# ruiminshen/yolo-tf

Hardware: AMD Instinct MI355X
Metric: train_throughput (higher is better)
Workload: dtype bf16; 1 GPU; Darknet-19 YOLOv2 VOC-20 416x416 training step (standardise+fwd+loss+bwd+Adam), batch 16 per GPU (BASELINE configs[1]); global_batch=16, parallelism=dp1, optimizer=adam, weights=random-init (Xavier, seed 0), collective=none (1 rank)

## Files before the change

include/yolo2_hip.h:

```cpp
#ifndef YOLO2_HIP_H
#define YOLO2_HIP_H

#include <stddef.h>
#include <stdint.h>

#ifdef __cplusplus
extern "C" {
#endif

enum { YOLO2_F32 = 0, YOLO2_BF16 = 1 };
enum {
    YOLO2_OK = 0,
    YOLO2_E_ARG = 1,
    YOLO2_E_LAUNCH = 2,
    YOLO2_E_UNSUPPORTED = 3
};

int yolo2_abi_version(void);
const char *yolo2_last_error(void);
uint32_t yolo2_crc32c(const void *data, size_t n, uint32_t crc);
int yolo2_shutdown(void);
int yolo2_check_async_errors(void *stream);
#define YOLO2_ASYNC_ERROR_WORDS 8
int yolo2_async_error_snapshot(unsigned *host_words, void *stream);

size_t yolo2_conv2d_workspace_bytes(int B, int H, int W, int Cp, int Nf, int ksize, int dtype);
size_t yolo2_bn_workspace_bytes(int C);
size_t yolo2_bias_grad_workspace_bytes(int ld);
size_t yolo2_image_prep_workspace_bytes(int B);
size_t yolo2_loss_workspace_bytes(int B, int cells, int A);
size_t yolo2_nms_workspace_bytes(int B, int N, int C);
size_t yolo2_clip_workspace_bytes(int nseg);
size_t yolo2_augment_workspace_bytes(int B);

int yolo2_conv2d(const void *P, const void *F, const float *bias, void *O,
                 int B, int H, int W, int Cp, int ldp, int Nf, int ldo, int ksize,
                 int dtype, void *stream);

int yolo2_conv2d_ws(const void *P, const void *F, const float *bias, void *O, float *ws,
                    size_t ws_bytes, int B, int H, int W, int Cp, int ldp, int Nf, int ldo,
                    int ksize, int dtype, void *stream);

int yolo2_conv2d_wgrad_accumulates(int B, int H, int W, int Cin, int ldx, int Cout, int ldy, int ksize, int dtype);
int yolo2_conv2d_wgrad(const void *X, const void *dY, float *dW,
                       int B, int H, int W, int Cin, int ldx, int Cout, int ldy, int ksize,
                       int dtype, void *stream);

size_t yolo2_conv2d_wgrad_workspace_bytes(int B, int H, int W, int Cin, int ldx, int Cout, int ldy, int ksize, int dtype);
int yolo2_conv2d_wgrad_ws(const void *X, const void *dY, float *dW, float *ws, size_t ws_bytes, int B, int H, int W,
                          int Cin, int ldx, int Cout, int ldy, int ksize, int dtype, void *stream);
int yolo2_set_deterministic(int on);
int yolo2_get_deterministic(void);

int yolo2_filter_prep(const float *W, void *Ffwd, void *Fdgr, int ksize, int Cin, int ldcin,
                      int Cout, int ldcout, int dtype, void *stream);

#define YOLO2_FILTER_PREP_TILE 64
#define YOLO2_FILTER_PREP_TILE_N 128
int yolo2_filter_prep_blocks(int ksize, int ldcin, int ldcout);
typedef struct yolo2_filter_desc {
    const float *W;
    void *Ffwd;
    void *Fdgr;
    int ksize, cin, ldcin, cout, ldcout, first_block;
} yolo2_filter_desc;
int yolo2_filter_prep_batch(const yolo2_filter_desc *descs_device, int n, int total_blocks, int dtype,
                            void *stream);

int yolo2_adam_filter_prep(const yolo2_filter_desc *descs_device, int n, int total_blocks, const long *small_ranges_device, int n_small,
                           float *params, const float *grads, float *m, float *v, float alpha, float beta1, float beta2, float eps,
                           float gscale, int dtype, void *stream);

int yolo2_conv2d_bias_leaky(const void *P, const void *F, const float *bias, void *O, float *ws, size_t ws_bytes, int B,
                            int H, int W, int Cp, int ldp, int Nf, int ldo, int ksize, float alpha, int dtype, void *stream);

int yolo2_conv2d_dgrad_bn(const void *dY, const void *F, void *dX, float *ws, size_t ws_bytes, int B, int H, int W, int Cp, int ldp,
                          int Nf, int ldo, int ksize, const void *Yprev, const float *mean, const float *var, const float *gamma,
                          const float *beta, float *dgamma, float *dbeta, float *bn_part, double *red_ws, float eps, float alpha,
                          int *pending, int dtype, void *stream);
int yolo2_conv2d_dgrad_bn_fuses(int B, int H, int W, int Nf, int ksize, int dtype);
int yolo2_bn_part_to_grads(float *bn_part, int C, float *dgamma, float *dbeta, void *stream);

#define YOLO2_BN_PART_ROWS 256
int yolo2_conv2d_bn(const void *P, const void *F, void *O, float *ws, size_t ws_bytes, int B, int H, int W, int Cp, int ldp,
                    int Nf, int ldo, int ksize, const float *shift, float *bn_part, int dtype, void *stream);
int yolo2_bn_finalize(float *bn_part, const float *shift, long M, int C, float *mean, float *var, float *moving_mean,
                      float *moving_var, double decay, void *stream);

int yolo2_last_bn_part_rows(void);
int yolo2_bn_fin_supported(int rows, int C, int dtype);
int yolo2_bn_leaky_fin(const void *Y, const float *bn_part, int rows, const float *shift, float *mean, float *var, float *moving_mean,
                       float *moving_var, double decay, const float *gamma, const float *beta, void *A, long M, int C, int lda,
                       float eps, float alpha, float *zero, long zero_floats, int dtype, void *stream);
int yolo2_bn_leaky_pool_fin(const void *Y, const float *bn_part, int rows, const float *shift, float *mean, float *var,
                            float *moving_mean, float *moving_var, double decay, const float *gamma, const float *beta, void *P,
                            unsigned char *idx, void *ymax, void *A_full, int B, int H, int W, int C, int ldp, float eps, float alpha,
                            float *zero, long zero_floats, int dtype, void *stream);
int yolo2_bn_leaky_bwd_apply_fin(const void *dA, int ldda, const void *Y, const float *mean, const float *var, const float *gamma,
                                 const float *beta, const float *part, int rows, long plane_stride, float *dgamma, float *dbeta,
                                 void *dY, long M, int C, float eps, float alpha, float *zero, long zero_floats, int dtype, void *stream);
int yolo2_bn_leaky_pool_bwd_apply_fin(const void *dP, int lddp, const unsigned char *idx, const void *Y, const float *mean,
                                      const float *var, const float *gamma, const float *beta, const float *part, int rows,
                                      long plane_stride, float *dgamma, float *dbeta, void *dY, int B, int H, int W, int C, float eps,
                                      float alpha, float *zero, long zero_floats, int dtype, void *stream);
int yolo2_first_layer_wgrad_bn(const void *X, const void *Y, const void *dP, int lddp, const unsigned char *idx, const float *mean, const float *var,
                               const float *gamma, const float *beta, const float *part, int rows, long plane_stride, float *dgamma, float *dbeta,
                               float *dW, int B, int H, int W, int Cin, float eps, float alpha, float *zero, long zero_floats, int dtype, void *stream);
int yolo2_bn_leaky_bwd_reduce_part(const void *dA, int ldda, const void *Y, const float *mean, const float *var, const float *gamma,
                                   const float *beta, double *ws, int *rows, int rows_limit, long M, int C, float eps, float alpha,
                                   int dtype, void *stream);
int yolo2_bn_leaky_pool_bwd_reduce_part(const void *dP, int lddp, const unsigned char *idx, const void *Y, const float *mean,
                                        const float *var, const float *gamma, const float *beta, double *ws, int *rows,
                                        int rows_limit, int B, int H, int W, int C, float eps, float alpha, int dtype, void *stream);

int yolo2_first_layer_stats(const void *P, const void *F, int B, int H, int W, const float *shift, float *bn_part, int dtype, void *stream);
int yolo2_first_layer_bn_leaky_pool(const void *P, const void *F, const float *mean, const float *var, const float *gamma,
                                    const float *beta, void *Pout, unsigned char *idx, int B, int H, int W, int ldp, float eps,
                                    float alpha, int dtype, void *stream);
int yolo2_first_layer_pool_bwd_reduce(const void *P, const void *F, const void *dP, int lddp, const unsigned char *idx,
                                      const float *mean, const float *var, const float *gamma, const float *beta, float *bn_part,
                                      int B, int H, int W, float eps, float alpha, int dtype, void *stream);
int yolo2_first_layer_pool_bwd_apply(const void *P, const void *F, const void *dP, int lddp, const unsigned char *idx,
                                     const float *mean, const float *var, const float *gamma, const float *beta,
                                     const float *dgamma, const float *dbeta, void *dY, int B, int H, int W, float eps, float alpha,
                                     int dtype, void *stream);

int yolo2_bn_stats(const void *Y, float *mean, float *var, double *ws, long M, int C,
                   int dtype, void *stream);
int yolo2_bn_stats_ema(const void *Y, float *mean, float *var, float *moving_mean, float *moving_var,
                       double decay, double *ws, long M, int C, int dtype, void *stream);
int yolo2_bn_ema(float *moving_mean, float *moving_var, const float *mean, const float *var,
                 int C, double decay, void *stream);
int yolo2_bn_leaky(const void *Y, const float *mean, const float *var, const float *gamma,
                   const float *beta, void *A, long M, int C, int lda, float eps, float alpha,
                   int dtype, void *stream);
int yolo2_bn_leaky_bwd_reduce(const void *dA, int ldda, const void *Y, const float *mean,
                              const float *var, const float *gamma, const float *beta,
                              float *dgamma, float *dbeta, double *ws, long M, int C,
                              float eps, float alpha, int dtype, void *stream);
int yolo2_bn_leaky_bwd_apply(const void *dA, int ldda, const void *Y, const float *mean,
                             const float *var, const float *gamma, const float *beta,
                             const float *dgamma, const float *dbeta, void *dY, long M, int C,
                             float eps, float alpha, int dtype, void *stream);

int yolo2_bn_leaky_pool(const void *Y, const float *mean, const float *var, const float *gamma, const float *beta, void *P,
                        unsigned char *idx, int B, int H, int W, int C, int ldp, float eps, float alpha, int dtype, void *stream);
int yolo2_bn_leaky_pool_bwd_reduce(const void *dP, int lddp, const unsigned char *idx, const void *Y, const float *mean,
                                   const float *var, const float *gamma, const float *beta, float *dgamma, float *dbeta,
                                   double *ws, int B, int H, int W, int C, float eps, float alpha, int dtype, void *stream);
int yolo2_bn_leaky_pool_bwd_apply(const void *dP, int lddp, const unsigned char *idx, const void *Y, const float *mean,
                                  const float *var, const float *gamma, const float *beta, const float *dgamma,
                                  const float *dbeta, void *dY, int B, int H, int W, int C, float eps, float alpha,
                                  int dtype, void *stream);

int yolo2_maxpool_fwd(const void *A, void *P, int B, int H, int W, int C, int stride,
                      int dtype, void *stream);
int yolo2_maxpool_bwd(const void *A, const void *dP, void *dA, int B, int H, int W, int C,
                      int stride, int dtype, void *stream);
int yolo2_maxpool_bwd_acc(const void *A, const void *dP, void *dA, int B, int H, int W, int C, int dtype, void *stream);

int yolo2_reorg(const void *in, void *out, int B, int H, int W, int C, int ldo, int dtype,
                void *stream);
int yolo2_reorg_bwd(const void *dout, int ldd, void *din, int B, int H, int W, int C, int dtype,
                    void *stream);
int yolo2_copy_channels(const void *src, int lds, void *dst, int ldd, long M, int C, int dtype,
                        void *stream);
int yolo2_add_inplace(void *dst, const void *src, long n, int dtype, void *stream);
int yolo2_bias_grad(const void *dY, int ld, float *dbias, double *ws, long M, int C, int dtype,
                    void *stream);

int yolo2_image_prep(const float *img, void *out, double *ws, int B, int HW, int mode, int dtype,
                     void *stream);

int yolo2_head_decode(const void *logits, int ld, const float *anchors, float *conf,
                      float *xy_min, float *xy_max, int *nan_flag, int B, int cell_h, int cell_w,
                      int A, int C, int dtype, void *stream);

int yolo2_head_decode_attrs(const void *logits, int ld, const float *anchors, float *iou, float *prob,
                            float *xy, float *wh, int B, int cell_h, int cell_w, int A, int C,
                            int dtype, void *stream);

int yolo2_loss(const void *logits, int ld, const float *anchors, const float *mask,
               const float *prob, const float *coords, const float *off_min, const float *off_max,
               const float *areas, const float *hparam, float *objectives, void *dlogits,
               float *ws, int B, int cell_h, int cell_w, int A, int C, int dtype, void *stream);
int yolo2_loss_partials(const void *logits, int ld, const float *anchors, const float *mask, const float *prob,
                        const float *coords, const float *off_min, const float *off_max, const float *areas,
                        const float *hparam, void *dlogits, float *ws, int B, int cell_h, int cell_w, int A, int C, int dtype,
                        void *stream);
int yolo2_loss_objectives(const float *ws, float *objectives, int B, int cell_h, int cell_w, int A, void *stream);
int yolo2_loss_box(const void *logits, int ld, const float *anchors, const float *mask,
                   const float *prob, const float *coords, const float *off_min, const float *off_max,
                   const float *areas, const float *hparam, float *objectives, void *dlogits,
                   float *ws, int B, int cell_h, int cell_w, int A, int C, int dtype, void *stream, int box_loss);
int yolo2_loss_box_partials(const void *logits, int ld, const float *anchors, const float *mask, const float *prob,
                            const float *coords, const float *off_min, const float *off_max, const float *areas,
                            const float *hparam, void *dlogits, float *ws, int B, int cell_h, int cell_w, int A, int C, int dtype,
                            void *stream, int box_loss);
typedef struct yolo2_loss_options {
    int   size;
    int   box_loss;
    int   class_loss;
    int   rescore;
    float ignore_thresh;
    float label_smoothing;
    float focal_gamma;
} yolo2_loss_options;
int yolo2_loss_ex(const void *logits, int ld, const float *anchors, const float *mask,
                  const float *prob, const float *coords, const float *off_min, const float *off_max,
                  const float *areas, const float *hparam, float *objectives, void *dlogits,
                  float *ws, int B, int cell_h, int cell_w, int A, int C, int dtype, void *stream, const yolo2_loss_options *opt);
int yolo2_loss_ex_partials(const void *logits, int ld, const float *anchors, const float *mask, const float *prob,
                           const float *coords, const float *off_min, const float *off_max, const float *areas,
                           const float *hparam, void *dlogits, float *ws, int B, int cell_h, int cell_w, int A, int C, int dtype,
                           void *stream, const yolo2_loss_options *opt);

int yolo1_loss(const void *net, int ld, const float *mask, const float *prob, const float *coords, const float *off_min,
               const float *off_max, const float *areas, const float *hparam, float *objectives, void *dnet, float *ws,
               int B, int cell_h, int cell_w, int boxes_per_cell, int C, int dtype, void *stream);
int yolo1_head_decode(const void *net, int ld, float *conf, float *xy_min, float *xy_max, int *nan_flag, int B, int cell_h,
                      int cell_w, int boxes_per_cell, int C, int dtype, void *stream);
int yolo2_leaky_bwd(const void *A, const void *dA, void *dZ, long n, float alpha, int dtype, void *stream);
int yolo2_dropout(const void *X, void *Y, unsigned char *mask, long n, float keep_prob, unsigned long long seed, int dtype,
                  void *stream);
int yolo2_dropout_bwd(const void *dY, const unsigned char *mask, void *dX, long n, float keep_prob, int dtype, void *stream);
int yolo2_l2_regularizer(const float *w, float *g, long n, float scale, double *loss, void *stream);

int yolo2_nms(float *conf, const float *xy_min, const float *xy_max, int *order_out, int *ws,
              int B, int N, int C, float threshold, float threshold_iou, void *stream);

#define YOLO2_NMS_HARD 0
#define YOLO2_NMS_LINEAR 1
#define YOLO2_NMS_GAUSSIAN 2
int yolo2_soft_nms(float *conf, const float *xy_min, const float *xy_max, int *order_out, int B, int N, int C, int method,
                   float threshold, float threshold_iou, float sigma, void *stream);

#define YOLO2_WBF_MAX_CANDIDATES 4096
#define YOLO2_WBF_FLAG_CANDIDATES 1
#define YOLO2_WBF_FLAG_CLUSTERS 2
#define YOLO2_WBF_FLAG_ROWS 4
size_t yolo2_wbf_workspace_bytes(int B, int C, int max_per_class);
int yolo2_tta_gather(const float *conf, const float *xy_min, const float *xy_max, float *out_conf, float *out_xy_min, float *out_xy_max,
                     int B, int N, int C, int M, int offset, float sx, float sy, float cell_w0, int flip, void *stream);
int yolo2_wbf(const float *conf, const float *xy_min, const float *xy_max, float *out_conf, float *out_xy_min, float *out_xy_max, int *rows,
              int *flags, void *ws, int B, int M, int C, int V, int max_per_class, int R, float threshold, float fuse_iou, void *stream);

int yolo2_adam(float *w, const float *g, float *m, float *v, long n, float alpha, float beta1,
               float beta2, float eps, float gscale, void *stream);
int yolo2_momentum(float *w, const float *g, float *acc, long n, float lr, float momentum,
                   float gscale, void *stream);
int yolo2_sgd(float *w, const float *g, long n, float lr, float gscale, void *stream);
int yolo2_rmsprop(float *w, const float *g, float *ms, float *mom, long n, float lr, float decay,
                  float momentum, float eps, float gscale, void *stream);
int yolo2_adagrad(float *w, const float *g, float *acc, long n, float lr, float gscale,
                  void *stream);
int yolo2_adadelta(float *w, const float *g, float *acc, float *acc_update, long n, float lr,
                   float rho, float eps, float gscale, void *stream);
int yolo2_ftrl(float *w, const float *g, float *accum, float *linear, long n, float lr, float lr_power,
               float l1, float l2, float gscale, void *stream);
int yolo2_ema_update(float *ema, const float *w, long n, float one_minus_decay, void *stream);
enum { YOLO2_GRAD_STORE = 0, YOLO2_GRAD_ADD = 1, YOLO2_GRAD_FINAL = 2 };
#define YOLO2_GRAD_COMBINE_CHUNK 4096
int yolo2_grad_combine(float *g, float *acc, float *w, long n, int mode, float scale, float decay, float shrink,
                       const long *ranges_device, int n_ranges, void *stream);
int yolo2_scale(float *x, long n, float scale, void *stream);
int yolo2_zero_ranges(float *x, const long *ranges_host, int nranges, void *stream);
int yolo2_bn_fold(const float *W, const float *gamma, const float *beta, const float *moving_mean,
                  const float *moving_var, float *Wf, float *bias, long rows, int C, float eps, void *stream);
int yolo2_clip_by_norm(float *g, const long *seg_off, int nseg, float clip, double *ws,
                       void *stream);
size_t yolo2_clip_fixed_workspace_bytes(int nseg);
int yolo2_clip_by_norm_fixed(float *g, const long *seg_off, int nseg, float clip, double *ws, size_t ws_bytes, void *stream);

int yolo2_selftest_tr16(short *out, void *stream);
int yolo2_debug_last_conv_plan(int *out8);
int yolo2_debug_conv_route(int B, int H, int W, int Cp, int ldp, int Nf, int ldo, int ksize, int dtype, int mode, int align_bits, size_t ws_bytes,
                           int cus, unsigned exclude, int *out12);
int yolo2_debug_noop(void *stream);
int yolo2_debug_set_igemm_tap(int mode);
int yolo2_debug_set_s4_abl(int abl);
int yolo2_debug_set_pp(int grid, int sched, int min_steps, int min_share);
int yolo2_debug_set_pp_cost(int cv);
int yolo2_debug_set_streamk_wait_us(int us, int unclamped);
int yolo2_debug_last_wgrad_plan(int *out8);
void yolo2_debug_set_wgrad_variant(int variant);
int yolo2_debug_wgrad_row_plan(int B, int H, int W, int Cin, int Cout, int cus, int force_variant, int *out9);
int yolo2_debug_wgrad_ws_plan(int B, int H, int W, int Cin, int ldx, int Cout, int ldy, int ksize, int dtype, int cus, int *out4);
int yolo2_debug_magic_u32(unsigned d, unsigned *m, unsigned *s);

#define YOLO2_AUG_FLIP 1u
#define YOLO2_AUG_BRIGHTNESS 2u
#define YOLO2_AUG_SATURATION 4u
#define YOLO2_AUG_HUE 8u
#define YOLO2_AUG_CONTRAST 16u
#define YOLO2_AUG_NOISE 32u
#define YOLO2_AUG_GRAY 64u
typedef struct yolo2_augment_params {
    long long src_offset;
    int src_w, src_h;
    int crop_x, crop_y, crop_w, crop_h;
    unsigned flags;
    float brightness, saturation, hue, contrast, noise_scale;
    unsigned long long noise_seed;
} yolo2_augment_params;
int yolo2_augment_images(const unsigned char *src, const yolo2_augment_params *params_device, double *ws, float *out,
                         int B, int H, int W, int any_contrast, void *stream);

typedef struct yolo2_compose_tile {
    long long src_offset;
    int src_w, src_h;
    int crop_x, crop_y, crop_w, crop_h;
    int view_w, view_h;
    int origin_x, origin_y;
    int x0, y0, x1, y1;
    unsigned flip;
} yolo2_compose_tile;
int yolo2_compose_images(const unsigned char *src, const yolo2_compose_tile *tiles, const yolo2_augment_params *photo,
                         const float *mix, double *ws, float *out, int B, int L, int T, int H, int W, float fill,
                         int any_contrast, void *stream);

int yolo2_transform_labels(const int *objects_class, const float *objects_coord, const int *first_object, float *mask,
                           float *prob, float *coords, float *offset_xy_min, float *offset_xy_max, float *areas, int B,
                           int classes, int cell_width, int cell_height, int *error_flag, void *stream);

int yolo2_set_stream_workgroups(int n);
int yolo2_get_stream_workgroups(void);
int yolo2_cast_f32_bf16(const float *src, void *dst, long n, void *stream);
int yolo2_cast_bf16_f32(const void *src, float *dst, long n, void *stream);
int yolo2_debug_occupy(int workgroups, int *stop, int *started, int max_us, void *stream);

enum { YOLO2_EVAL_MODE_DETECT = 0, YOLO2_EVAL_MODE_ALL = 1 };
enum { YOLO2_EVAL_FP = 0, YOLO2_EVAL_TP = 1, YOLO2_EVAL_IGNORED = 2 };
#define YOLO2_EVAL_MAX_GT_PER_IMAGE 512
#define YOLO2_EVAL_MAX_CLASSES (1 << 20)
#define YOLO2_EVAL_STATE_WORDS 2
typedef struct {
    float score;
    int image;
    int box;
    unsigned class_flag;
} yolo2_eval_record;
size_t yolo2_eval_record_bytes(long max_records);
size_t yolo2_eval_collect_workspace_bytes(int B);
size_t yolo2_eval_workspace_bytes(long max_records, int C);
size_t yolo2_eval_result_bytes(int C);
int yolo2_eval_collect(const float *conf, const float *xy_min, const float *xy_max, const int *gt_class, const float *gt_box,
                       const unsigned char *gt_difficult, const int *gt_first, int G, int B, int N, int C, int n_valid, int image_base,
                       int mode, float threshold, float iou_threshold, void *records, long max_records, unsigned long long *state,
                       int *npos, int *ws, void *stream);
int yolo2_eval_finalize(const void *records, long max_records, unsigned long long *state, const int *npos, int C, int n_images, int N,
                        void *ws, size_t ws_bytes, void *results, void *sorted_records, int *cum_tp, int *cum_fp, void *stream);

#define YOLO2_EVAL_COCO_MAX_AREAS 4
#define YOLO2_EVAL_COCO_MAX_IOUS 10
#define YOLO2_EVAL_COCO_MAX_RECALLS 101
#define YOLO2_EVAL_COCO_MAX_SLICES 8
#define YOLO2_EVAL_COCO_MAX_DETS 128
#define YOLO2_EVAL_COCO_MAX_CLASSES 1024
typedef struct {
    float score;
    int image;
    int box;
    int cls;
    int rank;
    unsigned reserved;
    unsigned long long matched;
    unsigned long long ignored;
} yolo2_eval_coco_record;
size_t yolo2_eval_coco_record_bytes(long max_records);
size_t yolo2_eval_coco_collect_workspace_bytes(int B, int N, int C);
size_t yolo2_eval_coco_workspace_bytes(long max_records, int C);
size_t yolo2_eval_coco_result_bytes(int S, int T, int A, int C);
int yolo2_eval_coco_collect(const float *conf, const float *xy_min, const float *xy_max, const int *gt_class, const float *gt_box,
                            const float *gt_area, const unsigned char *gt_flags, const int *gt_first, const float *scale, int G, int B,
                            int N, int C, int n_valid, int image_base, int mode, float threshold, const float *area_ranges, int A,
                            const float *iou_thresholds, int T, int max_dets, void *records, long max_records,
                            unsigned long long *state, int *npig, void *ws, size_t ws_bytes, void *stream);
int yolo2_eval_coco_finalize(const void *records, long max_records, unsigned long long *state, const int *npig, int C, int n_images, int N,
                             int A, int T, int max_dets, const int *slices, int S, const double *recall_thresholds, int R, void *ws,
                             size_t ws_bytes, void *results, void *stream);

#define YOLO2_ANCHOR_MAX_K 32
#define YOLO2_ANCHOR_MAX_JOBS 65535
#define YOLO2_ANCHOR_MAX_BOXES ((1 << 27) - 1)
size_t yolo2_anchor_workspace_bytes(int jobs, int kmax);
int yolo2_anchor_assign(const float *boxes, int n, const float *centroids, const int *job_k, int jobs, int kmax,
                        unsigned long long *ws, size_t ws_bytes, const int *done, unsigned char *assignment, void *stream);
int yolo2_anchor_update(float *centroids, const int *job_k, int jobs, int kmax, unsigned long long *ws, size_t ws_bytes, int n,
                        int *done, int *iterations, long long *counts, double *avg_iou, void *stream);

#define YOLO2_HIST_BUCKETS 1550
#define YOLO2_HIST_WORDS (YOLO2_HIST_BUCKETS + 6)
typedef struct yolo2_hist_job {
    const void *base;
    long long rows;
    int c, ld, dtype;
    int first_item;
} yolo2_hist_job;
size_t yolo2_histogram_workspace_bytes(int njobs);
size_t yolo2_histogram_result_bytes(int njobs);
int yolo2_histogram_items(long long rows, int c, int ld, int dtype);
int yolo2_histogram(const yolo2_hist_job *jobs, int njobs, int items, void *out, size_t out_bytes, void *ws, size_t ws_bytes, void *stream);

#define YOLO2_IMAGE_GROUP 8
#define YOLO2_IMAGE_RECORD_BYTES 16
typedef struct yolo2_image_job {
    const void *base;
    long long rows;
    int c, ld, dtype;
    int first_item;
    long long out_offset;
    long long sum_offset;
} yolo2_image_job;
size_t yolo2_image_summary_workspace_bytes(int njobs, long long sum_pixels);
size_t yolo2_image_summary_result_bytes(int njobs, long long image_bytes);
int yolo2_image_summary_items(long long rows, int c, int ld, int dtype);
// ... 32 lines not shown
```

yolo_tf_amd/_lib.py:

```python
import ctypes
import os

_HERE = os.path.dirname(os.path.abspath(__file__))
LIB_PATH = os.environ.get('YOLO2_LIB_PATH') or os.path.join(_HERE, 'csrc', 'libyolo2hip.so')

F32, BF16 = 0, 1
I8_OUT_I8, I8_OUT_BF16, I8_OUT_F32, I8_OUT_ACC = 0, 1, 2, 3
NMS_METHODS = {'hard': 0, 'linear': 1, 'gaussian': 2}
BOX_LOSSES = {'mse': 0, 'iou': 1, 'giou': 2, 'diou': 3, 'ciou': 4}
CLASS_LOSSES = {'mse': 0, 'ce': 1, 'focal': 2}


class HipKernelError(RuntimeError):
    pass


class LossOptions(ctypes.Structure):
    _fields_ = [('size', ctypes.c_int), ('box_loss', ctypes.c_int), ('class_loss', ctypes.c_int), ('rescore', ctypes.c_int),
                ('ignore_thresh', ctypes.c_float), ('label_smoothing', ctypes.c_float), ('focal_gamma', ctypes.c_float)]


_p = ctypes.c_void_p
_i = ctypes.c_int
_l = ctypes.c_long
_f = ctypes.c_float

SIGNATURES = {
    'yolo2_conv2d': [_p, _p, _p, _p, _i, _i, _i, _i, _i, _i, _i, _i, _i, _p],
    'yolo2_conv2d_ws': [_p, _p, _p, _p, _p, ctypes.c_size_t, _i, _i, _i, _i, _i, _i, _i, _i, _i, _p],
    'yolo2_conv2d_bias_leaky': [_p, _p, _p, _p, _p, ctypes.c_size_t, _i, _i, _i, _i, _i, _i, _i, _i, _f, _i, _p],
    'yolo2_conv2d_dgrad_bn': [_p, _p, _p, _p, ctypes.c_size_t, _i, _i, _i, _i, _i, _i, _i, _i, _p, _p, _p, _p, _p, _p, _p, _p, _p, _f, _f, _p, _i, _p],
    'yolo2_bn_part_to_grads': [_p, _i, _p, _p, _p],
    'yolo2_debug_noop': [_p],
    'yolo2_conv2d_wgrad': [_p, _p, _p, _i, _i, _i, _i, _i, _i, _i, _i, _i, _p],
    'yolo2_conv2d_wgrad_ws': [_p, _p, _p, _p, ctypes.c_size_t, _i, _i, _i, _i, _i, _i, _i, _i, _i, _p],
    'yolo2_set_deterministic': [_i],
    'yolo2_filter_prep': [_p, _p, _p, _i, _i, _i, _i, _i, _i, _p],
    'yolo2_filter_prep_batch': [_p, _i, _i, _i, _p],
    'yolo2_adam_filter_prep': [_p, _i, _i, _p, _i, _p, _p, _p, _p, _f, _f, _f, _f, _f, _i, _p],
    'yolo2_first_layer_stats': [_p, _p, _i, _i, _i, _p, _p, _i, _p],
    'yolo2_first_layer_bn_leaky_pool': [_p, _p, _p, _p, _p, _p, _p, _p, _i, _i, _i, _i, _f, _f, _i, _p],
    'yolo2_first_layer_pool_bwd_reduce': [_p, _p, _p, _i, _p, _p, _p, _p, _p, _p, _i, _i, _i, _f, _f, _i, _p],
    'yolo2_first_layer_pool_bwd_apply': [_p, _p, _p, _i, _p, _p, _p, _p, _p, _p, _p, _p, _i, _i, _i, _f, _f, _i, _p],
    'yolo2_conv2d_bn': [_p, _p, _p, _p, ctypes.c_size_t, _i, _i, _i, _i, _i, _i, _i, _i, _p, _p, _i, _p],
    'yolo2_bn_finalize': [_p, _p, _l, _i, _p, _p, _p, _p, ctypes.c_double, _p],
    'yolo2_bn_leaky_fin': [_p, _p, _i, _p, _p, _p, _p, _p, ctypes.c_double, _p, _p, _p, _l, _i, _i, _f, _f, _p, _l, _i, _p],
    'yolo2_bn_leaky_pool_fin': [_p, _p, _i, _p, _p, _p, _p, _p, ctypes.c_double, _p, _p, _p, _p, _p, _p, _i, _i, _i, _i, _i, _f, _f, _p, _l, _i, _p],
    'yolo2_bn_leaky_bwd_apply_fin': [_p, _i, _p, _p, _p, _p, _p, _p, _i, _l, _p, _p, _p, _l, _i, _f, _f, _p, _l, _i, _p],
    'yolo2_first_layer_wgrad_bn': [_p, _p, _p, _i, _p, _p, _p, _p, _p, _p, _i, _l, _p, _p, _p, _i, _i, _i, _i, _f, _f, _p, _l, _i, _p],
    'yolo2_bn_leaky_pool_bwd_apply_fin': [_p, _i, _p, _p, _p, _p, _p, _p, _p, _i, _l, _p, _p, _p, _i, _i, _i, _i, _f, _f, _p, _l, _i, _p],
    'yolo2_bn_leaky_bwd_reduce_part': [_p, _i, _p, _p, _p, _p, _p, _p, _p, _i, _l, _i, _f, _f, _i, _p],
    'yolo2_bn_leaky_pool_bwd_reduce_part': [_p, _i, _p, _p, _p, _p, _p, _p, _p, _p, _i, _i, _i, _i, _i, _f, _f, _i, _p],
    'yolo2_bn_leaky_pool': [_p, _p, _p, _p, _p, _p, _p, _i, _i, _i, _i, _i, _f, _f, _i, _p],
    'yolo2_bn_leaky_pool_bwd_reduce': [_p, _i, _p, _p, _p, _p, _p, _p, _p, _p, _p, _i, _i, _i, _i, _f, _f, _i, _p],
    'yolo2_bn_leaky_pool_bwd_apply': [_p, _i, _p, _p, _p, _p, _p, _p, _p, _p, _p, _i, _i, _i, _i, _f, _f, _i, _p],
    'yolo2_augment_images': [_p, _p, _p, _p, _i, _i, _i, _i, _p],
    'yolo2_compose_images': [_p, _p, _p, _p, _p, _p, _i, _i, _i, _i, _i, _f, _i, _p],
    'yolo2_transform_labels': [_p, _p, _p, _p, _p, _p, _p, _p, _p, _i, _i, _i, _i, _p, _p],
    'yolo2_bn_stats': [_p, _p, _p, _p, _l, _i, _i, _p],
    'yolo2_bn_stats_ema': [_p, _p, _p, _p, _p, ctypes.c_double, _p, _l, _i, _i, _p],
    'yolo2_bn_ema': [_p, _p, _p, _p, _i, ctypes.c_double, _p],
    'yolo2_bn_leaky': [_p, _p, _p, _p, _p, _p, _l, _i, _i, _f, _f, _i, _p],
    'yolo2_bn_leaky_bwd_reduce': [_p, _i, _p, _p, _p, _p, _p, _p, _p, _p, _l, _i, _f, _f, _i, _p],
    'yolo2_bn_leaky_bwd_apply': [_p, _i, _p, _p, _p, _p, _p, _p, _p, _p, _l, _i, _f, _f, _i, _p],
    'yolo2_maxpool_fwd': [_p, _p, _i, _i, _i, _i, _i, _i, _p],
    'yolo2_maxpool_bwd': [_p, _p, _p, _i, _i, _i, _i, _i, _i, _p],
    'yolo2_maxpool_bwd_acc': [_p, _p, _p, _i, _i, _i, _i, _i, _p],
    'yolo2_reorg': [_p, _p, _i, _i, _i, _i, _i, _i, _p],
    'yolo2_reorg_bwd': [_p, _i, _p, _i, _i, _i, _i, _i, _p],
    'yolo2_copy_channels': [_p, _i, _p, _i, _l, _i, _i, _p],
    'yolo2_add_inplace': [_p, _p, _l, _i, _p],
    'yolo2_bias_grad': [_p, _i, _p, _p, _l, _i, _i, _p],
    'yolo2_image_prep': [_p, _p, _p, _i, _i, _i, _i, _p],
    'yolo2_head_decode': [_p, _i, _p, _p, _p, _p, _p, _i, _i, _i, _i, _i, _i, _p],
    'yolo2_head_decode_attrs': [_p, _i, _p, _p, _p, _p, _p, _i, _i, _i, _i, _i, _i, _p],
    'yolo2_loss': [_p, _i, _p, _p, _p, _p, _p, _p, _p, ctypes.POINTER(_f), _p, _p, _p, _i, _i, _i, _i, _i, _i, _p],
    'yolo2_loss_partials': [_p, _i, _p, _p, _p, _p, _p, _p, _p, ctypes.POINTER(_f), _p, _p, _i, _i, _i, _i, _i, _i, _p],
    'yolo2_loss_objectives': [_p, _p, _i, _i, _i, _i, _p],
    'yolo2_loss_box': [_p, _i, _p, _p, _p, _p, _p, _p, _p, ctypes.POINTER(_f), _p, _p, _p, _i, _i, _i, _i, _i, _i, _p, _i],
    'yolo2_loss_box_partials': [_p, _i, _p, _p, _p, _p, _p, _p, _p, ctypes.POINTER(_f), _p, _p, _i, _i, _i, _i, _i, _i, _p, _i],
    'yolo2_loss_ex': [_p, _i, _p, _p, _p, _p, _p, _p, _p, ctypes.POINTER(_f), _p, _p, _p, _i, _i, _i, _i, _i, _i, _p, ctypes.POINTER(LossOptions)],
    'yolo2_loss_ex_partials': [_p, _i, _p, _p, _p, _p, _p, _p, _p, ctypes.POINTER(_f), _p, _p, _i, _i, _i, _i, _i, _i, _p, ctypes.POINTER(LossOptions)],
    'yolo1_loss': [_p, _i, _p, _p, _p, _p, _p, _p, ctypes.POINTER(_f), _p, _p, _p, _i, _i, _i, _i, _i, _i, _p],
    'yolo1_head_decode': [_p, _i, _p, _p, _p, _p, _i, _i, _i, _i, _i, _i, _p],
    'yolo2_leaky_bwd': [_p, _p, _p, _l, _f, _i, _p],
    'yolo2_dropout': [_p, _p, _p, _l, _f, ctypes.c_ulonglong, _i, _p],
    'yolo2_dropout_bwd': [_p, _p, _p, _l, _f, _i, _p],
    'yolo2_l2_regularizer': [_p, _p, _l, _f, _p, _p],
    'yolo2_nms': [_p, _p, _p, _p, _p, _i, _i, _i, _f, _f, _p],
    'yolo2_soft_nms': [_p, _p, _p, _p, _i, _i, _i, _i, _f, _f, _f, _p],
    'yolo2_tta_gather': [_p, _p, _p, _p, _p, _p, _i, _i, _i, _i, _i, _f, _f, _f, _i, _p],
    'yolo2_wbf': [_p, _p, _p, _p, _p, _p, _p, _p, _p, _i, _i, _i, _i, _i, _i, _f, _f, _p],
    'yolo2_adam': [_p, _p, _p, _p, _l, _f, _f, _f, _f, _f, _p],
    'yolo2_momentum': [_p, _p, _p, _l, _f, _f, _f, _p],
    'yolo2_sgd': [_p, _p, _l, _f, _f, _p],
    'yolo2_rmsprop': [_p, _p, _p, _p, _l, _f, _f, _f, _f, _f, _p],
    'yolo2_adagrad': [_p, _p, _p, _l, _f, _f, _p],
    'yolo2_adadelta': [_p, _p, _p, _p, _l, _f, _f, _f, _f, _p],
    'yolo2_clip_by_norm': [_p, _p, _i, _f, _p, _p],
    'yolo2_clip_by_norm_fixed': [_p, _p, _i, _f, _p, ctypes.c_size_t, _p],
    'yolo2_ftrl': [_p, _p, _p, _p, _l, _f, _f, _f, _f, _f, _p],
    'yolo2_scale': [_p, _l, _f, _p],
    'yolo2_ema_update': [_p, _p, _l, _f, _p],
    'yolo2_grad_combine': [_p, _p, _p, _l, _i, _f, _f, _f, _p, _i, _p],
    'yolo2_zero_ranges': [_p, _p, _i, _p],
    'yolo2_bn_fold': [_p, _p, _p, _p, _p, _p, _p, _l, _i, _f, _p],
    'yolo2_selftest_tr16': [_p, _p],
    'yolo2_set_stream_workgroups': [_i],
    'yolo2_cast_f32_bf16': [_p, _p, _l, _p],
    'yolo2_cast_bf16_f32': [_p, _p, _l, _p],
    'yolo2_debug_occupy': [_i, _p, _p, _i, _p],
    'yolo2_check_async_errors': [_p],
    'yolo2_async_error_snapshot': [_p, _p],
    'yolo2_debug_set_streamk_wait_us': [_i, _i],
    'yolo2_eval_collect': [_p, _p, _p, _p, _p, _p, _p, _i, _i, _i, _i, _i, _i, _i, _f, _f, _p, _l, _p, _p, _p, _p],
    'yolo2_eval_finalize': [_p, _l, _p, _p, _i, _i, _i, _p, ctypes.c_size_t, _p, _p, _p, _p, _p],
    'yolo2_eval_coco_collect': [_p] * 9 + [_i] * 7 + [_f, _p, _i, _p, _i, _i, _p, _l, _p, _p, _p, ctypes.c_size_t, _p],
    'yolo2_eval_coco_finalize': [_p, _l, _p, _p, _i, _i, _i, _i, _i, _i, _p, _i, _p, _i, _p, ctypes.c_size_t, _p, _p],
    'yolo2_anchor_assign': [_p, _i, _p, _p, _i, _i, _p, ctypes.c_size_t, _p, _p, _p],
    'yolo2_anchor_update': [_p, _p, _i, _i, _p, ctypes.c_size_t, _i, _p, _p, _p, _p, _p],
    'yolo2_histogram': [_p, _i, _i, _p, ctypes.c_size_t, _p, ctypes.c_size_t, _p],
    'yolo2_image_summary': [_p, _i, _i, _p, ctypes.c_size_t, _p, ctypes.c_size_t, _p],
    'yolo2_conv2d_i8': [_p, _p, _p, _p, _p, _i, _i, _i, _i, _i, _i, _i, _i, _f, _f, _i, _p],
    'yolo2_absmax': [_p, _i, _p, _p],
    'yolo2_calib_histogram': [_p, _i, _p, _p],
    'yolo2_quantize': [_p, _i, _p, _i, _l, _i, _f, _i, _p],
    'yolo2_maxpool_i8': [_p, _i, _p, _i, _i, _i, _i, _i, _i, _p],
    'yolo2_reorg_i8': [_p, _p, _i, _i, _i, _i, _i, _p],
}

QUERIES = {
    'yolo2_abi_version': (_i, []),
    'yolo2_last_error': (ctypes.c_char_p, []),
    'yolo2_shutdown': (_i, []),
    'yolo2_crc32c': (ctypes.c_uint32, [_p, ctypes.c_size_t, ctypes.c_uint32]),
    'yolo2_conv2d_wgrad_accumulates': (_i, [_i] * 9),
    'yolo2_filter_prep_blocks': (_i, [_i, _i, _i]),
    'yolo2_conv2d_dgrad_bn_fuses': (_i, [_i] * 6),
    'yolo2_debug_set_wgrad_variant': (None, [_i]),
    'yolo2_last_bn_part_rows': (_i, []),
    'yolo2_get_stream_workgroups': (_i, []),
    'yolo2_bn_fin_supported': (_i, [_i, _i, _i]),
    'yolo2_debug_last_conv_plan': (_i, [ctypes.POINTER(_i)]),
    'yolo2_debug_conv_route': (_i, [_i] * 11 + [ctypes.c_size_t, _i, ctypes.c_uint, ctypes.POINTER(_i)]),
    'yolo2_debug_set_igemm_tap': (_i, [_i]),
    'yolo2_debug_set_pp': (_i, [_i, _i, _i, _i]),
    'yolo2_debug_set_pp_cost': (_i, [_i]),
    'yolo2_debug_set_s4_abl': (_i, [_i]),
    'yolo2_debug_last_wgrad_plan': (_i, [ctypes.POINTER(_i)]),
    'yolo2_debug_wgrad_row_plan': (_i, [_i, _i, _i, _i, _i, _i, _i, ctypes.POINTER(_i)]),
    'yolo2_debug_wgrad_ws_plan': (_i, [_i] * 10 + [ctypes.POINTER(_i)]),
    'yolo2_conv2d_wgrad_workspace_bytes': (ctypes.c_size_t, [_i] * 9),
    'yolo2_get_deterministic': (_i, []),
    'yolo2_debug_magic_u32': (_i, [ctypes.c_uint, ctypes.POINTER(ctypes.c_uint), ctypes.POINTER(ctypes.c_uint)]),
    'yolo2_conv2d_workspace_bytes': (ctypes.c_size_t, [_i] * 7),
    'yolo2_bn_workspace_bytes': (ctypes.c_size_t, [_i]),
    'yolo2_bias_grad_workspace_bytes': (ctypes.c_size_t, [_i]),
    'yolo2_image_prep_workspace_bytes': (ctypes.c_size_t, [_i]),
    'yolo2_loss_workspace_bytes': (ctypes.c_size_t, [_i, _i, _i]),
    'yolo2_nms_workspace_bytes': (ctypes.c_size_t, [_i, _i, _i]),
    'yolo2_wbf_workspace_bytes': (ctypes.c_size_t, [_i, _i, _i]),
    'yolo2_clip_workspace_bytes': (ctypes.c_size_t, [_i]),
    'yolo2_clip_fixed_workspace_bytes': (ctypes.c_size_t, [_i]),
    'yolo2_augment_workspace_bytes': (ctypes.c_size_t, [_i]),
    'yolo2_eval_record_bytes': (ctypes.c_size_t, [_l]),
    'yolo2_eval_collect_workspace_bytes': (ctypes.c_size_t, [_i]),
    'yolo2_eval_workspace_bytes': (ctypes.c_size_t, [_l, _i]),
    'yolo2_eval_result_bytes': (ctypes.c_size_t, [_i]),
    'yolo2_eval_coco_record_bytes': (ctypes.c_size_t, [_l]),
    'yolo2_eval_coco_collect_workspace_bytes': (ctypes.c_size_t, [_i, _i, _i]),
    'yolo2_eval_coco_workspace_bytes': (ctypes.c_size_t, [_l, _i]),
    'yolo2_eval_coco_result_bytes': (ctypes.c_size_t, [_i, _i, _i, _i]),
    'yolo2_anchor_workspace_bytes': (ctypes.c_size_t, [_i, _i]),
    'yolo2_histogram_workspace_bytes': (ctypes.c_size_t, [_i]),
    'yolo2_histogram_result_bytes': (ctypes.c_size_t, [_i]),
    'yolo2_histogram_items': (_i, [ctypes.c_longlong, _i, _i, _i]),
    'yolo2_image_summary_workspace_bytes': (ctypes.c_size_t, [_i, ctypes.c_longlong]),
    'yolo2_image_summary_result_bytes': (ctypes.c_size_t, [_i, ctypes.c_longlong]),
    'yolo2_image_summary_items': (_i, [ctypes.c_longlong, _i, _i, _i]),
    'yolo2_image_summary_depth': (_i, [_i]),
}


class AugmentParams(ctypes.Structure):
    _fields_ = [('src_offset', ctypes.c_longlong), ('src_w', _i), ('src_h', _i), ('crop_x', _i), ('crop_y', _i), ('crop_w', _i), ('crop_h', _i),
                ('flags', ctypes.c_uint), ('brightness', _f), ('saturation', _f), ('hue', _f), ('contrast', _f), ('noise_scale', _f),
                ('noise_seed', ctypes.c_ulonglong)]


class ComposeTile(ctypes.Structure):
    _fields_ = [('src_offset', ctypes.c_longlong), ('src_w', _i), ('src_h', _i), ('crop_x', _i), ('crop_y', _i), ('crop_w', _i), ('crop_h', _i),
                ('view_w', _i), ('view_h', _i), ('origin_x', _i), ('origin_y', _i), ('x0', _i), ('y0', _i), ('x1', _i), ('y1', _i),
                ('flip', ctypes.c_uint)]


class HistJob(ctypes.Structure):
    _fields_ = [('base', ctypes.c_void_p), ('rows', ctypes.c_longlong), ('c', _i), ('ld', _i), ('dtype', _i), ('first_item', _i)]


class ImageJob(ctypes.Structure):
    _fields_ = [('base', ctypes.c_void_p), ('rows', ctypes.c_longlong), ('c', _i), ('ld', _i), ('dtype', _i), ('first_item', _i),
                ('out_offset', ctypes.c_longlong), ('sum_offset', ctypes.c_longlong)]


class AbsmaxJob(ctypes.Structure):
    _fields_ = [('base', ctypes.c_void_p), ('rows', ctypes.c_longlong), ('c', _i), ('ld', _i), ('dtype', _i), ('slot', _i)]


CALIB_BINS = 2048
CALIB_WORDS = CALIB_BINS + 2


class CalibJob(ctypes.Structure):
    _fields_ = [('base', ctypes.c_void_p), ('rows', ctypes.c_longlong), ('c', _i), ('ld', _i), ('dtype', _i), ('slot', _i), ('limit', _f), ('inv_width', _f)]


class FilterDesc(ctypes.Structure):
    _fields_ = [('W', ctypes.c_void_p), ('Ffwd', ctypes.c_void_p), ('Fdgr', ctypes.c_void_p), ('ksize', _i), ('cin', _i),
                ('ldcin', _i), ('cout', _i), ('ldcout', _i), ('first_block', _i)]


_lib = None
MISSING = set()


def _mapped_hip_runtimes():
    try:
        with open('/proc/self/maps') as f:
            return sorted({line.split()[-1] for line in f if 'libamdhip64' in line})
    except OSError:
        return []


def load():
    global _lib
    if _lib is not None:
        return _lib
    if not os.path.exists(LIB_PATH):
        raise HipKernelError(
            'HIP extension %s is missing: run `python yolo_tf_amd/csrc/build.py` (or __graft_entry__.build()). '
            'There is no CPU fallback.' % LIB_PATH)
    import torch
    lib = ctypes.CDLL(LIB_PATH)
    runtimes = _mapped_hip_runtimes()
    if len(runtimes) > 1:
        raise HipKernelError('two HIP runtimes are mapped in this process (%s): something loaded %s before torch' % (', '.join(runtimes), LIB_PATH))
    baseline = os.environ.get('YOLO2_LIB_BASELINE') == '1' and bool(os.environ.get('YOLO2_LIB_PATH'))

    def resolve(name):
        try:
            return getattr(lib, name)
        except AttributeError:
            if not baseline:
                raise
            MISSING.add(name)

            def absent(*_args, _name=name):
                raise HipKernelError('%s is not exported by the baseline library %s' % (_name, LIB_PATH))
            setattr(lib, name, absent)
            return None
    for name, (res, args) in QUERIES.items():
        fn = resolve(name)
        if fn is not None:
            fn.restype = res
            fn.argtypes = args
    for name, args in SIGNATURES.items():
        fn = resolve(name)
        if fn is not None:
            fn.restype = _i
            fn.argtypes = args
    _lib = lib
    over = env_overrides()
    if over:
        import warnings
        warnings.warn('YOLO2_* switches set in the environment change kernel selection away from the tested defaults: %s' % ', '.join(over))
    return lib


def env_overrides():
    return sorted('%s=%s' % (k, v) for k, v in os.environ.items() if k.startswith('YOLO2_'))


def query(name, *args):
    return getattr(load(), name)(*args)


def call(name, *args):
    lib = load()
    rc = getattr(lib, name)(*args)
    if rc != 0:
        raise HipKernelError('%s failed (code %d): %s' % (name, rc, lib.yolo2_last_error().decode()))


def ptr(t):
    return None if t is None else t.data_ptr()


def dtype_code(torch_dtype):
    import torch
    if torch_dtype == torch.float32:
        return F32
    if torch_dtype == torch.bfloat16:
        return BF16
    raise ValueError('unsupported dtype %r' % (torch_dtype,))
```

yolo_tf_amd/csrc/bn.hip:

```cpp
#include "common.h"
#include "bn_leaky.h"
#include "colsum.h"

template <typename T>
__global__ __launch_bounds__(256) void bn_leaky_kernel(const T *__restrict__ Y, const float *__restrict__ mean, const float *__restrict__ var,
                                                       const float *__restrict__ gamma, const float *__restrict__ beta, T *__restrict__ A,
                                                       long M, int C, int lda, float eps, float alpha) {
    constexpr int N = Vec16<T>::N;
    RowMap rm(C, N);
    if (!rm.active) return;
    float mu[N], sc[N], bt[N];
#pragma unroll
    for (int j = 0; j < N; ++j) {
        int c = rm.cg * N + j;
        mu[j] = mean[c];
        sc[j] = bn_inv_std(var[c], eps) * gamma[c];
        bt[j] = beta[c];
    }
    for (long r = (long)blockIdx.x * rm.rpp + rm.rs; r < M; r += (long)gridDim.x * rm.rpp) {
        Vec16<T> v = ld16(Y + r * C + rm.cg * N), o;
#pragma unroll
        for (int j = 0; j < N; ++j) o.set(j, bn_leaky(v.get(j), mu[j], sc[j], bt[j], alpha));
        st16(A + r * lda + rm.cg * N, o);
    }
}

static int rowmap_grid(long M, int C, int vec, int rows_per_thread) {
    int tpr = C / vec, rpp = 256 / tpr;
    if (rpp < 1) rpp = 1;
    long g = (M + (long)rpp * rows_per_thread - 1) / ((long)rpp * rows_per_thread);
    if (g > 4096) g = 4096;
    if (g < 1) g = 1;
    return (int)g;
}

extern "C" int yolo2_bn_leaky(const void *Y, const float *mean, const float *var, const float *gamma, const float *beta,
                              void *A, long M, int C, int lda, float eps, float alpha, int dtype, void *stream) {
    Y2_CHECK_ARG(Y && mean && var && gamma && beta && A && M > 0 && C > 0 && lda >= C);
    const int vec = dtype == YOLO2_BF16 ? 8 : 4;
    Y2_CHECK_ARG(C % vec == 0 && C / vec <= 256 && lda % vec == 0);
    int grid = rowmap_grid(M, C, vec, 4);
    Y2_DISPATCH_DTYPE(dtype, bn_leaky_kernel<T><<<grid, 256, 0, (hipStream_t)stream>>>((const T *)Y, mean, var, gamma, beta, (T *)A, M, C, lda, eps, alpha));
    Y2_CHECK_LAUNCH();
    return YOLO2_OK;
}

template <typename T>
__global__ __launch_bounds__(256) void bn_bwd_reduce_kernel(const T *__restrict__ dA, int ldda, const T *__restrict__ Y, const float *__restrict__ mean,
                                                            const float *__restrict__ var, const float *__restrict__ gamma, const float *__restrict__ beta,
                                                            float *__restrict__ ws, long M, int C, float eps, float alpha) {
    constexpr int N = Vec16<T>::N;
    RowMap rm(C, N);
    float part[2][N];
    float mu[N], inv[N], ga[N], bt[N];
#pragma unroll
    for (int j = 0; j < N; ++j) {
        part[0][j] = part[1][j] = 0.f;
        int c = rm.cg * N + j;
        bool ok = rm.active;
        mu[j] = ok ? mean[c] : 0.f;
        inv[j] = ok ? bn_inv_std(var[c], eps) : 0.f;
        ga[j] = ok ? gamma[c] : 0.f;
        bt[j] = ok ? beta[c] : 0.f;
    }
    if (rm.active) {
        const long step = (long)gridDim.x * rm.rpp;
        long r = (long)blockIdx.x * rm.rpp + rm.rs;
        auto accum = [&](const Vec16<T> &y, const Vec16<T> &d) {
#pragma unroll
            for (int j = 0; j < N; ++j) {
                const BnBwdTerm t = bn_leaky_bwd(y.get(j), d.get(j), mu[j], inv[j], ga[j], bt[j], alpha);
                part[0][j] += t.g * t.xh;
                part[1][j] += t.g;
            }
        };
        for (; r + 3 * step < M; r += 4 * step) {
            Vec16<T> y[4], d[4];
#pragma unroll
            for (int u = 0; u < 4; ++u) {
                y[u] = ld16(Y + (r + u * step) * C + rm.cg * N);
                d[u] = ld16(dA + (r + u * step) * ldda + rm.cg * N);
            }
#pragma unroll
            for (int u = 0; u < 4; ++u) accum(y[u], d[u]);
        }
        for (; r < M; r += step) {
            Vec16<T> y = ld16(Y + r * C + rm.cg * N), d = ld16(dA + r * ldda + rm.cg * N);
            accum(y, d);
        }
    }
    block_colsum_store<N, 2>(part, rm, C, ws, gridDim.x);
}
extern "C" int yolo2_bn_leaky_bwd_reduce(const void *dA, int ldda, const void *Y, const float *mean, const float *var, const float *gamma,
                                         const float *beta, float *dgamma, float *dbeta, double *ws, long M, int C, float eps, float alpha,
                                         int dtype, void *stream) {
    Y2_CHECK_ARG(dA && Y && mean && var && gamma && beta && dgamma && dbeta && ws && M > 0 && C > 0 && ldda >= C);
    const int vec = dtype == YOLO2_BF16 ? 8 : 4;
    Y2_CHECK_ARG(C % vec == 0 && C / vec <= 256 && ldda % vec == 0);
    hipStream_t st = (hipStream_t)stream;
    const int nb = colsum_grid(M, C, vec);
    float *part = (float *)ws;
    Y2_DISPATCH_DTYPE(dtype, bn_bwd_reduce_kernel<T><<<nb, 256, 0, st>>>((const T *)dA, ldda, (const T *)Y, mean, var, gamma, beta, part, M, C, eps, alpha));
    reduce_finalize_kernel<1><<<cdiv(C, 16), 256, 0, st>>>(part, nb, C, M, dgamma, dbeta, C);
    Y2_CHECK_LAUNCH();
    return YOLO2_OK;
}

template <typename T>
__global__ __launch_bounds__(256) void bn_bwd_apply_kernel(const T *__restrict__ dA, int ldda, const T *__restrict__ Y, const float *__restrict__ mean,
                                                           const float *__restrict__ var, const float *__restrict__ gamma, const float *__restrict__ beta,
                                                           const float *__restrict__ dgamma, const float *__restrict__ dbeta, T *__restrict__ dY,
                                                           long M, int C, float eps, float alpha) {
    constexpr int N = Vec16<T>::N;
    RowMap rm(C, N);
    if (!rm.active) return;
    const float invM = 1.0f / (float)M;
    float mu[N], inv[N], ga[N], bt[N], dgm[N], dbm[N];
#pragma unroll
    for (int j = 0; j < N; ++j) {
        int c = rm.cg * N + j;
        mu[j] = mean[c];
        inv[j] = bn_inv_std(var[c], eps);
        ga[j] = gamma[c];
        bt[j] = beta[c];
        dgm[j] = dgamma[c] * invM;
        dbm[j] = dbeta[c] * invM;
    }
    for (long r = (long)blockIdx.x * rm.rpp + rm.rs; r < M; r += (long)gridDim.x * rm.rpp) {
        Vec16<T> y = ld16(Y + r * C + rm.cg * N), d = ld16(dA + r * ldda + rm.cg * N), o;
#pragma unroll
        for (int j = 0; j < N; ++j) {
            float xh = (y.get(j) - mu[j]) * inv[j];
            float z = (y.get(j) - mu[j]) * (inv[j] * ga[j]) + bt[j];
            float g = z >= 0.f ? d.get(j) : alpha * d.get(j);
            o.set(j, (ga[j] * inv[j]) * (g - dbm[j] - xh * dgm[j]));
        }
        st16(dY + r * C + rm.cg * N, o);
    }
}

extern "C" int yolo2_bn_leaky_bwd_apply(const void *dA, int ldda, const void *Y, const float *mean, const float *var, const float *gamma,
                                        const float *beta, const float *dgamma, const float *dbeta, void *dY, long M, int C, float eps,
                                        float alpha, int dtype, void *stream) {
    Y2_CHECK_ARG(dA && Y && mean && var && gamma && beta && dgamma && dbeta && dY && M > 0 && C > 0 && ldda >= C);
    const int vec = dtype == YOLO2_BF16 ? 8 : 4;
    Y2_CHECK_ARG(C % vec == 0 && C / vec <= 256 && ldda % vec == 0);
    int grid = rowmap_grid(M, C, vec, 4);
    Y2_DISPATCH_DTYPE(dtype, bn_bwd_apply_kernel<T><<<grid, 256, 0, (hipStream_t)stream>>>((const T *)dA, ldda, (const T *)Y, mean, var, gamma, beta, dgamma, dbeta, (T *)dY, M, C, eps, alpha));
    Y2_CHECK_LAUNCH();
    return YOLO2_OK;
}

template <typename T>
__global__ __launch_bounds__(256) void bn_leaky_pool_kernel(const T *__restrict__ Y, const float *__restrict__ mean, const float *__restrict__ var,
                                                            const float *__restrict__ gamma, const float *__restrict__ beta, T *__restrict__ P,
                                                            unsigned char *__restrict__ idx, int B, int H, int W, int C, int ldp, float eps, float alpha) {
    constexpr int N = Vec16<T>::N;
    RowMap rm(C, N);
    if (!rm.active) return;
    float mu[N], sc[N], bt[N];
#pragma unroll
    for (int j = 0; j < N; ++j) {
        int c = rm.cg * N + j;
        mu[j] = mean[c];
        sc[j] = bn_inv_std(var[c], eps) * gamma[c];
        bt[j] = beta[c];
    }
    const PoolRow pr(H, W, C);
    const long MP = (long)B * pr.OH * pr.OW;
    for (long r = (long)blockIdx.x * rm.rpp + rm.rs; r < MP; r += (long)gridDim.x * rm.rpp) {
        const T *src = Y + pr.base(r) + rm.cg * N;
        Vec16<T> v[4], o;
        v[0] = ld16(src);
        v[1] = ld16(src + C);
        v[2] = ld16(src + (long)W * C);
        v[3] = ld16(src + (long)W * C + C);
        typename IdxPack<N>::type pack = 0;
#pragma unroll
        for (int j = 0; j < N; ++j) {
            float a[4], m;
#pragma unroll
            for (int k = 0; k < 4; ++k) a[k] = pool_round<T>(bn_leaky(v[k].get(j), mu[j], sc[j], bt[j], alpha));
            const int arg = pool_first_max(a, m);
            o.set(j, m);
            pack |= idx_pack_byte<N>(arg, j);
        }
        st16(P + r * ldp + rm.cg * N, o);
        if (idx) *reinterpret_cast<typename IdxPack<N>::type *>(idx + r * C + rm.cg * N) = pack;
    }
}

template <typename T>
__global__ __launch_bounds__(256) void bn_pool_bwd_reduce_kernel(const T *__restrict__ dP, int lddp, const unsigned char *__restrict__ idx, const T *__restrict__ Y,
                                                                 const float *__restrict__ mean, const float *__restrict__ var, const float *__restrict__ gamma,
                                                                 const float *__restrict__ beta, float *__restrict__ ws, int B, int H, int W, int C, float eps, float alpha) {
    constexpr int N = Vec16<T>::N;
    RowMap rm(C, N);
    float part[2][N];
    float mu[N], inv[N], ga[N], bt[N];
#pragma unroll
    for (int j = 0; j < N; ++j) {
        part[0][j] = part[1][j] = 0.f;
        int c = rm.cg * N + j;
        bool ok = rm.active;
        mu[j] = ok ? mean[c] : 0.f;
        inv[j] = ok ? bn_inv_std(var[c], eps) : 0.f;
        ga[j] = ok ? gamma[c] : 0.f;
        bt[j] = ok ? beta[c] : 0.f;
    }
    if (rm.active) {
        const PoolRow pr(H, W, C);
        const long MP = (long)B * pr.OH * pr.OW;
        for (long r = (long)blockIdx.x * rm.rpp + rm.rs; r < MP; r += (long)gridDim.x * rm.rpp) {
            const T *src = Y + pr.base(r) + rm.cg * N;
            Vec16<T> v[4];
            v[0] = ld16(src);
            v[1] = ld16(src + C);
            v[2] = ld16(src + (long)W * C);
            v[3] = ld16(src + (long)W * C + C);
            const Vec16<T> d = ld16(dP + r * lddp + rm.cg * N);
            const typename IdxPack<N>::type pack = *reinterpret_cast<const typename IdxPack<N>::type *>(idx + r * C + rm.cg * N);
#pragma unroll
            for (int j = 0; j < N; ++j) {
                const int k = idx_pack_get(pack, j);
                const float y = k == 0 ? v[0].get(j) : k == 1 ? v[1].get(j) : k == 2 ? v[2].get(j) : v[3].get(j);
                const float xh = (y - mu[j]) * inv[j];
                const float z = (y - mu[j]) * (inv[j] * ga[j]) + bt[j];
                const float g = z >= 0.f ? d.get(j) : alpha * d.get(j);
                part[0][j] += g * xh;
                part[1][j] += g;
            }
        }
    }
    block_colsum_store<N, 2>(part, rm, C, ws, gridDim.x);
}

template <typename T>
__global__ __launch_bounds__(256) void bn_pool_bwd_apply_kernel(const T *__restrict__ dP, int lddp, const unsigned char *__restrict__ idx, const T *__restrict__ Y,
                                                                const float *__restrict__ mean, const float *__restrict__ var, const float *__restrict__ gamma,
                                                                const float *__restrict__ beta, const float *__restrict__ dgamma, const float *__restrict__ dbeta,
                                                                T *__restrict__ dY, int B, int H, int W, int C, float eps, float alpha) {
    constexpr int N = Vec16<T>::N;
    RowMap rm(C, N);
    if (!rm.active) return;
    const float invM = 1.0f / (float)((long)B * H * W);
    float mu[N], inv[N], ga[N], bt[N], dgm[N], dbm[N];
#pragma unroll
    for (int j = 0; j < N; ++j) {
        int c = rm.cg * N + j;
        mu[j] = mean[c];
        inv[j] = bn_inv_std(var[c], eps);
        ga[j] = gamma[c];
        bt[j] = beta[c];
        dgm[j] = dgamma[c] * invM;
        dbm[j] = dbeta[c] * invM;
    }
    const PoolRow pr(H, W, C);
    const long MP = (long)B * pr.OH * pr.OW;
    for (long r = (long)blockIdx.x * rm.rpp + rm.rs; r < MP; r += (long)gridDim.x * rm.rpp) {
        const long off = pr.base(r) + rm.cg * N;
        const long koff[4] = {0, C, (long)W * C, (long)W * C + C};
        Vec16<T> v[4];
#pragma unroll
        for (int k = 0; k < 4; ++k) v[k] = ld16(Y + off + koff[k]);
        const Vec16<T> d = ld16(dP + r * lddp + rm.cg * N);
        const typename IdxPack<N>::type pack = *reinterpret_cast<const typename IdxPack<N>::type *>(idx + r * C + rm.cg * N);
#pragma unroll
        for (int k = 0; k < 4; ++k) {
            Vec16<T> o;
#pragma unroll
            for (int j = 0; j < N; ++j) {
                const float da = pool_route(idx_pack_get(pack, j), k, d.get(j));
                o.set(j, bn_bwd_apply(bn_leaky_bwd(v[k].get(j), da, mu[j], inv[j], ga[j], bt[j], alpha), inv[j], ga[j], dgm[j], dbm[j]));
            }
            st16(dY + off + koff[k], o);
        }
    }
}

struct SliceMap {
    int lpr, rpb, lane, row, cg, cs, c0;
    __device__ SliceMap(int C, int vec) {
        const int tpr = C / vec;
        lpr = tpr < 16 ? tpr : 16;
        rpb = 256 / lpr;
        lane = threadIdx.x % lpr;
        row = threadIdx.x / lpr;
        cg = blockIdx.y * lpr + lane;
        cs = lpr * vec;
        c0 = blockIdx.y * cs;
    }
};
#define Y2_SLICE_MAX 128

template <int G>
__device__ __forceinline__ void slice_wave_sums(double (&v)[4]) {
#pragma unroll
    for (int j = 0; j < 4; ++j) v[j] = y2_lane_group_sum_f64<G>(v[j]);
}
__device__ __forceinline__ void slice_partial_sums(const float *__restrict__ part, int rows, long plane, int C, const SliceMap &sm, double (&sums)[2]) {
    __shared__ double red[4 * Y2_SLICE_MAX];
    const int q = sm.cs >> 2;
    const int l4 = threadIdx.x % q, g = threadIdx.x / q, ng = 256 / q;
    const int lane = threadIdx.x & 63, wave = threadIdx.x >> 6;
    const bool valu = q == 4 || q == 8 || q == 16 || q == 32;
    sums[0] = sums[1] = 0.0;
#pragma unroll
    for (int k = 0; k < 2; ++k) {
        const float *p = part + (long)k * plane + sm.c0 + l4 * 4;
        double s[4] = {0.0, 0.0, 0.0, 0.0}, t[4] = {0.0, 0.0, 0.0, 0.0};
        for (int r = g; r < rows; r += 4 * ng) {
            f32x4 v[4];
#pragma unroll
            for (int u = 0; u < 4; ++u) v[u] = *reinterpret_cast<const f32x4 *>(p + (long)(r + u * ng < rows ? r + u * ng : g) * C);
#pragma unroll
            for (int u = 0; u < 4; ++u) {
                const bool ok = r + u * ng < rows;
#pragma unroll
                for (int j = 0; j < 4; ++j) {
                    const double x = ok ? (double)v[u][j] : 0.0;
                    if (u & 1) t[j] += x; else s[j] += x;
                }
            }
        }
#pragma unroll
        for (int j = 0; j < 4; ++j) s[j] += t[j];
        if (k) __syncthreads();
        if (valu) {
            if (q == 4) slice_wave_sums<4>(s); else if (q == 8) slice_wave_sums<8>(s); else if (q == 16) slice_wave_sums<16>(s); else slice_wave_sums<32>(s);
            if (lane < q) {
#pragma unroll
                for (int j = 0; j < 4; ++j) red[wave * sm.cs + lane * 4 + j] = s[j];
            }
            __syncthreads();
            if (threadIdx.x < sm.cs) sums[k] = (red[threadIdx.x] + red[sm.cs + threadIdx.x]) + (red[2 * sm.cs + threadIdx.x] + red[3 * sm.cs + threadIdx.x]);
        } else {
            const int gmax = 4 * Y2_SLICE_MAX / sm.cs;
            double a = 0.0;
            for (int g0 = 0; g0 < ng; g0 += gmax) {
                if (g0) __syncthreads();
                if (g >= g0 && g < g0 + gmax) {
#pragma unroll
                    for (int j = 0; j < 4; ++j) red[(g - g0) * sm.cs + l4 * 4 + j] = s[j];
                }
                __syncthreads();
                if (threadIdx.x < sm.cs)
                    for (int j = 0; j < gmax && g0 + j < ng; ++j) a += red[j * sm.cs + threadIdx.x];
            }
            if (threadIdx.x < sm.cs) sums[k] = a;
        }
    }
    __syncthreads();
}

__device__ __forceinline__ void grid_zero(float *__restrict__ zero, long zero_vec4) {
    if (!zero) return;
    const long nthreads = (long)gridDim.x * gridDim.y * 256;
    f32x4 z = {0.f, 0.f, 0.f, 0.f};
    for (long i = ((long)blockIdx.y * gridDim.x + blockIdx.x) * 256 + threadIdx.x; i < zero_vec4; i += nthreads) reinterpret_cast<f32x4 *>(zero)[i] = z;
}

template <typename T, bool POOL>
__global__ __launch_bounds__(256) void bn_leaky_fin_kernel(const T *__restrict__ Y, const float *__restrict__ part, int rows, const float *__restrict__ shift,
                                                           long Mstat, float *__restrict__ mean_out, float *__restrict__ var_out, float *__restrict__ mm,
                                                           float *__restrict__ mv, float omd, const float *__restrict__ gamma, const float *__restrict__ beta,
                                                           T *__restrict__ A, unsigned char *__restrict__ idx, T *__restrict__ ymax, T *__restrict__ Afull,
                                                           int B, int H, int W, int C, int lda, float eps, float alpha, float *__restrict__ zero, long zero_vec4) {
    constexpr int N = Vec16<T>::N;
    const SliceMap sm(C, N);
    double sums[2];
    __shared__ float cst[3][Y2_SLICE_MAX];
    const PoolRow pr(H, W, C);
    const long ML = POOL ? (long)B * pr.OH * pr.OW : (long)B * H * W;
    const long step = (long)gridDim.x * sm.rpb;
    long r = (long)blockIdx.x * sm.rpb + sm.row;
    Vec16<T> v[POOL ? 4 : 1];
    if (r < ML) {
        if (POOL) {
            const T *src = Y + pr.base(r) + sm.cg * N;
            v[0] = ld16(src);
            v[POOL ? 1 : 0] = ld16(src + C);
            v[POOL ? 2 : 0] = ld16(src + (long)W * C);
            v[POOL ? 3 : 0] = ld16(src + (long)W * C + C);
        } else v[0] = ld16(Y + r * C + sm.cg * N);
    }
    slice_partial_sums(part, rows, (long)Y2_BN_PART_ROWS * C, C, sm, sums);
    if (threadIdx.x < sm.cs) {
        const int c = sm.c0 + threadIdx.x;
        const double dm = sums[0] / (double)Mstat;
        const double var = sums[1] / (double)Mstat - dm * dm;
        const float fm = (float)((double)shift[c] + dm), fv = (float)(var > 0.0 ? var : 0.0);
        cst[0][threadIdx.x] = fm;
        cst[1][threadIdx.x] = bn_inv_std(fv, eps) * gamma[c];
        cst[2][threadIdx.x] = beta[c];
        if (blockIdx.x == 0) {
            mean_out[c] = fm;
            var_out[c] = fv;
            if (mm) {
                mm[c] = bn_ema(mm[c], fm, omd);
                mv[c] = bn_ema(mv[c], fv, omd);
            }
        }
    }
    __syncthreads();
    float mu[N], sc[N], bt[N];
#pragma unroll
    for (int j = 0; j < N; ++j) {
        mu[j] = cst[0][sm.lane * N + j];
        sc[j] = cst[1][sm.lane * N + j];
        bt[j] = cst[2][sm.lane * N + j];
    }
    grid_zero(zero, zero_vec4);
    while (r < ML) {
        const long rn = r + step;
        Vec16<T> vn[POOL ? 4 : 1];
        if (rn < ML) {
            if (POOL) {
                const T *src = Y + pr.base(rn) + sm.cg * N;
                vn[0] = ld16(src);
                vn[POOL ? 1 : 0] = ld16(src + C);
                vn[POOL ? 2 : 0] = ld16(src + (long)W * C);
                vn[POOL ? 3 : 0] = ld16(src + (long)W * C + C);
            } else vn[0] = ld16(Y + rn * C + sm.cg * N);
        }
        Vec16<T> o;
        if (!POOL) {
#pragma unroll
            for (int j = 0; j < N; ++j) o.set(j, bn_leaky(v[0].get(j), mu[j], sc[j], bt[j], alpha));
            st16(A + r * lda + sm.cg * N, o);
        } else {
            typename IdxPack<N>::type pack = 0;
            Vec16<T> ym, af[4];
#pragma unroll
            for (int j = 0; j < N; ++j) {
                float a[4], m;
#pragma unroll
                for (int k = 0; k < 4; ++k) {
                    a[k] = pool_round<T>(bn_leaky(v[POOL ? k : 0].get(j), mu[j], sc[j], bt[j], alpha));
                    af[k].set(j, a[k]);
                }
                const int arg = pool_first_max(a, m);
                o.set(j, m);
                ym.set(j, arg == 0 ? v[0].get(j) : arg == 1 ? v[POOL ? 1 : 0].get(j) : arg == 2 ? v[POOL ? 2 : 0].get(j) : v[POOL ? 3 : 0].get(j));
                pack |= idx_pack_byte<N>(arg, j);
            }
            st16(A + r * lda + sm.cg * N, o);
            if (idx) *reinterpret_cast<typename IdxPack<N>::type *>(idx + r * C + sm.cg * N) = pack;
            if (Afull) {
                T *dst = Afull + pr.base(r) + sm.cg * N;
                st16(dst, af[0]);
                st16(dst + C, af[1]);
                st16(dst + (long)W * C, af[2]);
                st16(dst + (long)W * C + C, af[3]);
            }
            if (ymax) st16(ymax + r * C + sm.cg * N, ym);
        }
#pragma unroll
        for (int k = 0; k < (POOL ? 4 : 1); ++k) v[k] = vn[k];
        r = rn;
    }
}

template <typename T, bool POOL>
__global__ __launch_bounds__(256) void bn_bwd_apply_fin_kernel(const T *__restrict__ dA, int ldda, const unsigned char *__restrict__ idx, const T *__restrict__ Y,
                                                               const float *__restrict__ mean, const float *__restrict__ var, const float *__restrict__ gamma,
                                                               const float *__restrict__ beta, const float *__restrict__ part, int rows, long plane,
                                                               float *__restrict__ dgamma, float *__restrict__ dbeta, T *__restrict__ dY, int B, int H, int W, int C,
                                                               float eps, float alpha, float *__restrict__ zero, long zero_vec4) {
    constexpr int N = Vec16<T>::N;
    const SliceMap sm(C, N);
    double sums[2];
    __shared__ float cst[2][Y2_SLICE_MAX];
    const PoolRow pr(H, W, C);
    const long ML = POOL ? (long)B * pr.OH * pr.OW : (long)B * H * W;
    const long step = (long)gridDim.x * sm.rpb;
    long r = (long)blockIdx.x * sm.rpb + sm.row;
    const long koff[4] = {0, C, (long)W * C, (long)W * C + C};
    Vec16<T> v[POOL ? 4 : 1], d;
    typename IdxPack<N>::type pack = 0;
    auto fetch = [&](long row, Vec16<T> (&yv)[POOL ? 4 : 1], Vec16<T> &dv, typename IdxPack<N>::type &pk) {
        if (POOL) {
            const long off = pr.base(row) + sm.cg * N;
#pragma unroll
            for (int k = 0; k < (POOL ? 4 : 1); ++k) yv[k] = ld16(Y + off + koff[k]);
            pk = *reinterpret_cast<const typename IdxPack<N>::type *>(idx + row * C + sm.cg * N);
        } else yv[0] = ld16(Y + row * C + sm.cg * N);
        dv = ld16(dA + row * ldda + sm.cg * N);
    };
    if (r < ML) fetch(r, v, d, pack);
    slice_partial_sums(part, rows, plane, C, sm, sums);
    if (threadIdx.x < sm.cs) {
        const float dg = (float)sums[0], db = (float)sums[1];
        cst[0][threadIdx.x] = dg;
        cst[1][threadIdx.x] = db;
        if (blockIdx.x == 0) {
            dgamma[sm.c0 + threadIdx.x] = dg;
            dbeta[sm.c0 + threadIdx.x] = db;
        }
    }
    __syncthreads();
    const float invM = 1.0f / (float)((long)B * H * W);
    float mu[N], inv[N], ga[N], bt[N], dgm[N], dbm[N];
#pragma unroll
    for (int j = 0; j < N; ++j) {
        const int c = sm.cg * N + j;
        mu[j] = mean[c];
        inv[j] = bn_inv_std(var[c], eps);
        ga[j] = gamma[c];
        bt[j] = beta[c];
        dgm[j] = cst[0][sm.lane * N + j] * invM;
        dbm[j] = cst[1][sm.lane * N + j] * invM;
    }
    grid_zero(zero, zero_vec4);
    while (r < ML) {
        const long rn = r + step;
        Vec16<T> vn[POOL ? 4 : 1], dn;
        typename IdxPack<N>::type packn = 0;
        if (rn < ML) fetch(rn, vn, dn, packn);
        if (!POOL) {
            Vec16<T> o;
#pragma unroll
            for (int j = 0; j < N; ++j) {
                float xh = (v[0].get(j) - mu[j]) * inv[j];
                float z = (v[0].get(j) - mu[j]) * (inv[j] * ga[j]) + bt[j];
                float g = z >= 0.f ? d.get(j) : alpha * d.get(j);
                o.set(j, (ga[j] * inv[j]) * (g - dbm[j] - xh * dgm[j]));
            }
            st16(dY + r * C + sm.cg * N, o);
        } else {
            const long off = pr.base(r) + sm.cg * N;
#pragma unroll
            for (int k = 0; k < 4; ++k) {
                Vec16<T> o;
#pragma unroll
                for (int j = 0; j < N; ++j) {
                    const float da = pool_route(idx_pack_get(pack, j), k, d.get(j));
                    o.set(j, bn_bwd_apply(bn_leaky_bwd(v[POOL ? k : 0].get(j), da, mu[j], inv[j], ga[j], bt[j], alpha), inv[j], ga[j], dgm[j], dbm[j]));
                }
                st16(dY + off + koff[k], o);
            }
        }
#pragma unroll
        for (int k = 0; k < (POOL ? 4 : 1); ++k) v[k] = vn[k];
        d = dn;
        pack = packn;
        r = rn;
    }
}

static bool pool_args_ok(int B, int H, int W, int C, int dtype) {
    const int vec = dtype == YOLO2_BF16 ? 8 : 4;
    return B > 0 && H > 0 && W > 0 && C > 0 && H % 2 == 0 && W % 2 == 0 && C % vec == 0 && C / vec <= 256;
}
extern "C" int yolo2_bn_leaky_pool(const void *Y, const float *mean, const float *var, const float *gamma, const float *beta, void *P,
                                   unsigned char *idx, int B, int H, int W, int C, int ldp, float eps, float alpha, int dtype, void *stream) {
    Y2_CHECK_ARG(Y && mean && var && gamma && beta && P && ldp >= C);
    Y2_CHECK_ARG(pool_args_ok(B, H, W, C, dtype) && ldp % (dtype == YOLO2_BF16 ? 8 : 4) == 0);
    const int vec = dtype == YOLO2_BF16 ? 8 : 4;
    const long MP = (long)B * (H / 2) * (W / 2);
    int grid = rowmap_grid(MP, C, vec, 2);
    Y2_DISPATCH_DTYPE(dtype, bn_leaky_pool_kernel<T><<<grid, 256, 0, (hipStream_t)stream>>>((const T *)Y, mean, var, gamma, beta, (T *)P, idx, B, H, W, C, ldp, eps, alpha));
    Y2_CHECK_LAUNCH();
    return YOLO2_OK;
}
static int pool_bwd_reduce_impl(const void *dP, int lddp, const unsigned char *idx, const void *Y, const float *mean, const float *var,
                                const float *gamma, const float *beta, float *dgamma, float *dbeta, double *ws, int *rows, int rows_limit, int B, int H, int W,
                                int C, float eps, float alpha, int dtype, void *stream) {
    Y2_CHECK_ARG(dP && idx && Y && mean && var && gamma && beta && ws && lddp >= C);
    Y2_CHECK_ARG(pool_args_ok(B, H, W, C, dtype));
    const int vec = dtype == YOLO2_BF16 ? 8 : 4;
    hipStream_t st = (hipStream_t)stream;
    const long MP = (long)B * (H / 2) * (W / 2);
    int nb = colsum_grid(MP, C, vec);
    const int big = 1024;
    if (big > nb && (long)B * H * W * C * (16 / vec) >= (64L << 20)) {
        const int tpr = C / vec, rpp = 256 / tpr < 1 ? 1 : 256 / tpr;
        long g = (MP + (long)rpp * 4 - 1) / ((long)rpp * 4);
        nb = (int)(g < big ? g : big);
        if (nb > 1024) nb = 1024;
    }
    if (nb > rows_limit) nb = rows_limit;
    float *part = (float *)ws;
    Y2_DISPATCH_DTYPE(dtype, bn_pool_bwd_reduce_kernel<T><<<nb, 256, 0, st>>>((const T *)dP, lddp, idx, (const T *)Y, mean, var, gamma, beta, part, B, H, W, C, eps, alpha));
    if (rows) *rows = nb;
    else reduce_finalize_kernel<1><<<cdiv(C, 16), 256, 0, st>>>(part, nb, C, (long)B * H * W, dgamma, dbeta, C);
    Y2_CHECK_LAUNCH();
    return YOLO2_OK;
}
extern "C" int yolo2_bn_leaky_pool_bwd_reduce(const void *dP, int lddp, const unsigned char *idx, const void *Y, const float *mean, const float *var,
                                              const float *gamma, const float *beta, float *dgamma, float *dbeta, double *ws, int B, int H, int W,
                                              int C, float eps, float alpha, int dtype, void *stream) {
    Y2_CHECK_ARG(dgamma && dbeta);
    return pool_bwd_reduce_impl(dP, lddp, idx, Y, mean, var, gamma, beta, dgamma, dbeta, ws, nullptr, 1024, B, H, W, C, eps, alpha, dtype, stream);
}
extern "C" int yolo2_bn_leaky_pool_bwd_reduce_part(const void *dP, int lddp, const unsigned char *idx, const void *Y, const float *mean, const float *var,
                                                   const float *gamma, const float *beta, double *ws, int *rows, int rows_limit, int B, int H, int W, int C,
                                                   float eps, float alpha, int dtype, void *stream) {
    Y2_CHECK_ARG(rows && rows_limit >= 1);
    return pool_bwd_reduce_impl(dP, lddp, idx, Y, mean, var, gamma, beta, nullptr, nullptr, ws, rows, rows_limit, B, H, W, C, eps, alpha, dtype, stream);
}
extern "C" int yolo2_bn_leaky_pool_bwd_apply(const void *dP, int lddp, const unsigned char *idx, const void *Y, const float *mean, const float *var,
                                             const float *gamma, const float *beta, const float *dgamma, const float *dbeta, void *dY, int B, int H,
                                             int W, int C, float eps, float alpha, int dtype, void *stream) {
    Y2_CHECK_ARG(dP && idx && Y && mean && var && gamma && beta && dgamma && dbeta && dY && lddp >= C);
    Y2_CHECK_ARG(pool_args_ok(B, H, W, C, dtype));
    const int vec = dtype == YOLO2_BF16 ? 8 : 4;
    const long MP = (long)B * (H / 2) * (W / 2);
    int grid = rowmap_grid(MP, C, vec, 2);
    Y2_DISPATCH_DTYPE(dtype, bn_pool_bwd_apply_kernel<T><<<grid, 256, 0, (hipStream_t)stream>>>((const T *)dP, lddp, idx, (const T *)Y, mean, var, gamma, beta, dgamma, dbeta, (T *)dY, B, H, W, C, eps, alpha));
    Y2_CHECK_LAUNCH();
    return YOLO2_OK;
}

static bool fin_shape_ok(int rows, int C, int dtype) {
    const int vec = dtype == YOLO2_BF16 ? 8 : 4;
    if (rows < 1 || C < vec || C % vec) return false;
    const int tpr = C / vec;
    if (tpr & (tpr - 1)) return false;
    const int lpr = tpr < 16 ? tpr : 16;
    return (long)rows * lpr * vec * 8 <= (128L << 10);
}
extern "C" int yolo2_bn_fin_supported(int rows, int C, int dtype) { return fin_shape_ok(rows, C, dtype) ? 1 : 0; }

static dim3 slice_grid(long loop_rows, int C, int vec, int rows_per_thread, int part_rows) {
    const int tpr = C / vec, lpr = tpr < 16 ? tpr : 16, rpb = 256 / lpr, slices = tpr / lpr;
    long gx = (loop_rows + (long)rpb * rows_per_thread - 1) / ((long)rpb * rows_per_thread);
    const long per = (long)part_rows * lpr * vec * 8;
    long cap = (48L << 20) / (per * slices);
    const long floor_ = (512 + slices - 1) / slices;
    if (cap < floor_) cap = floor_;
    if (cap > 4096 / slices) cap = 4096 / slices;
    if (gx > cap) gx = cap;
    if (gx < 1) gx = 1;
    return dim3((unsigned)gx, (unsigned)slices);
}
#define Y2_CHECK_ZERO(zero, zero_floats) Y2_CHECK_ARG((zero_floats) >= 0 && (zero_floats) % 4 == 0 && ((zero) || (zero_floats) == 0) && ((uintptr_t)(zero) & 15) == 0)

extern "C" int yolo2_bn_leaky_fin(const void *Y, const float *bn_part, int rows, const float *shift, float *mean, float *var, float *moving_mean,
                                  float *moving_var, double decay, const float *gamma, const float *beta, void *A, long M, int C, int lda, float eps,
                                  float alpha, float *zero, long zero_floats, int dtype, void *stream) {
    Y2_CHECK_ARG(Y && bn_part && shift && mean && var && gamma && beta && A && M > 0 && C > 0 && lda >= C && M < (1L << 31));
    Y2_CHECK_ARG((moving_mean == nullptr) == (moving_var == nullptr) && rows <= Y2_BN_PART_ROWS && fin_shape_ok(rows, C, dtype));
    Y2_CHECK_ARG(shift != moving_mean && shift != mean);
    Y2_CHECK_ZERO(zero, zero_floats);
    const int vec = dtype == YOLO2_BF16 ? 8 : 4;
    Y2_CHECK_ARG(lda % vec == 0);
    const dim3 grid = slice_grid(M, C, vec, 4, rows);
    Y2_DISPATCH_DTYPE(dtype, bn_leaky_fin_kernel<T, false><<<grid, 256, 0, (hipStream_t)stream>>>((const T *)Y, bn_part, rows, shift, M, mean, var, moving_mean, moving_var,
                      (float)(1.0 - decay), gamma, beta, (T *)A, nullptr, nullptr, nullptr, 1, 1, (int)M, C, lda, eps, alpha, zero, zero_floats / 4));
    Y2_CHECK_LAUNCH();
    return YOLO2_OK;
}

extern "C" int yolo2_bn_leaky_pool_fin(const void *Y, const float *bn_part, int rows, const float *shift, float *mean, float *var, float *moving_mean,
                                       float *moving_var, double decay, const float *gamma, const float *beta, void *P, unsigned char *idx, void *ymax,
                                       void *A_full, int B, int H, int W, int C, int ldp, float eps, float alpha, float *zero, long zero_floats, int dtype,
                                       void *stream) {
    Y2_CHECK_ARG(Y && bn_part && shift && mean && var && gamma && beta && P && ldp >= C);
    Y2_CHECK_ARG(pool_args_ok(B, H, W, C, dtype) && ldp % (dtype == YOLO2_BF16 ? 8 : 4) == 0);
    Y2_CHECK_ARG((moving_mean == nullptr) == (moving_var == nullptr) && rows <= Y2_BN_PART_ROWS && fin_shape_ok(rows, C, dtype));
    Y2_CHECK_ARG(shift != moving_mean && shift != mean);
    Y2_CHECK_ZERO(zero, zero_floats);
    const int vec = dtype == YOLO2_BF16 ? 8 : 4;
    const dim3 grid = slice_grid((long)B * (H / 2) * (W / 2), C, vec, 2, rows);
    Y2_DISPATCH_DTYPE(dtype, bn_leaky_fin_kernel<T, true><<<grid, 256, 0, (hipStream_t)stream>>>((const T *)Y, bn_part, rows, shift, (long)B * H * W, mean, var, moving_mean,
                      moving_var, (float)(1.0 - decay), gamma, beta, (T *)P, idx, (T *)ymax, (T *)A_full, B, H, W, C, ldp, eps, alpha, zero, zero_floats / 4));
    Y2_CHECK_LAUNCH();
    return YOLO2_OK;
}

extern "C" int yolo2_bn_leaky_bwd_apply_fin(const void *dA, int ldda, const void *Y, const float *mean, const float *var, const float *gamma, const float *beta,
                                            const float *part, int rows, long plane_stride, float *dgamma, float *dbeta, void *dY, long M, int C, float eps,
                                            float alpha, float *zero, long zero_floats, int dtype, void *stream) {
    Y2_CHECK_ARG(dA && Y && mean && var && gamma && beta && part && dgamma && dbeta && dY && M > 0 && C > 0 && ldda >= C && M < (1L << 31));
    Y2_CHECK_ARG(plane_stride >= (long)rows * C && fin_shape_ok(rows, C, dtype));
    Y2_CHECK_ZERO(zero, zero_floats);
    const int vec = dtype == YOLO2_BF16 ? 8 : 4;
    Y2_CHECK_ARG(ldda % vec == 0);
    const dim3 grid = slice_grid(M, C, vec, 4, rows);
    Y2_DISPATCH_DTYPE(dtype, bn_bwd_apply_fin_kernel<T, false><<<grid, 256, 0, (hipStream_t)stream>>>((const T *)dA, ldda, nullptr, (const T *)Y, mean, var, gamma, beta, part, rows,
                      plane_stride, dgamma, dbeta, (T *)dY, 1, 1, (int)M, C, eps, alpha, zero, zero_floats / 4));
    Y2_CHECK_LAUNCH();
    return YOLO2_OK;
}

extern "C" int yolo2_bn_leaky_pool_bwd_apply_fin(const void *dP, int lddp, const unsigned char *idx, const void *Y, const float *mean, const float *var,
                                                 const float *gamma, const float *beta, const float *part, int rows, long plane_stride, float *dgamma,
                                                 float *dbeta, void *dY, int B, int H, int W, int C, float eps, float alpha, float *zero, long zero_floats,
                                                 int dtype, void *stream) {
    Y2_CHECK_ARG(dP && idx && Y && mean && var && gamma && beta && part && dgamma && dbeta && dY && lddp >= C);
    Y2_CHECK_ARG(pool_args_ok(B, H, W, C, dtype) && plane_stride >= (long)rows * C && fin_shape_ok(rows, C, dtype));
    Y2_CHECK_ZERO(zero, zero_floats);
    const int vec = dtype == YOLO2_BF16 ? 8 : 4;
    const dim3 grid = slice_grid((long)B * (H / 2) * (W / 2), C, vec, 2, rows);
    Y2_DISPATCH_DTYPE(dtype, bn_bwd_apply_fin_kernel<T, true><<<grid, 256, 0, (hipStream_t)stream>>>((const T *)dP, lddp, idx, (const T *)Y, mean, var, gamma, beta, part, rows,
                      plane_stride, dgamma, dbeta, (T *)dY, B, H, W, C, eps, alpha, zero, zero_floats / 4));
    Y2_CHECK_LAUNCH();
    return YOLO2_OK;
}

extern "C" int yolo2_bn_leaky_bwd_reduce_part(const void *dA, int ldda, const void *Y, const float *mean, const float *var, const float *gamma,
                                              const float *beta, double *ws, int *rows, int rows_limit, long M, int C, float eps, float alpha, int dtype,
                                              void *stream) {
    Y2_CHECK_ARG(dA && Y && mean && var && gamma && beta && ws && rows && rows_limit >= 1 && M > 0 && C > 0 && ldda >= C);
    const int vec = dtype == YOLO2_BF16 ? 8 : 4;
    Y2_CHECK_ARG(C % vec == 0 && C / vec <= 256 && ldda % vec == 0);
    int nb = colsum_grid(M, C, vec);
    const int big = 1024;
    if (big > nb && M * C * (16 / vec) * 2 >= (32L << 20)) {
        const int tpr = C / vec, rpp = 256 / tpr < 1 ? 1 : 256 / tpr;
        const long g = (M + (long)rpp * 16 - 1) / ((long)rpp * 16);
        nb = (int)(g < big ? g : big);
        if (nb > 1024) nb = 1024;
    }
    if (nb > rows_limit) nb = rows_limit;
    Y2_DISPATCH_DTYPE(dtype, bn_bwd_reduce_kernel<T><<<nb, 256, 0, (hipStream_t)stream>>>((const T *)dA, ldda, (const T *)Y, mean, var, gamma, beta, (float *)ws, M, C, eps, alpha));
    Y2_CHECK_LAUNCH();
    *rows = nb;
    return YOLO2_OK;
}
```

yolo_tf_amd/engine.py:

```python
import numpy as np
import os
from collections import namedtuple

import torch

from . import ops, _lib
from .graph import pad8

BN_EPS = 1e-5
BN_DECAY = 0.999
LEAKY_ALPHA = 0.1

_DTYPES = {'bf16': torch.bfloat16, 'bfloat16': torch.bfloat16, 'f32': torch.float32, 'float32': torch.float32}


BN_PART_ROWS = 256
ARENA_ALIGN = 64


def layout_params(graph):
    offsets, off = {}, 0
    for v in reversed(graph.trainable()):
        offsets[v.name] = (off, v.size)
        off += (v.size + ARENA_ALIGN - 1) // ARENA_ALIGN * ARENA_ALIGN
    return offsets, off


def layer_end_offsets(graph, offsets):
    ends = {}
    for op in graph.ops:
        if op['kind'] == 'conv':
            names = [op['weights'].name] + [op[k].name for k in ('gamma', 'beta', 'biases') if k in op]
            ends[op['name']] = max(offsets[n][0] + (offsets[n][1] + ARENA_ALIGN - 1) // ARENA_ALIGN * ARENA_ALIGN for n in names)
    return ends


Options = namedtuple('Options', 'deterministic sync_bn fuse_pool fold_bn fuse_bn_stats fold_finalize fuse_first fuse_first_wgrad fuse_bn_bwd '
                                'overlap_wgrad side_priority')


def read_options(training, deterministic=False, sync_bn=False, side_priority=-1, env=None):
    env = os.environ if env is None else env
    det, sync = bool(deterministic) and training, bool(sync_bn) and training

    def on(name):
        return env.get(name, '1') != '0'
    return Options(
        deterministic=det, sync_bn=sync,
        fuse_pool=on('YOLO2_FUSE_POOL'),
        fold_bn=on('YOLO2_FOLD_BN'),
        fuse_bn_stats=on('YOLO2_FUSE_BN_STATS') and not det,
        fold_finalize=on('YOLO2_FOLD_FINALIZE') and not sync,
        fuse_first='infer' if det else env.get('YOLO2_FUSE_FIRST', 'infer'),
        fuse_first_wgrad=on('YOLO2_FUSE_FIRST_WGRAD') and not det,
        fuse_bn_bwd=on('YOLO2_FUSE_BN_BWD') and not det,
        overlap_wgrad=on('YOLO2_OVERLAP_WGRAD'),
        side_priority=int(env.get('YOLO2_SIDE_PRIORITY', str(side_priority))))


LayerPlan = namedtuple('LayerPlan', 'path pool fwd_pool stats fin_limit first_wgrad bn_bwd zero')
Plan = namedtuple('Plan', 'layers zero_ranges unstored fused_pool fwd_pool bn_bwd_fused')


def plan_binding(graph, batch, dtype, training, opts, pools='all'):
    assert pools in ('all', 'image'), pools
    inputs = set(graph.inputs.values())
    ld = {t: t.storage()[2] for t in graph.tensors}
    readers = {}
    for op in graph.ops:
        for t in (op.get('inputs') or [op['x']]):
            readers[t] = readers.get(t, 0) + 1
    convs = [op for op in graph.ops if op['kind'] == 'conv']
    producers = {op['out']: op for op in convs}
    fused_pool, fwd_pool = {}, {}
    for op in graph.ops if opts.fuse_pool else ():
        x = op.get('x')
        if (op['kind'] == 'pool' and op['stride'] == 2 and x in producers and producers[x]['bn'] and x.h % 2 == 0 and x.w % 2 == 0
                and ld[x] == x.c and ld[op['out']] == op['out'].c and ld[producers[x]['y']] == x.c and x.c // (8 if dtype == torch.bfloat16 else 4) <= 256):
            if readers[x] > 1:
                if training:
                    fwd_pool[x] = op
            elif pools == 'all' or producers[x]['x'] in inputs:
                fused_pool[x] = op
    offsets, _ = layout_params(graph)
    fin_limits, layers, bn_bwd_fused, unstored, ranges = {}, {}, {}, set(), []
    for op in convs:
        x, out, cin, cout, k = op['x'], op['out'], op['cin'], op['cout'], op['ksize']
        pool = fused_pool.get(out)
        image = (op['bn'] and x in inputs and k == 3 and cin <= 8 and ld[x] == 8 and cout == 32 and pool is not None and ld[pool['out']] >= 32
                 and x.h % 2 == 0 and x.w % 2 == 0)
        if not training and opts.fold_bn and op['bn'] and pool is None and x not in inputs:
            path = 'fold'
        elif image and cin == 3 and opts.fuse_first != '0' and (not training or (opts.fuse_first == '1' and opts.fuse_bn_stats)):
            path = 'first'
        else:
            path = 'bn' if op['bn'] else 'bias_leaky' if op['act'] else 'bias'
        fin_limit = 0
        if training and op['bn'] and opts.fold_finalize:
            if cout not in fin_limits:
                fin_limits[cout] = ops.bn_fin_rows_limit(cout, dtype)
            fin_limit = fin_limits[cout]
        first_wgrad = bool(training and image and path != 'first' and opts.fuse_first_wgrad and ld[pool['out']] % 8 == 0 and fin_limit >= 128
                           and 'yolo2_first_layer_wgrad_bn' not in _lib.MISSING)
        bn_bwd = None
        if (training and opts.fuse_bn_bwd and x in producers and producers[x]['bn'] and readers[x] == 1 and x not in fused_pool
                and x.storage()[0] not in inputs and ld[x] == x.c and ld[producers[x]['y']] == x.c
                and ops.conv2d_dgrad_bn_fuses(batch, x.h, x.w, cin, k, dtype)):
            bn_bwd = bn_bwd_fused[op['name']] = producers[x]
        zero = bool(training and not opts.deterministic and (
            first_wgrad or ops.conv2d_wgrad_accumulates(batch, x.h, x.w, cin, ld[x], cout, pad8(cout), k, dtype)))
        if zero:
            off, size = offsets[op['weights'].name]
            ranges.append((off, off + (size + 3) // 4 * 4))
        if training and pool is not None:
            unstored.add(out)
        if training and path == 'first':
            unstored.add(op['y'])
        layers[op['name']] = LayerPlan(path, pool, fwd_pool.get(out), bool(path == 'bn' and training and opts.fuse_bn_stats and ld[op['y']] == cout),
                                       fin_limit, first_wgrad, bn_bwd, zero)
    zero_ranges = []
    for a, b in sorted(ranges):
        if zero_ranges and a - zero_ranges[-1][1] <= (1 << 20):
            zero_ranges[-1] = (zero_ranges[-1][0], max(zero_ranges[-1][1], b))
        else:
            zero_ranges.append((a, b))
    return Plan(layers, zero_ranges, frozenset(unstored), fused_pool, fwd_pool, bn_bwd_fused)


_SKEW_KB = 20
_skew_counter = [0]


def staggered(n, dtype, device, fill=0.0):
    esz = torch.empty(0, dtype=dtype).element_size()
    if _SKEW_KB <= 0 or n * esz < (1 << 20):
        return torch.full((n,), fill, dtype=dtype, device=device) if fill else torch.zeros(n, dtype=dtype, device=device)
    k = _skew_counter[0] = _skew_counter[0] + 1
    skew = (k % 16) * _SKEW_KB * 1024 // esz
    base = torch.full((n + 16 * _SKEW_KB * 1024 // esz,), fill, dtype=dtype, device=device) if fill else torch.zeros(n + 16 * _SKEW_KB * 1024 // esz, dtype=dtype, device=device)
    return base[skew:skew + n]


class _PartPool(object):

    def __init__(self, n, floats, device):
        self.bufs = [torch.zeros(floats, dtype=torch.float32, device=device) for _ in range(n)]
        self.dirty = [0] * n
        self.busy = [False] * n

    def acquire(self, floats):
        for i, (d, b) in enumerate(zip(self.dirty, self.busy)):
            if d == 0 and not b:
                break
        else:
            i = next(j for j, b in enumerate(self.busy) if not b)
            self.bufs[i][:self.dirty[i]].zero_()
        self.dirty[i] = int(floats)
        self.busy[i] = True
        return i

    def consumed(self, i, cleared=False):
        self.busy[i] = False
        if cleared:
            self.dirty[i] = 0

    def take_to_zero(self, exclude):
        for i, (d, b) in enumerate(zip(self.dirty, self.busy)):
            if i != exclude and d and not b:
                self.dirty[i] = 0
                return self.bufs[i], d
        return None, 0


_Sums = namedtuple('_Sums', 'buf rows stride part')


class Engine(object):
    def __init__(self, graph, batch_size, dtype='bf16', training=True, seed=0, device=None, sync_bn=False, side_priority=-1, deterministic=False,
                 pools='all'):
        self.deterministic = bool(deterministic) and training
        if self.deterministic and any(op.get('l2') or (op['kind'] == 'conv' and not op['bn'] and op['act']) for op in graph.ops):
            raise NotImplementedError('deterministic=True covers the YOLOv2 family: the YOLO (v1) fully connected head is not audited')
        if not torch.cuda.is_available():
            raise RuntimeError('yolo_tf_amd.Engine needs an MI355X (no CPU path exists)')
        ops._lib.load()
        self.sync_bn = bool(sync_bn) and training
        self.bn_group, self.bn_world = None, 1
        self.graph = graph
        self.B = int(batch_size)
        self.dtype = _DTYPES[dtype] if isinstance(dtype, str) else dtype
        self.training = training
        self.device = torch.device(device if device is not None else 'cuda:%d' % torch.cuda.current_device())
        self.opts = o = read_options(training, self.deterministic, self.sync_bn, side_priority)
        self.pools = pools
        self.fuse_bn_stats, self.fuse_first_wgrad, self.fold_finalize = o.fuse_bn_stats, o.fuse_first_wgrad, o.fold_finalize
        self.overlap_wgrad = o.overlap_wgrad
        self._alloc_variables()
        self._alloc_activations()
        self.init_variables(seed)
        self._filters_dirty = True
        self.reg_loss = torch.zeros(1, dtype=torch.float64, device=self.device)
        self._has_l2 = any(op.get('l2') for op in graph.ops)
        self.dropout_masks = None
        self.dropout_seed = int(seed) + 1
        self.dropout_rank = 0
        self.dropout_step = 0
        self._dropout_calls = 0
        self._masks = {}
        self._phase = 'fwd'
        self.kernel_timer = None

    def _alloc_variables(self):
        g = self.graph
        other = [v for v in g.variables.values() if not v.trainable]
        self.param_offsets, off = layout_params(g)
        self.n_params = off
        self.params = staggered(off, torch.float32, self.device)
        self.grads = staggered(off, torch.float32, self.device) if self.training else None
        self.state_offsets = {}
        off = 0
        for v in other:
            self.state_offsets[v.name] = (off, v.size)
            off += (v.size + 3) // 4 * 4
        self.state = torch.zeros(max(off, 4), dtype=torch.float32, device=self.device)
        self.state_snap = torch.zeros_like(self.state)
        self.svar = {}
        self.var = {}
        self.gvar = {}
        for name, (o, n) in self.param_offsets.items():
            self.var[name] = self.params[o:o + n]
            if self.training:
                self.gvar[name] = self.grads[o:o + n]
        for name, (o, n) in self.state_offsets.items():
            self.var[name] = self.state[o:o + n]
            self.svar[name] = self.state_snap[o:o + n]
        segs = sorted(self.param_offsets.values())
        self.seg_off = torch.tensor([s[0] for s in segs] + [self.n_params], dtype=torch.int64, device=self.device)
        self.n_seg = len(segs)

    def init_variables(self, seed=0):
        rng = np.random.RandomState(seed)
        for v in self.graph.variables.values():
            self.var[v.name].copy_(torch.from_numpy(v.init(rng, v.shape).reshape(-1)))
        self._filters_dirty = True

    def get_variables(self):
        torch.cuda.synchronize()
        return {v.name: self.var[v.name].cpu().numpy().reshape(v.shape) for v in self.graph.variables.values()}

    def set_variables(self, values, strict=True):
        for v in self.graph.variables.values():
            if v.name in values:
                a = np.asarray(values[v.name], np.float32)
                assert a.shape == v.shape, (v.name, a.shape, v.shape)
                self.var[v.name].copy_(torch.from_numpy(np.ascontiguousarray(a).reshape(-1)))
            elif strict:
                raise KeyError(v.name)
        self._filters_dirty = True

    def get_gradients(self):
        torch.cuda.synchronize()
        return {v.name: self.gvar[v.name].cpu().numpy().reshape(v.shape) for v in self.graph.trainable()}

    def _alloc_activations(self):
        B, T, dev = self.B, self.dtype, self.device
        self._roots, self._groots = {}, {}
        for t in self.graph.tensors:
            if t.base is None:
                self._roots[t.name] = staggered(B * t.h * t.w * t.ld, T, dev)
                if self.training and t not in self.graph.inputs.values():
                    self._groots[t.name] = staggered(B * t.h * t.w * t.ld, T, dev)
        self.conv = {}
        max_y = 0
        max_c = 8
        for op in self.graph.ops:
            if op['kind'] != 'conv':
                continue
            k, cin, cout = op['ksize'], op['cin'], op['cout']
            cp, ldy = pad8(cin), pad8(cout)
            st = {'Ffwd': staggered(cout * k * k * cp, T, dev)}
            if self.training and op['x'] not in self.graph.inputs.values():
                st['Fdgr'] = staggered(cin * k * k * ldy, T, dev)
            if op['bn']:
                st['mean'] = torch.zeros(cout, dtype=torch.float32, device=dev)
                st['var'] = torch.ones(cout, dtype=torch.float32, device=dev)
            self.conv[op['name']] = st
            max_y = max(max_y, B * op['out'].h * op['out'].w * ldy)
            max_c = max(max_c, ldy)
        self._bindings = {}
        self._tmp_roots = {}
        self._bind(self.graph)
        self.parts = _PartPool(3, 2 * 256 * max(max_c, 8), dev)
        self._bz_pending = {}
        conv_bytes = 0
        for op in self.graph.ops:
            if op['kind'] == 'conv':
                x = op['x']
                for cp, nf in ((pad8(op['cin']), op['cout']), (pad8(op['cout']), op['cin'])):
                    conv_bytes = max(conv_bytes, ops.workspace_bytes('conv2d', B, x.h, x.w, cp, nf, op['ksize'], ops.dtype_code(T)))
        self.conv_ws = torch.zeros(conv_bytes // 4 + 1024, dtype=torch.float32, device=dev)
        ws_bytes = max(ops.workspace_bytes('bn', max_c), ops.workspace_bytes('bias_grad', max_c)) + ops.workspace_bytes('image_prep', B)
        self.ws = torch.zeros(ws_bytes // 8 + 64, dtype=torch.float64, device=dev)
        if self.training:
            self.dy_ring = [staggered(max_y, T, dev) for _ in range(3)]
            self.dy_free = [None, None, None]
            lo, hi = torch.cuda.Stream.priority_range()
            self.side_stream = torch.cuda.Stream(device=dev, priority=max(min(self.opts.side_priority, max(lo, hi)), min(lo, hi)))
            self.wgrad_ws = None
            if self.deterministic:
                self._alloc_wgrad_ws(self.graph)
        self.img = None

    def _bind(self, graph):
        B, T, dev = self.B, self.dtype, self.device
        act, gact = {}, {}
        for t in graph.tensors:
            r, off, ld = t.storage()
            root = self._roots[r.name]
            assert B * r.h * r.w * r.ld <= root.numel(), 'input size exceeds the one the engine was allocated for (%s)' % r.name
            act[t] = (root[off:], ld)
            if r.name in self._groots:
                gact[t] = (self._groots[r.name][off:], ld)
        plan = plan_binding(graph, B, T, self.training, self.opts, self.pools)
        for op in graph.ops:
            if op['kind'] != 'conv':
                continue
            lp, st = plan.layers[op['name']], self.conv[op['name']]
            if self.training and lp.pool is not None:
                need = B * (op['out'].h // 2) * (op['out'].w // 2) * op['cout']
                if 'pool_idx' not in st or st['pool_idx'].numel() < need:
                    st['pool_idx'] = torch.zeros(need, dtype=torch.uint8, device=dev)
                if self.opts.fold_finalize and ('pool_ymax' not in st or st['pool_ymax'].numel() < need):
                    st['pool_ymax'] = staggered(need, T, dev)
            if lp.path == 'fold' and 'fold_w' not in st:
                st['fold_w'] = torch.empty_like(self.var[op['weights'].name])
                st['fold_bias'] = torch.empty(op['cout'], dtype=torch.float32, device=dev)
        inp = next(iter(graph.inputs.values()))
        self._bindings[(inp.h, inp.w)] = {'graph': graph, 'act': act, 'gact': gact, 'plan': plan, 'tmp_grad': {}}
        self._use(inp.h, inp.w)

    def _use(self, h, w):
        self._cur = bnd = self._bindings[(h, w)]
        self.graph, self.act, self.gact, self.plan, self.tmp_grad = bnd['graph'], bnd['act'], bnd['gact'], bnd['plan'], bnd['tmp_grad']

    fused_pool = property(lambda self: self.plan.fused_pool)
    fwd_pool = property(lambda self: self.plan.fwd_pool)
    bn_bwd_fused = property(lambda self: self.plan.bn_bwd_fused)

    def _first_fused(self, op):
        return self.plan.layers[op['name']].path == 'first'

    def _plan_grad_zeroing(self):
        return list(self.plan.zero_ranges)

    def add_size(self, graph):
        names = [v.name for v in graph.variables.values()]
        assert names == [v.name for v in self._bindings[next(iter(self._bindings))]['graph'].variables.values()], 'different network'
        (inp,) = self.graph.inputs.values()
        self._bind(graph)
        if self.deterministic:
            self._alloc_wgrad_ws(graph)
        self._use(inp.h, inp.w)

    def _alloc_wgrad_ws(self, graph):
        need = 0
        for op in graph.ops:
            if op['kind'] == 'conv':
                x = op['x']
                r, off, ldx = x.storage()
                need = max(need, ops.conv2d_wgrad_workspace_bytes(self.B, x.h, x.w, op['cin'], ldx, op['cout'], pad8(op['cout']), op['ksize'], self.dtype))
        if self.wgrad_ws is None or self.wgrad_ws.numel() * 4 < need:
            self.wgrad_ws = torch.empty(need // 4 + 4, dtype=torch.float32, device=self.device)

    def _wgrad(self, xb, dy, dW, B, h, w, cin, ldx, cout, ldy, k):
        if self.deterministic:
            stream = torch.cuda.current_stream().cuda_stream
            if self._wgrad_stream is None:
                self._wgrad_stream = stream
            assert stream == self._wgrad_stream, 'deterministic mode: filter gradients of one backward sweep on two streams share one workspace'
            ops.conv2d_wgrad_ws(xb, dy, dW, self.wgrad_ws, B, h, w, cin, ldx, cout, ldy, k)
        else:
            ops.conv2d_wgrad(xb, dy, dW, B, h, w, cin, ldx, cout, ldy, k)

    def set_size(self, height, width):
        if (height, width) not in self._bindings:
            raise KeyError('input size %dx%d was not bound (Engine.add_size)' % (height, width))
        self._use(height, width)

    def _timer(self, H, W, Nf, k, real_k):
        t = self.kernel_timer if Nf > 64 else None
        if t is not None:
            t.start(2.0 * self.B * H * W * Nf * real_k, self._phase if k == 3 else '1x1')
        return t

    def _conv(self, P, F, bias, O, H, W, Cp, ldp, Nf, ldo, k, real_k):
        t = self._timer(H, W, Nf, k, real_k)
        ops.conv2d_ws(P, F, bias, O, self.conv_ws, self.B, H, W, Cp, ldp, Nf, ldo, k)
        if t is not None:
            t.stop()

    def _conv_stats(self, P, F, O, H, W, Cp, ldp, Nf, ldo, k, real_k, shift):
        t = self._timer(H, W, Nf, k, real_k)
        part = self.parts.acquire(2 * 256 * Nf)
        ops.conv2d_bn(P, F, O, self.conv_ws, self.B, H, W, Cp, ldp, Nf, ldo, k, shift, self.parts.bufs[part])
        if t is not None:
            t.stop()
        return part, ops.last_bn_part_rows()

    def _conv_dgrad_bn(self, P, F, O, H, W, Cp, ldp, Nf, ldo, k, real_k, prod):
        pst = self.conv[prod['name']]
        dgam, dbet = self.gvar[prod['gamma'].name], self.gvar[prod['beta'].name]
        t = self._timer(H, W, Nf, k, real_k)
        part = self.parts.acquire(2 * 256 * Nf)
        pending = ops.conv2d_dgrad_bn(P, F, O, self.conv_ws, self.B, H, W, Cp, ldp, Nf, ldo, k, self.act[prod['y']][0], pst['mean'], pst['var'],
                                      self.var[prod['gamma'].name], self.var[prod['beta'].name], dgam, dbet,
                                      self.parts.bufs[part], self.ws, BN_EPS, LEAKY_ALPHA)
        if t is not None:
            t.stop()
        if not pending:
            self.parts.dirty[part] = 0
            self.parts.consumed(part)
            return None
        rows = ops.last_bn_part_rows()
        if self.opts.fold_finalize and ops.bn_fin_supported(rows, Nf, self.dtype):
            return _Sums(self.parts.bufs[part], rows, 256 * Nf, part)
        ops.bn_part_to_grads(self.parts.bufs[part], Nf, dgam, dbet)
        self.parts.consumed(part, cleared=True)
        return None

    def _prepare_filters(self):
        if not self._filters_dirty:
            return
        self._filter_descs()
        for op in self.graph.ops:
            if op['kind'] == 'conv' and self.plan.layers[op['name']].path == 'fold':
                st = self.conv[op['name']]
                ops.bn_fold(self.var[op['weights'].name], self.var[op['gamma'].name], self.var[op['beta'].name], self.var[op['moving_mean'].name],
                            self.var[op['moving_variance'].name], st['fold_w'], st['fold_bias'], op['ksize'] ** 2 * op['cin'], op['cout'], BN_EPS)
        ops.filter_prep_batch(self._fdesc, self._fdesc_n, self._fdesc_blocks, self.dtype)
        self._filters_dirty = False

    def _filter_descs(self):
        if getattr(self, '_fdesc', None) is not None:
            return
        from ._lib import FilterDesc
        convs = [op for op in self.graph.ops if op['kind'] == 'conv']
        arr = (FilterDesc * len(convs))()
        first = 0
        for d, op in zip(arr, convs):
            st = self.conv[op['name']]
            k, ldcin, ldcout = op['ksize'], pad8(op['cin']), pad8(op['cout'])
            d.W = (st['fold_w'] if self.plan.layers[op['name']].path == 'fold' else self.var[op['weights'].name]).data_ptr()
            d.Ffwd = st['Ffwd'].data_ptr()
            d.Fdgr = st['Fdgr'].data_ptr() if 'Fdgr' in st else None
            d.ksize, d.cin, d.ldcin, d.cout, d.ldcout, d.first_block = k, op['cin'], ldcin, op['cout'], ldcout, first
            first += ops.filter_prep_blocks(k, ldcin, ldcout)
        raw = bytes(arr)
        self._fdesc = torch.frombuffer(bytearray(raw), dtype=torch.uint8).to(self.device)
        self._fdesc_n, self._fdesc_blocks = len(convs), first
        import ctypes
        self._fdesc1_info = {}
        size = ctypes.sizeof(FilterDesc)
        bounds = [d.first_block for d in arr] + [first]
        for i, (d, op) in enumerate(zip(arr, convs)):
            self._fdesc1_info[op['name']] = (i * size, bounds[i + 1] - bounds[i])
            d.first_block = 0
        self._fdesc1 = torch.frombuffer(bytearray(bytes(arr)), dtype=torch.uint8).to(self.device)
        covered = sorted(self.param_offsets[op['weights'].name] for op in self.graph.ops if op['kind'] == 'conv')
        small = sorted(v for k, v in self.param_offsets.items() if v not in covered)
        flat = [x for o, n in small for x in (o, n)]
        self._small = torch.tensor(flat if flat else [0, 0], dtype=torch.int64, device=self.device)
        self._n_small = len(small)

    def adam_update_and_prepare(self, m, v, alpha, beta1, beta2, eps, gscale):
        self._filter_descs()
        ops.adam_filter_prep(self._fdesc, self._fdesc_n, self._fdesc_blocks, self._small, self._n_small, self.params, self.grads, m, v,
                             alpha, beta1, beta2, eps, gscale, self.dtype)
        self._filters_dirty = False

    def adam_update_layer(self, op, m, v, alpha, beta1, beta2, eps, gscale):
        self._filter_descs()
        off, blocks = self._fdesc1_info[op['name']]
        ops.adam_filter_prep(self._fdesc1[off:], 1, blocks, self._small, 0, self.params, self.grads, m, v, alpha, beta1, beta2, eps, gscale, self.dtype)

    def adam_update_small(self, m, v, alpha, beta1, beta2, eps, gscale):
        self._filter_descs()
        ops.adam_filter_prep(self._fdesc, 0, 0, self._small, self._n_small, self.params, self.grads, m, v, alpha, beta1, beta2, eps, gscale, self.dtype)
        self._filters_dirty = False

    def set_images(self, images, mode=0):
        (inp,) = self.graph.inputs.values()
        assert images.dtype == torch.float32 and images.is_cuda and images.numel() == self.B * inp.h * inp.w * 3
        self.img = images.contiguous()
        ops.image_prep(self.img, self.act[inp][0], self.ws, self.B, inp.h * inp.w, mode)

    def zero_grads(self):
        if self.plan.zero_ranges:
            ops.zero_ranges(self.grads, self.plan.zero_ranges)

    def forward(self):
        with ops.deterministic_launches(self.deterministic):
            self._forward()

    def _forward(self):
        self._prepare_filters()
        B = self.B
        if self.training:
            self.state_snap.copy_(self.state)
        pooled = set()
        for op in self.graph.ops:
            kind = op['kind']
            if kind == 'conv':
                x, out = op['x'], op['out']
                xb, ldx = self.act[x]
                st = self.conv[op['name']]
                M = B * out.h * out.w
                lp = self.plan.layers[op['name']]
                pool = lp.pool
                if lp.path == 'fold':
                    ob, ldo = self.act[out]
                    ops.conv2d_bias_leaky(xb, st['Ffwd'], st['fold_bias'], ob, self.conv_ws, B, x.h, x.w, pad8(x.c), ldx, op['cout'], ldo, op['ksize'], LEAKY_ALPHA)
                elif lp.path == 'first':
                    gamma, beta = self.var[op['gamma'].name], self.var[op['beta'].name]
                    mmean, mvar = self.var[op['moving_mean'].name], self.var[op['moving_variance'].name]
                    pb, ldp = self.act[pool['out']]
                    if self.training:
                        part = self.parts.acquire(2 * 256 * 32)
                        shift = self.svar[op['moving_mean'].name]
                        ops.first_layer_stats(xb, st['Ffwd'], B, x.h, x.w, shift, self.parts.bufs[part])
                        ops.bn_finalize(self.parts.bufs[part], shift, M, 32, st['mean'], st['var'], mmean, mvar, BN_DECAY)
                        self.parts.consumed(part, cleared=True)
                        mean, var = st['mean'], st['var']
                    else:
                        mean, var = mmean, mvar
                    ops.first_layer_bn_leaky_pool(xb, st['Ffwd'], mean, var, gamma, beta, pb, st.get('pool_idx') if self.training else None,
                                                  B, x.h, x.w, ldp, BN_EPS, LEAKY_ALPHA)
                elif lp.path == 'bn':
                    yb, ldy = self.act[op['y']]
                    gamma, beta = self.var[op['gamma'].name], self.var[op['beta'].name]
                    mmean, mvar = self.var[op['moving_mean'].name], self.var[op['moving_variance'].name]
                    shift = self.svar[op['moving_mean'].name]
                    conv = (xb, st['Ffwd'], yb, x.h, x.w, pad8(x.c), ldx, op['cout'], ldy, op['ksize'], op['ksize'] ** 2 * op['cin'])
                    mean, var = (st['mean'], st['var']) if self.training else (mmean, mvar)
                    fin = False
                    if lp.stats:
                        part, rows = self._conv_stats(*conv, shift)
                        fin = self.opts.fold_finalize and ops.bn_fin_supported(rows, op['cout'], self.dtype)
                        if not fin:
                            if self.sync_bn and self.bn_world > 1:
                                self._sync_bn_sums(self.parts.bufs[part], op['cout'])
                            ops.bn_finalize(self.parts.bufs[part], shift, M * (self.bn_world if self.sync_bn else 1), op['cout'], st['mean'], st['var'],
                                            mmean, mvar, BN_DECAY)
                            self.parts.consumed(part, cleared=True)
                    else:
                        self._conv(conv[0], conv[1], None, *conv[2:])
                        if self.training:
                            assert not (self.sync_bn and self.bn_world > 1), 'sync_bn needs the statistics from the convolution epilogue (YOLO2_FUSE_BN_STATS=1, dense output)'
                            ops.bn_stats_ema(yb, st['mean'], st['var'], mmean, mvar, BN_DECAY, self.ws, M, op['cout'])
                    if fin:
                        zbuf, zn = self.parts.take_to_zero(part)
                        if pool is not None:
                            pb, ldp = self.act[pool['out']]
                            ops.bn_leaky_pool_fin(yb, self.parts.bufs[part], rows, shift, mean, var, mmean, mvar, BN_DECAY, gamma, beta, pb, st.get('pool_idx'),
                                                  B, out.h, out.w, op['cout'], ldp, BN_EPS, LEAKY_ALPHA, zbuf, zn, ymax=st.get('pool_ymax'))
                            st['ymax_valid'] = 'pool_ymax' in st
                        elif lp.fwd_pool is not None:
                            pb, ldp = self.act[lp.fwd_pool['out']]
                            ops.bn_leaky_pool_fin(yb, self.parts.bufs[part], rows, shift, mean, var, mmean, mvar, BN_DECAY, gamma, beta, pb, None,
                                                  B, out.h, out.w, op['cout'], ldp, BN_EPS, LEAKY_ALPHA, zbuf, zn, a_full=self.act[out][0])
                            pooled.add(lp.fwd_pool['name'])
                        else:
                            ob, ldo = self.act[out]
                            ops.bn_leaky_fin(yb, self.parts.bufs[part], rows, shift, mean, var, mmean, mvar, BN_DECAY, gamma, beta, ob, M, op['cout'], ldo,
                                             BN_EPS, LEAKY_ALPHA, zbuf, zn)
                        self.parts.consumed(part)
                    elif pool is not None:
                        pb, ldp = self.act[pool['out']]
                        ops.bn_leaky_pool(yb, mean, var, gamma, beta, pb, st.get('pool_idx'), B, out.h, out.w, op['cout'], ldp, BN_EPS, LEAKY_ALPHA)
                        st['ymax_valid'] = False
                    else:
                        ob, ldo = self.act[out]
                        ops.bn_leaky(yb, mean, var, gamma, beta, ob, M, op['cout'], ldo, BN_EPS, LEAKY_ALPHA)
                elif lp.path == 'bias_leaky':
                    ob, ldo = self.act[out]
                    ops.conv2d_bias_leaky(xb, st['Ffwd'], self.var[op['biases'].name], ob, self.conv_ws, B, x.h, x.w, pad8(x.c), ldx, op['cout'], ldo, op['ksize'], LEAKY_ALPHA)
                else:
                    ob, ldo = self.act[out]
                    self._conv(xb, st['Ffwd'], self.var[op['biases'].name], ob, x.h, x.w, pad8(x.c), ldx, op['cout'], ldo, op['ksize'], op['ksize'] ** 2 * op['cin'])
            elif kind == 'flatten':
                pass
            elif kind == 'dropout':
                x, out = op['x'], op['out']
                n = B * x.h * x.w * self.act[x][1]
                mask = self._dropout_mask(op, n)
                fixed = self.dropout_masks is not None
                self._dropout_calls += 1
                ops.dropout(self.act[x][0], self.act[out][0], mask, n, op['keep_prob'], 0 if fixed else self._dropout_seed_for(op))
            elif kind == 'pool':
                x, out = op['x'], op['out']
                if x in self.fused_pool or op['name'] in pooled:
                    continue
                assert self.act[x][1] == x.c and self.act[out][1] == out.c
                ops.maxpool_fwd(self.act[x][0], self.act[out][0], B, x.h, x.w, x.c, op['stride'])
            elif kind == 'reorg':
                x, out = op['x'], op['out']
                assert self.act[x][1] == x.c
                ops.reorg(self.act[x][0], self.act[out][0], B, x.h, x.w, x.c, self.act[out][1])
            elif kind == 'concat':
                pass
            else:
                raise ValueError(kind)

    def _grad_sink(self, t, written):
        gb, ld = self.gact[t]
        if t not in written:
            written.add(t)
            return gb, ld, None
        tmp = self.tmp_grad.get(t)
        if tmp is None:
            n = self.B * t.h * t.w * ld
            root = self._tmp_roots.get(t.name)
            if root is None or root.numel() < n:
                root = self._tmp_roots[t.name] = torch.zeros(n, dtype=self.dtype, device=self.device)
            tmp = self.tmp_grad[t] = root
        n = self.B * t.h * t.w * ld
        return tmp, ld, (lambda: ops.add_inplace(gb, tmp, n))

    def backward(self, on_layer_done=None):
        with ops.deterministic_launches(self.deterministic):
            self._backward(on_layer_done)

    def _backward(self, on_layer_done=None):
        B = self.B
        self._wgrad_stream = None
        written = set()
        reduced = set()
        inputs = set(self.graph.inputs.values())
        self._phase = 'dgrad'
        if self._has_l2:
            self.reg_loss.zero_()
        main = torch.cuda.current_stream()
        side = self.side_stream if self.overlap_wgrad else None
        slot = 0

        def next_dy():
            nonlocal slot
            slot = (slot + 1) % 3
            if self.dy_free[slot] is not None:
                main.wait_event(self.dy_free[slot])
            return self.dy_ring[slot]
        for op in reversed(self.graph.ops):
            kind = op['kind']
            if kind == 'conv':
                x, out = op['x'], op['out']
                st = self.conv[op['name']]
                lp = self.plan.layers[op['name']]
                M = B * out.h * out.w
                cout, k = op['cout'], op['ksize']
                ldy = pad8(cout)
                gob, ldgo = self.gact[out]
                xb, ldx = self.act[x]
                if op['bn']:
                    yb, _ = self.act[op['y']]
                    gamma, beta = self.var[op['gamma'].name], self.var[op['beta'].name]
                    dgam, dbet = self.gvar[op['gamma'].name], self.gvar[op['beta'].name]
                    pool, limit, first = lp.pool, lp.fin_limit, lp.path == 'first'
                    pfin = None
                    if first:
                        dpb, lddp = self.gact[pool['out']]
                        part = self.parts.acquire(2 * 256 * 32)
                        ops.first_layer_pool_bwd_reduce(xb, st['Ffwd'], dpb, lddp, st['pool_idx'], st['mean'], st['var'], gamma, beta, self.parts.bufs[part],
                                                        B, x.h, x.w, BN_EPS, LEAKY_ALPHA)
                        ops.bn_part_to_grads(self.parts.bufs[part], 32, dgam, dbet)
                        self.parts.consumed(part, cleared=True)
                    elif pool is not None:
                        dpb, lddp = self.gact[pool['out']]
                        if limit >= 64 and st.get('ymax_valid'):
                            rows = ops.bn_leaky_bwd_reduce_part(dpb, lddp, st['pool_ymax'], st['mean'], st['var'], gamma, beta, self.ws, limit,
                                                                M // 4, cout, BN_EPS, LEAKY_ALPHA)
                            pfin = _Sums(self.ws, rows, rows * cout, -1)
                        elif limit >= 128:
                            rows = ops.bn_leaky_pool_bwd_reduce_part(dpb, lddp, st['pool_idx'], yb, st['mean'], st['var'], gamma, beta, self.ws, limit,
                                                                     B, out.h, out.w, cout, BN_EPS, LEAKY_ALPHA)
                            pfin = _Sums(self.ws, rows, rows * cout, -1)
                        else:
                            ops.bn_leaky_pool_bwd_reduce(dpb, lddp, st['pool_idx'], yb, st['mean'], st['var'], gamma, beta, dgam, dbet, self.ws,
                                                         B, out.h, out.w, cout, BN_EPS, LEAKY_ALPHA)
                    elif op['name'] in reduced:
                        pfin = self._bz_pending.pop(op['name'], None)
                    elif limit >= 64:
                        rows = ops.bn_leaky_bwd_reduce_part(gob, ldgo, yb, st['mean'], st['var'], gamma, beta, self.ws, limit, M, cout, BN_EPS, LEAKY_ALPHA)
                        pfin = _Sums(self.ws, rows, rows * cout, -1)
                    else:
                        ops.bn_leaky_bwd_reduce(gob, ldgo, yb, st['mean'], st['var'], gamma, beta, dgam, dbet, self.ws, M, cout, BN_EPS, LEAKY_ALPHA)
                    dy = None if lp.first_wgrad else next_dy()
                    assert dy is not None or pfin is not None
                    if first:
                        ops.first_layer_pool_bwd_apply(xb, st['Ffwd'], dpb, lddp, st['pool_idx'], st['mean'], st['var'], gamma, beta, dgam, dbet, dy,
                                                       B, x.h, x.w, BN_EPS, LEAKY_ALPHA)
                    elif pfin is not None:
                        zbuf, zn = self.parts.take_to_zero(pfin.part)
                        if lp.first_wgrad:
                            ops.first_layer_wgrad_bn(xb, yb, dpb, lddp, st['pool_idx'], st['mean'], st['var'], gamma, beta, pfin.buf, pfin.rows, pfin.stride,
                                                     dgam, dbet, self.gvar[op['weights'].name], B, x.h, x.w, op['cin'], BN_EPS, LEAKY_ALPHA, zbuf, zn)
                            self._l2(op)
                        elif pool is not None:
                            ops.bn_leaky_pool_bwd_apply_fin(dpb, lddp, st['pool_idx'], yb, st['mean'], st['var'], gamma, beta, pfin.buf, pfin.rows, pfin.stride,
                                                            dgam, dbet, dy, B, out.h, out.w, cout, BN_EPS, LEAKY_ALPHA, zbuf, zn)
                        else:
                            ops.bn_leaky_bwd_apply_fin(gob, ldgo, yb, st['mean'], st['var'], gamma, beta, pfin.buf, pfin.rows, pfin.stride, dgam, dbet, dy,
                                                       M, cout, BN_EPS, LEAKY_ALPHA, zbuf, zn)
                        if pfin.part >= 0:
                            self.parts.consumed(pfin.part)
                    elif pool is not None:
                        ag, ab = self._sync_bn_grads(dgam, dbet, cout)
                        ops.bn_leaky_pool_bwd_apply(dpb, lddp, st['pool_idx'], yb, st['mean'], st['var'], gamma, beta, ag, ab, dy,
                                                    B, out.h, out.w, cout, BN_EPS, LEAKY_ALPHA)
                    else:
                        ag, ab = self._sync_bn_grads(dgam, dbet, cout)
                        ops.bn_leaky_bwd_apply(gob, ldgo, yb, st['mean'], st['var'], gamma, beta, ag, ab, dy, M, cout, BN_EPS, LEAKY_ALPHA)
                    ring = True
                elif op['act']:
                    assert ldgo == ldy and self.act[out][1] == ldy
                    dy = next_dy()
                    ops.leaky_bwd(self.act[out][0], gob, dy, M * ldy, LEAKY_ALPHA)
                    ops.bias_grad(dy, ldy, self.gvar[op['biases'].name], self.ws, M, cout)
                    ring = True
                else:
                    dy = gob
                    assert ldgo == ldy
                    ops.bias_grad(dy, ldy, self.gvar[op['biases'].name], self.ws, M, cout)
                    ring = False
                done = None
                if lp.first_wgrad:
                    pass
                elif side is not None:
                    ready = torch.cuda.Event()
                    ready.record(main)
                    side.wait_event(ready)
                    with torch.cuda.stream(side):
                        self._wgrad(xb, dy, self.gvar[op['weights'].name], B, x.h, x.w, op['cin'], ldx, cout, ldy, k)
                        self._l2(op)
                        done = torch.cuda.Event()
                        done.record(side)
                    if ring:
                        self.dy_free[slot] = done
                else:
                    self._wgrad(xb, dy, self.gvar[op['weights'].name], B, x.h, x.w, op['cin'], ldx, cout, ldy, k)
                    self._l2(op)
                if x not in inputs:
                    prod = lp.bn_bwd
                    dst, ldd, fin = self._grad_sink(x, written)
                    if prod is not None and fin is None:
                        pend = self._conv_dgrad_bn(dy, st['Fdgr'], dst, x.h, x.w, ldy, ldy, op['cin'], ldd, k, k * k * cout, prod)
                        reduced.add(prod['name'])
                        if pend is not None:
                            self._bz_pending[prod['name']] = pend
                    else:
                        self._conv(dy, st['Fdgr'], None, dst, x.h, x.w, ldy, ldy, op['cin'], ldd, k, k * k * cout)
                    if fin:
                        fin()
                if on_layer_done is not None:
                    on_layer_done(op, done)
            elif kind == 'pool':
                x, out = op['x'], op['out']
                if x in self.fused_pool:
                    continue
                if x in written and op['stride'] == 2 and self.gact[x][1] == x.c:
                    ops.maxpool_bwd_acc(self.act[x][0], self.gact[out][0], self.gact[x][0], B, x.h, x.w, x.c)
                    continue
                dst, ldd, fin = self._grad_sink(x, written)
                assert ldd == x.c
                ops.maxpool_bwd(self.act[x][0], self.gact[out][0], dst, B, x.h, x.w, x.c, op['stride'])
                if fin:
                    fin()
            elif kind == 'reorg':
                x, out = op['x'], op['out']
                dst, ldd, fin = self._grad_sink(x, written)
                assert ldd == x.c
                ops.reorg_bwd(self.gact[out][0], self.gact[out][1], dst, B, x.h, x.w, x.c)
                if fin:
                    fin()
            elif kind == 'concat':
                for v in op['inputs']:
                    written.add(v)
            elif kind == 'flatten':
                written.add(op['x'])
            elif kind == 'dropout':
                x, out = op['x'], op['out']
                dst, ldd, fin = self._grad_sink(x, written)
                n = B * x.h * x.w * ldd
                ops.dropout_bwd(self.gact[out][0], self._dropout_mask(op, n), dst, n, op['keep_prob'])
                if fin:
                    fin()
        self._phase = 'fwd'
        if side is not None:
            main.wait_stream(side)

    def _sync_bn_sums(self, part, C):
        import torch.distributed as dist
        sums = self._bn_sync_buf(2 * C)
        ops.bn_part_to_grads(part, C, sums[:C], sums[C:])
        dist.all_reduce(sums, group=self.bn_group)
        part[:C].copy_(sums[:C])
        part[BN_PART_ROWS * C:BN_PART_ROWS * C + C].copy_(sums[C:])

    def _sync_bn_grads(self, dgam, dbet, C):
        if not (self.sync_bn and self.bn_world > 1):
            return dgam, dbet
        import torch.distributed as dist
        sums = self._bn_sync_buf(2 * C)
        sums[:C].copy_(dgam)
        sums[C:].copy_(dbet)
        dist.all_reduce(sums, group=self.bn_group)
        sums.mul_(1.0 / self.bn_world)
        return sums[:C], sums[C:]

    def _bn_sync_buf(self, n):
        buf = getattr(self, '_bn_sync', None)
        if buf is None or buf.numel() < n:
            buf = self._bn_sync = torch.zeros(max(n, 4096), dtype=torch.float32, device=self.device)
        return buf[:n]

    def _l2(self, op):
        if op.get('l2', 0.0) > 0.0:
            w = self.var[op['weights'].name]
            ops.l2_regularizer(w, self.gvar[op['weights'].name], w.numel(), op['l2'], self.reg_loss)

    def _dropout_seed_for(self, op):
        idx = [o['name'] for o in self.graph.ops if o['kind'] == 'dropout'].index(op['name'])
        h = (self.dropout_seed * 0x9E3779B97F4A7C15 + self.dropout_rank * 0xC2B2AE3D27D4EB4F + self.dropout_step * 0x165667B19E3779F9 + idx * 0xD6E8FEB86659FD93)
        h &= (1 << 64) - 1
        h ^= h >> 31
        return (h % ((1 << 62) - 1)) + 1

    def _dropout_mask(self, op, n):
        if self.dropout_masks is not None:
            return self.dropout_masks[op['name']]
        m = self._masks.get(op['name'])
        if m is None or m.numel() < n:
            m = self._masks[op['name']] = torch.zeros(n, dtype=torch.uint8, device=self.device)
        return m

    def output(self):
        return self.graph.ops[-1]['out']

    def summarizable_tensors(self):
        assert self.training, 'the summaries describe a training step'
        out = []
        for t in self.graph.tensors:
            if t.flat_of is not None:
                continue
            if t in self.plan.unstored:
                out.append((t, None))
            else:
                buf, ld = self.act[t]
                out.append((t, (buf, self.B * t.h * t.w, t.c, ld)))
        return out
```

yolo_tf_amd/ops.py:

```python
import ctypes

import numpy as np
import torch

from . import _lib
from ._lib import call, ptr, dtype_code


_raw_stream = getattr(torch._C, '_cuda_getCurrentRawStream', None)
_raw_device = getattr(torch._C, '_cuda_getDevice', None)


def _stream():
    if _raw_stream is None or _raw_device is None:
        return ctypes.c_void_p(torch.cuda.current_stream().cuda_stream)
    return ctypes.c_void_p(_raw_stream(_raw_device()))


def pad8(c):
    return (c + 7) // 8 * 8


def conv2d(P, F, bias, O, B, H, W, Cp, ldp, Nf, ldo, ksize):
    call('yolo2_conv2d', ptr(P), ptr(F), ptr(bias), ptr(O), B, H, W, Cp, ldp, Nf, ldo, ksize, dtype_code(P.dtype), _stream())


def conv2d_ws(P, F, bias, O, ws, B, H, W, Cp, ldp, Nf, ldo, ksize):
    call('yolo2_conv2d_ws', ptr(P), ptr(F), ptr(bias), ptr(O), ptr(ws), ws.numel() * ws.element_size(), B, H, W, Cp, ldp, Nf, ldo, ksize,
         dtype_code(P.dtype), _stream())


def conv2d_bias_leaky(P, F, bias, O, ws, B, H, W, Cp, ldp, Nf, ldo, ksize, alpha):
    call('yolo2_conv2d_bias_leaky', ptr(P), ptr(F), ptr(bias), ptr(O), ptr(ws), ws.numel() * ws.element_size(), B, H, W, Cp, ldp, Nf, ldo, ksize,
         alpha, dtype_code(P.dtype), _stream())


def conv2d_bn(P, F, O, ws, B, H, W, Cp, ldp, Nf, ldo, ksize, shift, bn_part):
    call('yolo2_conv2d_bn', ptr(P), ptr(F), ptr(O), ptr(ws), ws.numel() * ws.element_size(), B, H, W, Cp, ldp, Nf, ldo, ksize,
         ptr(shift), ptr(bn_part), dtype_code(P.dtype), _stream())


def conv2d_dgrad_bn(dY, F, dX, ws, B, H, W, Cp, ldp, Nf, ldo, ksize, Yprev, mean, var, gamma, beta, dgamma, dbeta, bn_part, red_ws, eps, alpha):
    pending = ctypes.c_int(0)
    call('yolo2_conv2d_dgrad_bn', ptr(dY), ptr(F), ptr(dX), ptr(ws), ws.numel() * ws.element_size(), B, H, W, Cp, ldp, Nf, ldo, ksize,
         ptr(Yprev), ptr(mean), ptr(var), ptr(gamma), ptr(beta), ptr(dgamma), ptr(dbeta), ptr(bn_part), ptr(red_ws), eps, alpha,
         ctypes.byref(pending), dtype_code(dY.dtype), _stream())
    return bool(pending.value)


def conv2d_dgrad_bn_fuses(B, H, W, Nf, ksize, dtype):
    lib = _lib.load()
    if 'yolo2_conv2d_dgrad_bn_fuses' in _lib.MISSING:
        return True
    return bool(lib.yolo2_conv2d_dgrad_bn_fuses(B, H, W, Nf, ksize, dtype_code(dtype)))


def filter_prep_blocks(ksize, ldcin, ldcout):
    lib = _lib.load()
    if 'yolo2_filter_prep_blocks' in _lib.MISSING:
        return ksize * ksize * ((ldcin + 63) // 64) * ((ldcout + 63) // 64)
    return int(lib.yolo2_filter_prep_blocks(ksize, ldcin, ldcout))


def bn_part_to_grads(bn_part, C, dgamma, dbeta):
    call('yolo2_bn_part_to_grads', ptr(bn_part), C, ptr(dgamma), ptr(dbeta), _stream())


def bn_finalize(bn_part, shift, M, C, mean, var, mm, mv, decay):
    call('yolo2_bn_finalize', ptr(bn_part), ptr(shift), M, C, ptr(mean), ptr(var), ptr(mm), ptr(mv), decay, _stream())


def conv2d_wgrad_accumulates(B, H, W, Cin, ldx, Cout, ldy, ksize, dtype):
    return bool(_lib.load().yolo2_conv2d_wgrad_accumulates(B, H, W, Cin, ldx, Cout, ldy, ksize, dtype_code(dtype)))


def conv2d_wgrad(X, dY, dW, B, H, W, Cin, ldx, Cout, ldy, ksize):
    call('yolo2_conv2d_wgrad', ptr(X), ptr(dY), ptr(dW), B, H, W, Cin, ldx, Cout, ldy, ksize, dtype_code(X.dtype), _stream())


def conv2d_wgrad_workspace_bytes(B, H, W, Cin, ldx, Cout, ldy, ksize, dtype):
    return int(_lib.query('yolo2_conv2d_wgrad_workspace_bytes', B, H, W, Cin, ldx, Cout, ldy, ksize, dtype_code(dtype)))


def conv2d_wgrad_ws(X, dY, dW, ws, B, H, W, Cin, ldx, Cout, ldy, ksize):
    call('yolo2_conv2d_wgrad_ws', ptr(X), ptr(dY), ptr(dW), ptr(ws), 0 if ws is None else ws.numel() * ws.element_size(), B, H, W, Cin, ldx, Cout, ldy,
         ksize, dtype_code(X.dtype), _stream())


def wgrad_ws_plan(B, H, W, Cin, ldx, Cout, ldy, ksize, dtype, cus):
    out = (ctypes.c_int * 4)()
    rc = _lib.load().yolo2_debug_wgrad_ws_plan(B, H, W, Cin, ldx, Cout, ldy, ksize, dtype_code(dtype), cus, out)
    if rc != 0:
        raise _lib.HipKernelError('yolo2_debug_wgrad_ws_plan failed (code %d)' % rc)
    return dict(zip(('family', 'slots', 'slot_floats', 'blocks'), list(out)))


def set_deterministic(on):
    call('yolo2_set_deterministic', 1 if on else 0)


class deterministic_launches(object):

    def __init__(self, on):
        self.on = bool(on)
        self.prev = 0

    def __enter__(self):
        if self.on:
            self.prev = int(_lib.query('yolo2_get_deterministic'))
            if not self.prev:
                set_deterministic(True)

    def __exit__(self, *exc):
        if self.on and not self.prev:
            set_deterministic(False)
        return False


def filter_prep(Wt, Ffwd, Fdgr, ksize, Cin, ldcin, Cout, ldcout, dtype):
    call('yolo2_filter_prep', ptr(Wt), ptr(Ffwd), ptr(Fdgr), ksize, Cin, ldcin, Cout, ldcout, dtype_code(dtype), _stream())


def filter_prep_batch(descs_dev, n, total_blocks, dtype):
    call('yolo2_filter_prep_batch', ptr(descs_dev), n, total_blocks, dtype_code(dtype), _stream())


def adam_filter_prep(descs_dev, n, total_blocks, small_dev, n_small, params, grads, m, v, alpha, b1, b2, eps, gscale, dtype):
    call('yolo2_adam_filter_prep', ptr(descs_dev), n, total_blocks, ptr(small_dev), n_small, ptr(params), ptr(grads), ptr(m), ptr(v), alpha, b1, b2, eps, gscale,
         dtype_code(dtype), _stream())


def bn_stats(Y, mean, var, ws, M, C):
    call('yolo2_bn_stats', ptr(Y), ptr(mean), ptr(var), ptr(ws), M, C, dtype_code(Y.dtype), _stream())


def bn_stats_ema(Y, mean, var, mm, mv, decay, ws, M, C):
    call('yolo2_bn_stats_ema', ptr(Y), ptr(mean), ptr(var), ptr(mm), ptr(mv), decay, ptr(ws), M, C, dtype_code(Y.dtype), _stream())


def bn_ema(mm, mv, mean, var, C, decay):
    call('yolo2_bn_ema', ptr(mm), ptr(mv), ptr(mean), ptr(var), C, decay, _stream())


def bn_leaky(Y, mean, var, gamma, beta, A, M, C, lda, eps, alpha):
    call('yolo2_bn_leaky', ptr(Y), ptr(mean), ptr(var), ptr(gamma), ptr(beta), ptr(A), M, C, lda, eps, alpha, dtype_code(Y.dtype), _stream())


def bn_leaky_bwd_reduce(dA, ldda, Y, mean, var, gamma, beta, dgamma, dbeta, ws, M, C, eps, alpha):
    call('yolo2_bn_leaky_bwd_reduce', ptr(dA), ldda, ptr(Y), ptr(mean), ptr(var), ptr(gamma), ptr(beta), ptr(dgamma), ptr(dbeta), ptr(ws),
         M, C, eps, alpha, dtype_code(Y.dtype), _stream())


def bn_leaky_bwd_apply(dA, ldda, Y, mean, var, gamma, beta, dgamma, dbeta, dY, M, C, eps, alpha):
    call('yolo2_bn_leaky_bwd_apply', ptr(dA), ldda, ptr(Y), ptr(mean), ptr(var), ptr(gamma), ptr(beta), ptr(dgamma), ptr(dbeta), ptr(dY),
         M, C, eps, alpha, dtype_code(Y.dtype), _stream())


def last_bn_part_rows():
    return int(_lib.load().yolo2_last_bn_part_rows())


def bn_fin_supported(rows, C, dtype):
    return bool(_lib.load().yolo2_bn_fin_supported(int(rows), int(C), dtype_code(dtype)))


def bn_fin_rows_limit(C, dtype, cap=1024):
    r = cap
    while r >= 1 and not bn_fin_supported(r, C, dtype):
        r //= 2
    return r


def _zero_args(zero, zero_floats):
    return (ptr(zero) if zero_floats else None), int(zero_floats)


def bn_leaky_fin(Y, bn_part, rows, shift, mean, var, mm, mv, decay, gamma, beta, A, M, C, lda, eps, alpha, zero=None, zero_floats=0):
    z, zn = _zero_args(zero, zero_floats)
    call('yolo2_bn_leaky_fin', ptr(Y), ptr(bn_part), rows, ptr(shift), ptr(mean), ptr(var), ptr(mm), ptr(mv), decay, ptr(gamma), ptr(beta), ptr(A),
         M, C, lda, eps, alpha, z, zn, dtype_code(Y.dtype), _stream())


def bn_leaky_pool_fin(Y, bn_part, rows, shift, mean, var, mm, mv, decay, gamma, beta, P, idx, B, H, W, C, ldp, eps, alpha, zero=None, zero_floats=0, ymax=None, a_full=None):
    z, zn = _zero_args(zero, zero_floats)
    call('yolo2_bn_leaky_pool_fin', ptr(Y), ptr(bn_part), rows, ptr(shift), ptr(mean), ptr(var), ptr(mm), ptr(mv), decay, ptr(gamma), ptr(beta),
         ptr(P), ptr(idx), ptr(ymax), ptr(a_full), B, H, W, C, ldp, eps, alpha, z, zn, dtype_code(Y.dtype), _stream())


def bn_leaky_bwd_apply_fin(dA, ldda, Y, mean, var, gamma, beta, part, rows, plane_stride, dgamma, dbeta, dY, M, C, eps, alpha, zero=None, zero_floats=0):
    z, zn = _zero_args(zero, zero_floats)
    call('yolo2_bn_leaky_bwd_apply_fin', ptr(dA), ldda, ptr(Y), ptr(mean), ptr(var), ptr(gamma), ptr(beta), ptr(part), rows, plane_stride,
         ptr(dgamma), ptr(dbeta), ptr(dY), M, C, eps, alpha, z, zn, dtype_code(Y.dtype), _stream())


def bn_leaky_pool_bwd_apply_fin(dP, lddp, idx, Y, mean, var, gamma, beta, part, rows, plane_stride, dgamma, dbeta, dY, B, H, W, C, eps, alpha,
                                zero=None, zero_floats=0):
    z, zn = _zero_args(zero, zero_floats)
    call('yolo2_bn_leaky_pool_bwd_apply_fin', ptr(dP), lddp, ptr(idx), ptr(Y), ptr(mean), ptr(var), ptr(gamma), ptr(beta), ptr(part), rows, plane_stride,
         ptr(dgamma), ptr(dbeta), ptr(dY), B, H, W, C, eps, alpha, z, zn, dtype_code(Y.dtype), _stream())


def first_layer_wgrad_bn(X, Y, dP, lddp, idx, mean, var, gamma, beta, part, rows, plane_stride, dgamma, dbeta, dW, B, H, W, Cin, eps, alpha,
                         zero=None, zero_floats=0):
    z, zn = _zero_args(zero, zero_floats)
    call('yolo2_first_layer_wgrad_bn', ptr(X), ptr(Y), ptr(dP), lddp, ptr(idx), ptr(mean), ptr(var), ptr(gamma), ptr(beta), ptr(part), rows, plane_stride,
         ptr(dgamma), ptr(dbeta), ptr(dW), B, H, W, Cin, eps, alpha, z, zn, dtype_code(Y.dtype), _stream())


def bn_leaky_bwd_reduce_part(dA, ldda, Y, mean, var, gamma, beta, ws, rows_limit, M, C, eps, alpha):
    rows = ctypes.c_int(0)
    call('yolo2_bn_leaky_bwd_reduce_part', ptr(dA), ldda, ptr(Y), ptr(mean), ptr(var), ptr(gamma), ptr(beta), ptr(ws), ctypes.byref(rows), rows_limit, M, C,
         eps, alpha, dtype_code(Y.dtype), _stream())
    return rows.value


def bn_leaky_pool_bwd_reduce_part(dP, lddp, idx, Y, mean, var, gamma, beta, ws, rows_limit, B, H, W, C, eps, alpha):
    rows = ctypes.c_int(0)
    call('yolo2_bn_leaky_pool_bwd_reduce_part', ptr(dP), lddp, ptr(idx), ptr(Y), ptr(mean), ptr(var), ptr(gamma), ptr(beta), ptr(ws), ctypes.byref(rows),
         rows_limit, B, H, W, C, eps, alpha, dtype_code(Y.dtype), _stream())
    return rows.value


def bn_leaky_pool(Y, mean, var, gamma, beta, P, idx, B, H, W, C, ldp, eps, alpha):
    call('yolo2_bn_leaky_pool', ptr(Y), ptr(mean), ptr(var), ptr(gamma), ptr(beta), ptr(P), ptr(idx), B, H, W, C, ldp, eps, alpha,
         dtype_code(Y.dtype), _stream())


def bn_leaky_pool_bwd_reduce(dP, lddp, idx, Y, mean, var, gamma, beta, dgamma, dbeta, ws, B, H, W, C, eps, alpha):
    call('yolo2_bn_leaky_pool_bwd_reduce', ptr(dP), lddp, ptr(idx), ptr(Y), ptr(mean), ptr(var), ptr(gamma), ptr(beta), ptr(dgamma), ptr(dbeta),
         ptr(ws), B, H, W, C, eps, alpha, dtype_code(Y.dtype), _stream())


def bn_leaky_pool_bwd_apply(dP, lddp, idx, Y, mean, var, gamma, beta, dgamma, dbeta, dY, B, H, W, C, eps, alpha):
    call('yolo2_bn_leaky_pool_bwd_apply', ptr(dP), lddp, ptr(idx), ptr(Y), ptr(mean), ptr(var), ptr(gamma), ptr(beta), ptr(dgamma), ptr(dbeta),
         ptr(dY), B, H, W, C, eps, alpha, dtype_code(Y.dtype), _stream())


def maxpool_fwd(A, P, B, H, W, C, stride):
    call('yolo2_maxpool_fwd', ptr(A), ptr(P), B, H, W, C, stride, dtype_code(A.dtype), _stream())


def maxpool_bwd(A, dP, dA, B, H, W, C, stride):
    call('yolo2_maxpool_bwd', ptr(A), ptr(dP), ptr(dA), B, H, W, C, stride, dtype_code(A.dtype), _stream())


def maxpool_bwd_acc(A, dP, dA, B, H, W, C):
    call('yolo2_maxpool_bwd_acc', ptr(A), ptr(dP), ptr(dA), B, H, W, C, dtype_code(A.dtype), _stream())


def reorg(x, out, B, H, W, C, ldo):
    call('yolo2_reorg', ptr(x), ptr(out), B, H, W, C, ldo, dtype_code(x.dtype), _stream())


def reorg_bwd(dout, ldd, din, B, H, W, C):
    call('yolo2_reorg_bwd', ptr(dout), ldd, ptr(din), B, H, W, C, dtype_code(din.dtype), _stream())


def copy_channels(src, lds, dst, ldd, M, C):
    call('yolo2_copy_channels', ptr(src), lds, ptr(dst), ldd, M, C, dtype_code(src.dtype), _stream())


def add_inplace(dst, src, n):
    call('yolo2_add_inplace', ptr(dst), ptr(src), n, dtype_code(dst.dtype), _stream())


def bias_grad(dY, ld, dbias, ws, M, C):
    call('yolo2_bias_grad', ptr(dY), ld, ptr(dbias), ptr(ws), M, C, dtype_code(dY.dtype), _stream())


def image_prep(img, out, ws, B, HW, mode):
    call('yolo2_image_prep', ptr(img), ptr(out), ptr(ws), B, HW, mode, dtype_code(out.dtype), _stream())


def head_decode(logits, ld, anchors, conf, xy_min, xy_max, nan_flag, B, ch, cw, A, C):
    call('yolo2_head_decode', ptr(logits), ld, ptr(anchors), ptr(conf), ptr(xy_min), ptr(xy_max), ptr(nan_flag), B, ch, cw, A, C,
         dtype_code(logits.dtype), _stream())


def head_decode_attrs(logits, ld, anchors, iou, prob, xy, wh, B, ch, cw, A, C):
    call('yolo2_head_decode_attrs', ptr(logits), ld, ptr(anchors), ptr(iou), ptr(prob), ptr(xy), ptr(wh), B, ch, cw, A, C,
         dtype_code(logits.dtype), _stream())


def box_loss_code(box_loss):
    try:
        return _lib.BOX_LOSSES[box_loss]
    except (KeyError, TypeError):
        raise ValueError('box_loss = %r: one of %s' % (box_loss, ', '.join(_lib.BOX_LOSSES)))


def loss_options(box_loss='mse', class_loss='mse', ignore_thresh=0.0, rescore=False, label_smoothing=0.0, focal_gamma=2.0):
    mode = box_loss_code(box_loss)
    try:
        cls = _lib.CLASS_LOSSES[class_loss]
    except (KeyError, TypeError):
        raise ValueError('class_loss = %r: one of %s' % (class_loss, ', '.join(_lib.CLASS_LOSSES)))
    try:
        t, eps, gamma = float(ignore_thresh), float(label_smoothing), float(focal_gamma)
    except (TypeError, ValueError):
        raise ValueError('ignore_thresh, label_smoothing and focal_gamma are numbers, not %r, %r, %r' % (ignore_thresh, label_smoothing, focal_gamma))
    if not (t == 0.0 or 0.0 < t < 1.0):
        raise ValueError('ignore_thresh = %r: 0 (off) or a threshold inside (0, 1)' % (ignore_thresh,))
    if rescore not in (False, True, 0, 1):
        raise ValueError('rescore = %r: True or False' % (rescore,))
    if not 0.0 <= eps < 1.0:
        raise ValueError('label_smoothing = %r: lies in [0, 1)' % (label_smoothing,))
    if eps != 0.0 and cls == 0:
        raise ValueError('label_smoothing = %r with class_loss mse: smoothing belongs to ce and focal' % (label_smoothing,))
    if cls == 2 and not (gamma == 0.0 or (1.0 <= gamma < float('inf'))):
        raise ValueError('focal_gamma = %r: 0 or at least 1' % (focal_gamma,))
    if cls == 0 and t == 0.0 and not rescore:
        return None
    return _lib.LossOptions(ctypes.sizeof(_lib.LossOptions), mode, cls, int(bool(rescore)), t, eps, gamma if cls == 2 else 2.0)


def loss(logits, ld, anchors, labels, hparam, objectives, dlogits, ws, B, ch, cw, A, C, box_loss='mse', class_loss='mse', ignore_thresh=0.0,
         rescore=False, label_smoothing=0.0, focal_gamma=2.0):
    mode = box_loss_code(box_loss)
    opt = loss_options(box_loss, class_loss, ignore_thresh, rescore, label_smoothing, focal_gamma)
    hp = (ctypes.c_float * 4)(*[float(v) for v in hparam])
    mask, prob, coords, omin, omax, areas = labels
    if opt is not None:
        call('yolo2_loss_ex', ptr(logits), ld, ptr(anchors), ptr(mask), ptr(prob), ptr(coords), ptr(omin), ptr(omax), ptr(areas), hp,
             ptr(objectives), ptr(dlogits), ptr(ws), B, ch, cw, A, C, dtype_code(logits.dtype), _stream(), ctypes.byref(opt))
    elif mode == 0:
        call('yolo2_loss', ptr(logits), ld, ptr(anchors), ptr(mask), ptr(prob), ptr(coords), ptr(omin), ptr(omax), ptr(areas), hp,
             ptr(objectives), ptr(dlogits), ptr(ws), B, ch, cw, A, C, dtype_code(logits.dtype), _stream())
    else:
        call('yolo2_loss_box', ptr(logits), ld, ptr(anchors), ptr(mask), ptr(prob), ptr(coords), ptr(omin), ptr(omax), ptr(areas), hp,
             ptr(objectives), ptr(dlogits), ptr(ws), B, ch, cw, A, C, dtype_code(logits.dtype), _stream(), mode)


def loss_partials(logits, ld, anchors, labels, hparam, dlogits, ws, B, ch, cw, A, C, box_loss='mse', class_loss='mse', ignore_thresh=0.0,
                  rescore=False, label_smoothing=0.0, focal_gamma=2.0):
    mode = box_loss_code(box_loss)
    opt = loss_options(box_loss, class_loss, ignore_thresh, rescore, label_smoothing, focal_gamma)
    hp = (ctypes.c_float * 4)(*[float(v) for v in hparam])
    mask, prob, coords, omin, omax, areas = labels
    if opt is not None:
        call('yolo2_loss_ex_partials', ptr(logits), ld, ptr(anchors), ptr(mask), ptr(prob), ptr(coords), ptr(omin), ptr(omax), ptr(areas), hp,
             ptr(dlogits), ptr(ws), B, ch, cw, A, C, dtype_code(logits.dtype), _stream(), ctypes.byref(opt))
    elif mode == 0:
        call('yolo2_loss_partials', ptr(logits), ld, ptr(anchors), ptr(mask), ptr(prob), ptr(coords), ptr(omin), ptr(omax), ptr(areas), hp,
             ptr(dlogits), ptr(ws), B, ch, cw, A, C, dtype_code(logits.dtype), _stream())
    else:
        call('yolo2_loss_box_partials', ptr(logits), ld, ptr(anchors), ptr(mask), ptr(prob), ptr(coords), ptr(omin), ptr(omax), ptr(areas), hp,
             ptr(dlogits), ptr(ws), B, ch, cw, A, C, dtype_code(logits.dtype), _stream(), mode)


def loss_objectives(ws, objectives, B, ch, cw, A):
    call('yolo2_loss_objectives', ptr(ws), ptr(objectives), B, ch, cw, A, _stream())


def loss_ws_floats(B, cells, A):
    return workspace_bytes('loss', B, cells, A) // 4


def nms(conf, xy_min, xy_max, order, ws, B, N, C, thr, thr_iou):
    call('yolo2_nms', ptr(conf), ptr(xy_min), ptr(xy_max), ptr(order), ptr(ws), B, N, C, thr, thr_iou, _stream())


def soft_nms(conf, xy_min, xy_max, order, B, N, C, method, thr, thr_iou, sigma=0.5):
    if isinstance(method, str):
        if method not in _lib.NMS_METHODS:
            raise ValueError('nms method must be one of %s, not %r' % (', '.join(_lib.NMS_METHODS), method))
        method = _lib.NMS_METHODS[method]
    call('yolo2_soft_nms', ptr(conf), ptr(xy_min), ptr(xy_max), ptr(order), B, N, C, int(method), thr, thr_iou, sigma, _stream())


def tta_gather(conf, xy_min, xy_max, out_conf, out_xy_min, out_xy_max, B, N, C, M, offset, sx, sy, cell_w0, flip):
    call('yolo2_tta_gather', ptr(conf), ptr(xy_min), ptr(xy_max), ptr(out_conf), ptr(out_xy_min), ptr(out_xy_max), B, N, C, M, int(offset),
         float(sx), float(sy), float(cell_w0), int(bool(flip)), _stream())


def wbf(conf, xy_min, xy_max, out_conf, out_xy_min, out_xy_max, rows, flags, ws, B, M, C, V, max_per_class, R, thr, fuse_iou):
    call('yolo2_wbf', ptr(conf), ptr(xy_min), ptr(xy_max), ptr(out_conf), ptr(out_xy_min), ptr(out_xy_max), ptr(rows), ptr(flags), ptr(ws),
         B, M, C, int(V), int(max_per_class), int(R), float(thr), float(fuse_iou), _stream())


WBF_MAX_CANDIDATES = 4096
WBF_FLAG_CANDIDATES, WBF_FLAG_CLUSTERS, WBF_FLAG_ROWS = 1, 2, 4


def adam(w, g, m, v, n, alpha, b1, b2, eps, gscale=1.0):
    call('yolo2_adam', ptr(w), ptr(g), ptr(m), ptr(v), n, alpha, b1, b2, eps, gscale, _stream())


def momentum(w, g, acc, n, lr, mom, gscale=1.0):
    call('yolo2_momentum', ptr(w), ptr(g), ptr(acc), n, lr, mom, gscale, _stream())


def sgd(w, g, n, lr, gscale=1.0):
    call('yolo2_sgd', ptr(w), ptr(g), n, lr, gscale, _stream())


def rmsprop(w, g, ms, mom, n, lr, decay, momentum_, eps, gscale=1.0):
    call('yolo2_rmsprop', ptr(w), ptr(g), ptr(ms), ptr(mom), n, lr, decay, momentum_, eps, gscale, _stream())


def adagrad(w, g, acc, n, lr, gscale=1.0):
    call('yolo2_adagrad', ptr(w), ptr(g), ptr(acc), n, lr, gscale, _stream())


def adadelta(w, g, acc, accu, n, lr, rho, eps, gscale=1.0):
    call('yolo2_adadelta', ptr(w), ptr(g), ptr(acc), ptr(accu), n, lr, rho, eps, gscale, _stream())


def ftrl(w, g, accum, linear, n, lr, lr_power, l1, l2, gscale=1.0):
    call('yolo2_ftrl', ptr(w), ptr(g), ptr(accum), ptr(linear), n, lr, lr_power, l1, l2, gscale, _stream())


def scale(x, n, s):
    call('yolo2_scale', ptr(x), n, s, _stream())


def ema_update(ema, w, n, one_minus_decay):
    call('yolo2_ema_update', ptr(ema), ptr(w), n, one_minus_decay, _stream())


GRAD_STORE, GRAD_ADD, GRAD_FINAL = 0, 1, 2
GRAD_COMBINE_CHUNK = 4096


def check_grad_ranges(ranges, n):
    out, last = [], 0
    for b, e in ranges:
        b, e = int(b), int(e)
        if not (0 <= b < e <= n):
            raise ValueError('grad_combine: the range [%d, %d) is empty or outside [0, %d)' % (b, e, n))
        if b < last:
            raise ValueError('grad_combine: the range [%d, %d) is out of order or overlaps the range before it (which ends at %d)' % (b, e, last))
        out.append((b, e))
        last = e
    return out


def grad_ranges(ranges, n, device):
    flat = [v for be in check_grad_ranges(ranges, n) for v in be]
    return torch.tensor(flat, dtype=torch.int64, device=device) if flat else None


def grad_combine(g, acc, w, n, mode, scale=1.0, decay=0.0, shrink=1.0, table=None):
    call('yolo2_grad_combine', ptr(g), ptr(acc), ptr(w), n, mode, scale, decay, shrink, ptr(table), 0 if table is None else table.numel() // 2, _stream())


def zero_ranges(x, ranges):
    flat = (ctypes.c_long * (2 * len(ranges)))(*[int(v) for ab in ranges for v in ab])
    call('yolo2_zero_ranges', ptr(x), flat, len(ranges), _stream())


def bn_fold(W, gamma, beta, mean, var, Wf, bias, rows, C, eps):
    call('yolo2_bn_fold', ptr(W), ptr(gamma), ptr(beta), ptr(mean), ptr(var), ptr(Wf), ptr(bias), rows, C, eps, _stream())


def workspace_bytes(kind, *args):
    return int(_lib.query('yolo2_%s_workspace_bytes' % kind, *args))


def clip_by_norm(g, seg_off, nseg, clip, ws):
    call('yolo2_clip_by_norm', ptr(g), ptr(seg_off), nseg, clip, ptr(ws), _stream())


def clip_by_norm_fixed(g, seg_off, nseg, clip, ws):
    call('yolo2_clip_by_norm_fixed', ptr(g), ptr(seg_off), nseg, clip, ptr(ws), ws.numel() * ws.element_size(), _stream())


def selftest_tr16():
    out = torch.zeros(256, dtype=torch.int16, device='cuda')
    call('yolo2_selftest_tr16', ptr(out), _stream())
    torch.cuda.synchronize()
    return out.cpu().numpy().reshape(64, 4)


CONV_PLAN_KEYS = ('BM', 'BN', 'waves', 'chunks', 'stages', 'split', 'grid_x', 'grid_y')
WGRAD_PLAN_KEYS = ('BC', 'BN', 'waves', 'pair', 'ranges', 'remap', 'blocks', 'direct')


def last_conv_plan():
    out = (ctypes.c_int * 8)()
    _lib.load().yolo2_debug_last_conv_plan(out)
    return dict(zip(CONV_PLAN_KEYS, list(out)))


CONV_ROUTE_MODES = {'plain': 0, 'bias_act': 1, 'bn': 2, 'dgrad_bn': 3}
CONV_ROUTE_EXCLUDE = {'first': 1, 'c32': 2, 'c64': 4, 'd1': 8, 'tap': 16, 's4': 32, 'stream': 64}
CONV_ROUTE_STATS = ('none', 'epilogue', 'colsum', 'two_step')
CONV_ROUTE_FAMILIES = ('first', 'c32', 'c64', 'd1', 'pp', 's4', 'igemm')


def conv_route(B, H, W, Cp, ldp, Nf, ldo, ksize, dtype, mode, ws_bytes, cus=0, exclude=(), align_bits=7):
    out = (ctypes.c_int * 12)()
    mask = 0
    for name in exclude:
        mask |= CONV_ROUTE_EXCLUDE[name]
    rc = _lib.load().yolo2_debug_conv_route(B, H, W, Cp, ldp, Nf, ldo, ksize, dtype_code(dtype), CONV_ROUTE_MODES[mode], align_bits, ws_bytes, cus, mask, out)
    if rc != 0:
        raise _lib.HipKernelError('yolo2_debug_conv_route failed (code %d)' % rc)
    return dict(plan=dict(zip(CONV_PLAN_KEYS, list(out)[:8])), rows=out[8], stats=CONV_ROUTE_STATS[out[9]], pending=out[10], family=CONV_ROUTE_FAMILIES[out[11]])


def noop():
    call('yolo2_debug_noop', _stream())


def set_igemm_tap(mode):
    _lib.load().yolo2_debug_set_igemm_tap(int(mode))


def set_pp(grid=-1, dmapos=-1, min_steps=-1, min_share=-1):
    _lib.load().yolo2_debug_set_pp(int(grid), int(dmapos), int(min_steps), int(min_share))


def set_pp_cost(cv):
    lib = _lib.load()
    if 'yolo2_debug_set_pp_cost' not in _lib.MISSING:
        lib.yolo2_debug_set_pp_cost(int(cv))


def check_async_errors():
    call('yolo2_check_async_errors', _stream())


class AsyncErrorPoll(object):
# ... 354 lines not shown
```

Measured before the change: 4775 img/s.

## Fold YOLOv2 passthrough reorg into BN-leaky-pool forward and backward kernels

In YOLOv2 the passthrough layer's activation feeds both a maxpool and a space-to-depth reorg. This change writes the reorg output straight from the fused BN+leaky+pool finalize kernel. In backward, it reads the reorg gradient inside the pool BN reduce and apply kernels, adding it to the routed pool gradient. This removes the separate reorg forward and backward kernels and their extra passes over the full-resolution activation and gradient. In exchange it adds more loads and stores per thread in the fused kernels, plus plan and state bookkeeping to decide when folding applies.

```diff
diff --git a/include/yolo2_hip.h b/include/yolo2_hip.h
--- a/include/yolo2_hip.h
+++ b/include/yolo2_hip.h
@@ -112,6 +112,19 @@
 int yolo2_bn_leaky_pool_bwd_reduce_part(const void *dP, int lddp, const unsigned char *idx, const void *Y, const float *mean,
                                         const float *var, const float *gamma, const float *beta, double *ws, int *rows,
                                         int rows_limit, int B, int H, int W, int C, float eps, float alpha, int dtype, void *stream);
+int yolo2_bn_leaky_pool_fin_reorg(const void *Y, const float *bn_part, int rows, const float *shift, float *mean, float *var,
+                                  float *moving_mean, float *moving_var, double decay, const float *gamma, const float *beta, void *P,
+                                  unsigned char *idx, void *ymax, void *R, int ldr, int block, int B, int H, int W, int C, int ldp,
+                                  float eps, float alpha, float *zero, long zero_floats, int dtype, void *stream);
+int yolo2_bn_leaky_pool_bwd_reduce_part_reorg(const void *dP, int lddp, const unsigned char *idx, const void *Y, const void *dR, int ldr,
+                                              int block, const float *mean, const float *var, const float *gamma, const float *beta,
+                                              double *ws, int *rows, int rows_limit, int B, int H, int W, int C, float eps, float alpha,
+                                              int dtype, void *stream);
+int yolo2_bn_leaky_pool_bwd_apply_fin_reorg(const void *dP, int lddp, const unsigned char *idx, const void *Y, const void *dR, int ldr,
+                                            int block, const float *mean, const float *var, const float *gamma, const float *beta,
+                                            const float *part, int rows, long plane_stride, float *dgamma, float *dbeta, void *dY, int B,
+                                            int H, int W, int C, float eps, float alpha, float *zero, long zero_floats, int dtype,
+                                            void *stream);
 
 int yolo2_first_layer_stats(const void *P, const void *F, int B, int H, int W, const float *shift, float *bn_part, int dtype, void *stream);
 int yolo2_first_layer_bn_leaky_pool(const void *P, const void *F, const float *mean, const float *var, const float *gamma,
diff --git a/yolo_tf_amd/_lib.py b/yolo_tf_amd/_lib.py
--- a/yolo_tf_amd/_lib.py
+++ b/yolo_tf_amd/_lib.py
@@ -51,6 +51,9 @@
     'yolo2_bn_leaky_pool_bwd_apply_fin': [_p, _i, _p, _p, _p, _p, _p, _p, _p, _i, _l, _p, _p, _p, _i, _i, _i, _i, _f, _f, _p, _l, _i, _p],
     'yolo2_bn_leaky_bwd_reduce_part': [_p, _i, _p, _p, _p, _p, _p, _p, _p, _i, _l, _i, _f, _f, _i, _p],
     'yolo2_bn_leaky_pool_bwd_reduce_part': [_p, _i, _p, _p, _p, _p, _p, _p, _p, _p, _i, _i, _i, _i, _i, _f, _f, _i, _p],
+    'yolo2_bn_leaky_pool_fin_reorg': [_p, _p, _i, _p, _p, _p, _p, _p, ctypes.c_double, _p, _p, _p, _p, _p, _p, _i, _i, _i, _i, _i, _i, _i, _f, _f, _p, _l, _i, _p],
+    'yolo2_bn_leaky_pool_bwd_reduce_part_reorg': [_p, _i, _p, _p, _p, _i, _i, _p, _p, _p, _p, _p, _p, _i, _i, _i, _i, _i, _f, _f, _i, _p],
+    'yolo2_bn_leaky_pool_bwd_apply_fin_reorg': [_p, _i, _p, _p, _p, _i, _i, _p, _p, _p, _p, _p, _i, _l, _p, _p, _p, _i, _i, _i, _i, _f, _f, _p, _l, _i, _p],
     'yolo2_bn_leaky_pool': [_p, _p, _p, _p, _p, _p, _p, _i, _i, _i, _i, _i, _f, _f, _i, _p],
     'yolo2_bn_leaky_pool_bwd_reduce': [_p, _i, _p, _p, _p, _p, _p, _p, _p, _p, _p, _i, _i, _i, _i, _f, _f, _i, _p],
     'yolo2_bn_leaky_pool_bwd_apply': [_p, _i, _p, _p, _p, _p, _p, _p, _p, _p, _p, _i, _i, _i, _i, _f, _f, _i, _p],
diff --git a/yolo_tf_amd/csrc/bn.hip b/yolo_tf_amd/csrc/bn.hip
--- a/yolo_tf_amd/csrc/bn.hip
+++ b/yolo_tf_amd/csrc/bn.hip
@@ -190,10 +190,11 @@
     }
 }
 
-template <typename T>
+template <typename T, bool REORG = false>
 __global__ __launch_bounds__(256) void bn_pool_bwd_reduce_kernel(const T *__restrict__ dP, int lddp, const unsigned char *__restrict__ idx, const T *__restrict__ Y,
-                                                                 const float *__restrict__ mean, const float *__restrict__ var, const float *__restrict__ gamma,
-                                                                 const float *__restrict__ beta, float *__restrict__ ws, int B, int H, int W, int C, float eps, float alpha) {
+                                                                 const T *__restrict__ dR, int ldr, const float *__restrict__ mean, const float *__restrict__ var,
+                                                                 const float *__restrict__ gamma, const float *__restrict__ beta, float *__restrict__ ws, int B, int H,
+                                                                 int W, int C, float eps, float alpha) {
     constexpr int N = Vec16<T>::N;
     RowMap rm(C, N);
     float part[2][N];
@@ -213,13 +214,29 @@
         const long MP = (long)B * pr.OH * pr.OW;
         for (long r = (long)blockIdx.x * rm.rpp + rm.rs; r < MP; r += (long)gridDim.x * rm.rpp) {
             const T *src = Y + pr.base(r) + rm.cg * N;
-            Vec16<T> v[4];
+            Vec16<T> v[4], dr[REORG ? 4 : 1];
             v[0] = ld16(src);
             v[1] = ld16(src + C);
             v[2] = ld16(src + (long)W * C);
             v[3] = ld16(src + (long)W * C + C);
             const Vec16<T> d = ld16(dP + r * lddp + rm.cg * N);
             const typename IdxPack<N>::type pack = *reinterpret_cast<const typename IdxPack<N>::type *>(idx + r * C + rm.cg * N);
+            if (REORG) {
+#pragma unroll
+                for (int k = 0; k < (REORG ? 4 : 1); ++k) dr[k] = ld16(dR + r * ldr + (long)k * C + rm.cg * N);
+#pragma unroll
+                for (int j = 0; j < N; ++j) {
+                    const int arg = idx_pack_get(pack, j);
+#pragma unroll
+                    for (int k = 0; k < 4; ++k) {
+                        const float da = pool_round<T>(dr[REORG ? k : 0].get(j) + pool_route(arg, k, d.get(j)));
+                        const BnBwdTerm t = bn_leaky_bwd(v[k].get(j), da, mu[j], inv[j], ga[j], bt[j], alpha);
+                        part[0][j] += t.g * t.xh;
+                        part[1][j] += t.g;
+                    }
+                }
+                continue;
+            }
 #pragma unroll
             for (int j = 0; j < N; ++j) {
                 const int k = idx_pack_get(pack, j);
@@ -360,12 +377,13 @@
     for (long i = ((long)blockIdx.y * gridDim.x + blockIdx.x) * 256 + threadIdx.x; i < zero_vec4; i += nthreads) reinterpret_cast<f32x4 *>(zero)[i] = z;
 }
 
-template <typename T, bool POOL>
+template <typename T, bool POOL, bool REORG = false>
 __global__ __launch_bounds__(256) void bn_leaky_fin_kernel(const T *__restrict__ Y, const float *__restrict__ part, int rows, const float *__restrict__ shift,
                                                            long Mstat, float *__restrict__ mean_out, float *__restrict__ var_out, float *__restrict__ mm,
                                                            float *__restrict__ mv, float omd, const float *__restrict__ gamma, const float *__restrict__ beta,
                                                            T *__restrict__ A, unsigned char *__restrict__ idx, T *__restrict__ ymax, T *__restrict__ Afull,
-                                                           int B, int H, int W, int C, int lda, float eps, float alpha, float *__restrict__ zero, long zero_vec4) {
+                                                           int B, int H, int W, int C, int lda, float eps, float alpha, float *__restrict__ zero, long zero_vec4,
+                                                           int ldr) {
     constexpr int N = Vec16<T>::N;
     const SliceMap sm(C, N);
     double sums[2];
@@ -446,7 +464,11 @@
             }
             st16(A + r * lda + sm.cg * N, o);
             if (idx) *reinterpret_cast<typename IdxPack<N>::type *>(idx + r * C + sm.cg * N) = pack;
-            if (Afull) {
+            if (REORG) {
+                T *dst = Afull + r * ldr + sm.cg * N;
+#pragma unroll
+                for (int k = 0; k < 4; ++k) st16(dst + (long)k * C, af[k]);
+            } else if (Afull) {
                 T *dst = Afull + pr.base(r) + sm.cg * N;
                 st16(dst, af[0]);
                 st16(dst + C, af[1]);
@@ -461,12 +483,12 @@
     }
 }
 
-template <typename T, bool POOL>
+template <typename T, bool POOL, bool REORG = false>
 __global__ __launch_bounds__(256) void bn_bwd_apply_fin_kernel(const T *__restrict__ dA, int ldda, const unsigned char *__restrict__ idx, const T *__restrict__ Y,
                                                                const float *__restrict__ mean, const float *__restrict__ var, const float *__restrict__ gamma,
                                                                const float *__restrict__ beta, const float *__restrict__ part, int rows, long plane,
                                                                float *__restrict__ dgamma, float *__restrict__ dbeta, T *__restrict__ dY, int B, int H, int W, int C,
-                                                               float eps, float alpha, float *__restrict__ zero, long zero_vec4) {
+                                                               float eps, float alpha, float *__restrict__ zero, long zero_vec4, const T *__restrict__ dR, int ldr) {
     constexpr int N = Vec16<T>::N;
     const SliceMap sm(C, N);
     double sums[2];
@@ -476,9 +498,13 @@
     const long step = (long)gridDim.x * sm.rpb;
     long r = (long)blockIdx.x * sm.rpb + sm.row;
     const long koff[4] = {0, C, (long)W * C, (long)W * C + C};
-    Vec16<T> v[POOL ? 4 : 1], d;
+    Vec16<T> v[POOL ? 4 : 1], d, dr[REORG ? 4 : 1];
     typename IdxPack<N>::type pack = 0;
-    auto fetch = [&](long row, Vec16<T> (&yv)[POOL ? 4 : 1], Vec16<T> &dv, typename IdxPack<N>::type &pk) {
+    auto fetch = [&](long row, Vec16<T> (&yv)[POOL ? 4 : 1], Vec16<T> &dv, typename IdxPack<N>::type &pk, Vec16<T> (&rv)[REORG ? 4 : 1]) {
+        if (REORG) {
+#pragma unroll
+            for (int k = 0; k < (REORG ? 4 : 1); ++k) rv[k] = ld16(dR + row * ldr + (long)k * C + sm.cg * N);
+        }
         if (POOL) {
             const long off = pr.base(row) + sm.cg * N;
 #pragma unroll
@@ -487,7 +513,7 @@
         } else yv[0] = ld16(Y + row * C + sm.cg * N);
         dv = ld16(dA + row * ldda + sm.cg * N);
     };
-    if (r < ML) fetch(r, v, d, pack);
+    if (r < ML) fetch(r, v, d, pack, dr);
     slice_partial_sums(part, rows, plane, C, sm, sums);
     if (threadIdx.x < sm.cs) {
         const float dg = (float)sums[0], db = (float)sums[1];
@@ -514,9 +540,9 @@
     grid_zero(zero, zero_vec4);
     while (r < ML) {
         const long rn = r + step;
-        Vec16<T> vn[POOL ? 4 : 1], dn;
+        Vec16<T> vn[POOL ? 4 : 1], dn, drn[REORG ? 4 : 1];
         typename IdxPack<N>::type packn = 0;
-        if (rn < ML) fetch(rn, vn, dn, packn);
+        if (rn < ML) fetch(rn, vn, dn, packn, drn);
         if (!POOL) {
             Vec16<T> o;
 #pragma unroll
@@ -534,8 +560,10 @@
                 Vec16<T> o;
 #pragma unroll
                 for (int j = 0; j < N; ++j) {
-                    const float da = pool_route(idx_pack_get(pack, j), k, d.get(j));
-                    o.set(j, bn_bwd_apply(bn_leaky_bwd(v[POOL ? k : 0].get(j), da, mu[j], inv[j], ga[j], bt[j], alpha), inv[j], ga[j], dgm[j], dbm[j]));
+                    float da = pool_route(idx_pack_get(pack, j), k, d.get(j));
+                    if (REORG) da = pool_round<T>(dr[REORG ? k : 0].get(j) + da);
+                    const BnBwdTerm t = bn_leaky_bwd(v[POOL ? k : 0].get(j), da, mu[j], inv[j], ga[j], bt[j], alpha);
+                    o.set(j, REORG ? (ga[j] * inv[j]) * __builtin_fmaf(-t.xh, dgm[j], t.g - dbm[j]) : bn_bwd_apply(t, inv[j], ga[j], dgm[j], dbm[j]));
                 }
                 st16(dY + off + koff[k], o);
             }
@@ -544,6 +572,10 @@
         for (int k = 0; k < (POOL ? 4 : 1); ++k) v[k] = vn[k];
         d = dn;
         pack = packn;
+        if (REORG) {
+#pragma unroll
+            for (int k = 0; k < (REORG ? 4 : 1); ++k) dr[k] = drn[k];
+        }
         r = rn;
     }
 }
@@ -565,10 +597,11 @@
 }
 static int pool_bwd_reduce_impl(const void *dP, int lddp, const unsigned char *idx, const void *Y, const float *mean, const float *var,
                                 const float *gamma, const float *beta, float *dgamma, float *dbeta, double *ws, int *rows, int rows_limit, int B, int H, int W,
-                                int C, float eps, float alpha, int dtype, void *stream) {
+                                int C, float eps, float alpha, int dtype, void *stream, const void *dR = nullptr, int ldr = 0) {
     Y2_CHECK_ARG(dP && idx && Y && mean && var && gamma && beta && ws && lddp >= C);
     Y2_CHECK_ARG(pool_args_ok(B, H, W, C, dtype));
     const int vec = dtype == YOLO2_BF16 ? 8 : 4;
+    Y2_CHECK_ARG(!dR || (ldr >= 4 * C && ldr % vec == 0));
     hipStream_t st = (hipStream_t)stream;
     const long MP = (long)B * (H / 2) * (W / 2);
     int nb = colsum_grid(MP, C, vec);
@@ -581,7 +614,10 @@
     }
     if (nb > rows_limit) nb = rows_limit;
     float *part = (float *)ws;
-    Y2_DISPATCH_DTYPE(dtype, bn_pool_bwd_reduce_kernel<T><<<nb, 256, 0, st>>>((const T *)dP, lddp, idx, (const T *)Y, mean, var, gamma, beta, part, B, H, W, C, eps, alpha));
+    if (dR)
+        Y2_DISPATCH_DTYPE(dtype, bn_pool_bwd_reduce_kernel<T, true><<<nb, 256, 0, st>>>((const T *)dP, lddp, idx, (const T *)Y, (const T *)dR, ldr, mean, var, gamma, beta, part, B, H, W, C, eps, alpha));
+    else
+        Y2_DISPATCH_DTYPE(dtype, bn_pool_bwd_reduce_kernel<T><<<nb, 256, 0, st>>>((const T *)dP, lddp, idx, (const T *)Y, nullptr, 0, mean, var, gamma, beta, part, B, H, W, C, eps, alpha));
     if (rows) *rows = nb;
     else reduce_finalize_kernel<1><<<cdiv(C, 16), 256, 0, st>>>(part, nb, C, (long)B * H * W, dgamma, dbeta, C);
     Y2_CHECK_LAUNCH();
@@ -598,6 +634,12 @@
                                                    float eps, float alpha, int dtype, void *stream) {
     Y2_CHECK_ARG(rows && rows_limit >= 1);
     return pool_bwd_reduce_impl(dP, lddp, idx, Y, mean, var, gamma, beta, nullptr, nullptr, ws, rows, rows_limit, B, H, W, C, eps, alpha, dtype, stream);
+}
+extern "C" int yolo2_bn_leaky_pool_bwd_reduce_part_reorg(const void *dP, int lddp, const unsigned char *idx, const void *Y, const void *dR, int ldr, int block,
+                                                         const float *mean, const float *var, const float *gamma, const float *beta, double *ws, int *rows,
+                                                         int rows_limit, int B, int H, int W, int C, float eps, float alpha, int dtype, void *stream) {
+    Y2_CHECK_ARG(rows && rows_limit >= 1 && dR && block == 2);
+    return pool_bwd_reduce_impl(dP, lddp, idx, Y, mean, var, gamma, beta, nullptr, nullptr, ws, rows, rows_limit, B, H, W, C, eps, alpha, dtype, stream, dR, ldr);
 }
 extern "C" int yolo2_bn_leaky_pool_bwd_apply(const void *dP, int lddp, const unsigned char *idx, const void *Y, const float *mean, const float *var,
                                              const float *gamma, const float *beta, const float *dgamma, const float *dbeta, void *dY, int B, int H,
@@ -647,26 +689,46 @@
     Y2_CHECK_ARG(lda % vec == 0);
     const dim3 grid = slice_grid(M, C, vec, 4, rows);
     Y2_DISPATCH_DTYPE(dtype, bn_leaky_fin_kernel<T, false><<<grid, 256, 0, (hipStream_t)stream>>>((const T *)Y, bn_part, rows, shift, M, mean, var, moving_mean, moving_var,
-                      (float)(1.0 - decay), gamma, beta, (T *)A, nullptr, nullptr, nullptr, 1, 1, (int)M, C, lda, eps, alpha, zero, zero_floats / 4));
-    Y2_CHECK_LAUNCH();
-    return YOLO2_OK;
-}
-
-extern "C" int yolo2_bn_leaky_pool_fin(const void *Y, const float *bn_part, int rows, const float *shift, float *mean, float *var, float *moving_mean,
-                                       float *moving_var, double decay, const float *gamma, const float *beta, void *P, unsigned char *idx, void *ymax,
-                                       void *A_full, int B, int H, int W, int C, int ldp, float eps, float alpha, float *zero, long zero_floats, int dtype,
-                                       void *stream) {
+                      (float)(1.0 - decay), gamma, beta, (T *)A, nullptr, nullptr, nullptr, 1, 1, (int)M, C, lda, eps, alpha, zero, zero_floats / 4, 0));
+    Y2_CHECK_LAUNCH();
+    return YOLO2_OK;
+}
+
+static int pool_fin_impl(const void *Y, const float *bn_part, int rows, const float *shift, float *mean, float *var, float *moving_mean,
+                         float *moving_var, double decay, const float *gamma, const float *beta, void *P, unsigned char *idx, void *ymax,
+                         void *A_full, bool reorg, int ldr, int B, int H, int W, int C, int ldp, float eps, float alpha, float *zero, long zero_floats,
+                         int dtype, void *stream) {
     Y2_CHECK_ARG(Y && bn_part && shift && mean && var && gamma && beta && P && ldp >= C);
     Y2_CHECK_ARG(pool_args_ok(B, H, W, C, dtype) && ldp % (dtype == YOLO2_BF16 ? 8 : 4) == 0);
     Y2_CHECK_ARG((moving_mean == nullptr) == (moving_var == nullptr) && rows <= Y2_BN_PART_ROWS && fin_shape_ok(rows, C, dtype));
     Y2_CHECK_ARG(shift != moving_mean && shift != mean);
     Y2_CHECK_ZERO(zero, zero_floats);
     const int vec = dtype == YOLO2_BF16 ? 8 : 4;
+    Y2_CHECK_ARG(!reorg || (A_full && ldr >= 4 * C && ldr % vec == 0));
     const dim3 grid = slice_grid((long)B * (H / 2) * (W / 2), C, vec, 2, rows);
-    Y2_DISPATCH_DTYPE(dtype, bn_leaky_fin_kernel<T, true><<<grid, 256, 0, (hipStream_t)stream>>>((const T *)Y, bn_part, rows, shift, (long)B * H * W, mean, var, moving_mean,
-                      moving_var, (float)(1.0 - decay), gamma, beta, (T *)P, idx, (T *)ymax, (T *)A_full, B, H, W, C, ldp, eps, alpha, zero, zero_floats / 4));
-    Y2_CHECK_LAUNCH();
-    return YOLO2_OK;
+    if (reorg)
+        Y2_DISPATCH_DTYPE(dtype, bn_leaky_fin_kernel<T, true, true><<<grid, 256, 0, (hipStream_t)stream>>>((const T *)Y, bn_part, rows, shift, (long)B * H * W, mean, var, moving_mean,
+                          moving_var, (float)(1.0 - decay), gamma, beta, (T *)P, idx, (T *)ymax, (T *)A_full, B, H, W, C, ldp, eps, alpha, zero, zero_floats / 4, ldr));
+    else
+        Y2_DISPATCH_DTYPE(dtype, bn_leaky_fin_kernel<T, true><<<grid, 256, 0, (hipStream_t)stream>>>((const T *)Y, bn_part, rows, shift, (long)B * H * W, mean, var, moving_mean,
+                          moving_var, (float)(1.0 - decay), gamma, beta, (T *)P, idx, (T *)ymax, (T *)A_full, B, H, W, C, ldp, eps, alpha, zero, zero_floats / 4, 0));
+    Y2_CHECK_LAUNCH();
+    return YOLO2_OK;
+}
+extern "C" int yolo2_bn_leaky_pool_fin(const void *Y, const float *bn_part, int rows, const float *shift, float *mean, float *var, float *moving_mean,
+                                       float *moving_var, double decay, const float *gamma, const float *beta, void *P, unsigned char *idx, void *ymax,
+                                       void *A_full, int B, int H, int W, int C, int ldp, float eps, float alpha, float *zero, long zero_floats, int dtype,
+                                       void *stream) {
+    return pool_fin_impl(Y, bn_part, rows, shift, mean, var, moving_mean, moving_var, decay, gamma, beta, P, idx, ymax, A_full, false, 0, B, H, W, C, ldp, eps, alpha,
+                         zero, zero_floats, dtype, stream);
+}
+extern "C" int yolo2_bn_leaky_pool_fin_reorg(const void *Y, const float *bn_part, int rows, const float *shift, float *mean, float *var, float *moving_mean,
+                                             float *moving_var, double decay, const float *gamma, const float *beta, void *P, unsigned char *idx, void *ymax,
+                                             void *R, int ldr, int block, int B, int H, int W, int C, int ldp, float eps, float alpha, float *zero,
+                                             long zero_floats, int dtype, void *stream) {
+    Y2_CHECK_ARG(R && block == 2);
+    return pool_fin_impl(Y, bn_part, rows, shift, mean, var, moving_mean, moving_var, decay, gamma, beta, P, idx, ymax, R, true, ldr, B, H, W, C, ldp, eps, alpha,
+                         zero, zero_floats, dtype, stream);
 }
 
 extern "C" int yolo2_bn_leaky_bwd_apply_fin(const void *dA, int ldda, const void *Y, const float *mean, const float *var, const float *gamma, const float *beta,
@@ -679,24 +741,44 @@
     Y2_CHECK_ARG(ldda % vec == 0);
     const dim3 grid = slice_grid(M, C, vec, 4, rows);
     Y2_DISPATCH_DTYPE(dtype, bn_bwd_apply_fin_kernel<T, false><<<grid, 256, 0, (hipStream_t)stream>>>((const T *)dA, ldda, nullptr, (const T *)Y, mean, var, gamma, beta, part, rows,
-                      plane_stride, dgamma, dbeta, (T *)dY, 1, 1, (int)M, C, eps, alpha, zero, zero_floats / 4));
-    Y2_CHECK_LAUNCH();
-    return YOLO2_OK;
-}
-
+                      plane_stride, dgamma, dbeta, (T *)dY, 1, 1, (int)M, C, eps, alpha, zero, zero_floats / 4, nullptr, 0));
+    Y2_CHECK_LAUNCH();
+    return YOLO2_OK;
+}
+
+static int pool_bwd_apply_fin_impl(const void *dP, int lddp, const unsigned char *idx, const void *Y, const void *dR, int ldr, const float *mean, const float *var,
+                                   const float *gamma, const float *beta, const float *part, int rows, long plane_stride, float *dgamma,
+                                   float *dbeta, void *dY, int B, int H, int W, int C, float eps, float alpha, float *zero, long zero_floats,
+                                   int dtype, void *stream) {
+    Y2_CHECK_ARG(dP && idx && Y && mean && var && gamma && beta && part && dgamma && dbeta && dY && lddp >= C);
+    Y2_CHECK_ARG(pool_args_ok(B, H, W, C, dtype) && plane_stride >= (long)rows * C && fin_shape_ok(rows, C, dtype));
+    Y2_CHECK_ZERO(zero, zero_floats);
+    const int vec = dtype == YOLO2_BF16 ? 8 : 4;
+    Y2_CHECK_ARG(!dR || (ldr >= 4 * C && ldr % vec == 0));
+    const dim3 grid = slice_grid((long)B * (H / 2) * (W / 2), C, vec, 2, rows);
+    if (dR)
+        Y2_DISPATCH_DTYPE(dtype, bn_bwd_apply_fin_kernel<T, true, true><<<grid, 256, 0, (hipStream_t)stream>>>((const T *)dP, lddp, idx, (const T *)Y, mean, var, gamma, beta, part, rows,
+                          plane_stride, dgamma, dbeta, (T *)dY, B, H, W, C, eps, alpha, zero, zero_floats / 4, (const T *)dR, ldr));
+    else
+        Y2_DISPATCH_DTYPE(dtype, bn_bwd_apply_fin_kernel<T, true><<<grid, 256, 0, (hipStream_t)stream>>>((const T *)dP, lddp, idx, (const T *)Y, mean, var, gamma, beta, part, rows,
+                          plane_stride, dgamma, dbeta, (T *)dY, B, H, W, C, eps, alpha, zero, zero_floats / 4, nullptr, 0));
+    Y2_CHECK_LAUNCH();
+    return YOLO2_OK;
+}
 extern "C" int yolo2_bn_leaky_pool_bwd_apply_fin(const void *dP, int lddp, const unsigned char *idx, const void *Y, const float *mean, const float *var,
                                                  const float *gamma, const float *beta, const float *part, int rows, long plane_stride, float *dgamma,
                                                  float *dbeta, void *dY, int B, int H, int W, int C, float eps, float alpha, float *zero, long zero_floats,
                                                  int dtype, void *stream) {
-    Y2_CHECK_ARG(dP && idx && Y && mean && var && gamma && beta && part && dgamma && dbeta && dY && lddp >= C);
-    Y2_CHECK_ARG(pool_args_ok(B, H, W, C, dtype) && plane_stride >= (long)rows * C && fin_shape_ok(rows, C, dtype));
-    Y2_CHECK_ZERO(zero, zero_floats);
-    const int vec = dtype == YOLO2_BF16 ? 8 : 4;
-    const dim3 grid = slice_grid((long)B * (H / 2) * (W / 2), C, vec, 2, rows);
-    Y2_DISPATCH_DTYPE(dtype, bn_bwd_apply_fin_kernel<T, true><<<grid, 256, 0, (hipStream_t)stream>>>((const T *)dP, lddp, idx, (const T *)Y, mean, var, gamma, beta, part, rows,
-                      plane_stride, dgamma, dbeta, (T *)dY, B, H, W, C, eps, alpha, zero, zero_floats / 4));
-    Y2_CHECK_LAUNCH();
-    return YOLO2_OK;
+    return pool_bwd_apply_fin_impl(dP, lddp, idx, Y, nullptr, 0, mean, var, gamma, beta, part, rows, plane_stride, dgamma, dbeta, dY, B, H, W, C, eps, alpha,
+                                   zero, zero_floats, dtype, stream);
+}
+extern "C" int yolo2_bn_leaky_pool_bwd_apply_fin_reorg(const void *dP, int lddp, const unsigned char *idx, const void *Y, const void *dR, int ldr, int block,
+                                                       const float *mean, const float *var, const float *gamma, const float *beta, const float *part, int rows,
+                                                       long plane_stride, float *dgamma, float *dbeta, void *dY, int B, int H, int W, int C, float eps,
+                                                       float alpha, float *zero, long zero_floats, int dtype, void *stream) {
+    Y2_CHECK_ARG(dR && block == 2);
+    return pool_bwd_apply_fin_impl(dP, lddp, idx, Y, dR, ldr, mean, var, gamma, beta, part, rows, plane_stride, dgamma, dbeta, dY, B, H, W, C, eps, alpha,
+                                   zero, zero_floats, dtype, stream);
 }
 
 extern "C" int yolo2_bn_leaky_bwd_reduce_part(const void *dA, int ldda, const void *Y, const float *mean, const float *var, const float *gamma,
diff --git a/yolo_tf_amd/engine.py b/yolo_tf_amd/engine.py
--- a/yolo_tf_amd/engine.py
+++ b/yolo_tf_amd/engine.py
@@ -58,11 +58,16 @@
         side_priority=int(env.get('YOLO2_SIDE_PRIORITY', str(side_priority))))
 
 
-LayerPlan = namedtuple('LayerPlan', 'path pool fwd_pool stats fin_limit first_wgrad bn_bwd zero')
-Plan = namedtuple('Plan', 'layers zero_ranges unstored fused_pool fwd_pool bn_bwd_fused')
-
-
-def plan_binding(graph, batch, dtype, training, opts, pools='all'):
+def read_fuse_reorg(training, env=None):
+    env = os.environ if env is None else env
+    return bool(training) and env.get('YOLO2_FUSE_REORG', '0') == '1'
+
+
+LayerPlan = namedtuple('LayerPlan', 'path pool fwd_pool stats fin_limit first_wgrad bn_bwd zero reorg')
+Plan = namedtuple('Plan', 'layers zero_ranges unstored fused_pool fwd_pool bn_bwd_fused reorg_fused')
+
+
+def plan_binding(graph, batch, dtype, training, opts, pools='all', fuse_reorg=False):
     assert pools in ('all', 'image'), pools
     inputs = set(graph.inputs.values())
     ld = {t: t.storage()[2] for t in graph.tensors}
@@ -83,7 +88,7 @@
             elif pools == 'all' or producers[x]['x'] in inputs:
                 fused_pool[x] = op
     offsets, _ = layout_params(graph)
-    fin_limits, layers, bn_bwd_fused, unstored, ranges = {}, {}, {}, set(), []
+    fin_limits, layers, bn_bwd_fused, reorg_fused, unstored, ranges = {}, {}, {}, {}, set(), []
     for op in convs:
         x, out, cin, cout, k = op['x'], op['out'], op['cin'], op['cout'], op['ksize']
         pool = fused_pool.get(out)
@@ -112,19 +117,25 @@
         if zero:
             off, size = offsets[op['weights'].name]
             ranges.append((off, off + (size + 3) // 4 * 4))
-        if training and pool is not None:
+        reorg = None
+        if fuse_reorg and out in fwd_pool and readers[out] == 2 and path == 'bn' and opts.fuse_bn_stats and ld[op['y']] == cout and fin_limit >= 128:
+            taps = [r for r in graph.ops if r['kind'] == 'reorg' and r['x'] is out]
+            if len(taps) == 1 and ld[taps[0]['out']] >= 4 * cout and 'yolo2_bn_leaky_pool_fin_reorg' not in _lib.MISSING:
+                reorg = taps[0]
+                reorg_fused[out] = op
+        if training and (pool is not None or reorg is not None):
             unstored.add(out)
         if training and path == 'first':
             unstored.add(op['y'])
         layers[op['name']] = LayerPlan(path, pool, fwd_pool.get(out), bool(path == 'bn' and training and opts.fuse_bn_stats and ld[op['y']] == cout),
-                                       fin_limit, first_wgrad, bn_bwd, zero)
+                                       fin_limit, first_wgrad, bn_bwd, zero, reorg)
     zero_ranges = []
     for a, b in sorted(ranges):
         if zero_ranges and a - zero_ranges[-1][1] <= (1 << 20):
             zero_ranges[-1] = (zero_ranges[-1][0], max(zero_ranges[-1][1], b))
         else:
             zero_ranges.append((a, b))
-    return Plan(layers, zero_ranges, frozenset(unstored), fused_pool, fwd_pool, bn_bwd_fused)
+    return Plan(layers, zero_ranges, frozenset(unstored), fused_pool, fwd_pool, bn_bwd_fused, reorg_fused)
 
 
 _SKEW_KB = 20
@@ -192,6 +203,7 @@
         self.training = training
         self.device = torch.device(device if device is not None else 'cuda:%d' % torch.cuda.current_device())
         self.opts = o = read_options(training, self.deterministic, self.sync_bn, side_priority)
+        self.fuse_reorg = read_fuse_reorg(training)
         self.pools = pools
         self.fuse_bn_stats, self.fuse_first_wgrad, self.fold_finalize = o.fuse_bn_stats, o.fuse_first_wgrad, o.fold_finalize
         self.overlap_wgrad = o.overlap_wgrad
@@ -321,16 +333,16 @@
             act[t] = (root[off:], ld)
             if r.name in self._groots:
                 gact[t] = (self._groots[r.name][off:], ld)
-        plan = plan_binding(graph, B, T, self.training, self.opts, self.pools)
+        plan = plan_binding(graph, B, T, self.training, self.opts, self.pools, self.fuse_reorg)
         for op in graph.ops:
             if op['kind'] != 'conv':
                 continue
             lp, st = plan.layers[op['name']], self.conv[op['name']]
-            if self.training and lp.pool is not None:
+            if self.training and (lp.pool is not None or lp.reorg is not None):
                 need = B * (op['out'].h // 2) * (op['out'].w // 2) * op['cout']
                 if 'pool_idx' not in st or st['pool_idx'].numel() < need:
                     st['pool_idx'] = torch.zeros(need, dtype=torch.uint8, device=dev)
-                if self.opts.fold_finalize and ('pool_ymax' not in st or st['pool_ymax'].numel() < need):
+                if lp.pool is not None and self.opts.fold_finalize and ('pool_ymax' not in st or st['pool_ymax'].numel() < need):
                     st['pool_ymax'] = staggered(need, T, dev)
             if lp.path == 'fold' and 'fold_w' not in st:
                 st['fold_w'] = torch.empty_like(self.var[op['weights'].name])
@@ -346,6 +358,10 @@
     fused_pool = property(lambda self: self.plan.fused_pool)
     fwd_pool = property(lambda self: self.plan.fwd_pool)
     bn_bwd_fused = property(lambda self: self.plan.bn_bwd_fused)
+
+    def _reorg_folded(self, x):
+        op = self.plan.reorg_fused.get(x)
+        return op is not None and bool(self.conv[op['name']].get('reorg_folded'))
 
     def _first_fused(self, op):
         return self.plan.layers[op['name']].path == 'first'
@@ -543,6 +559,7 @@
                     conv = (xb, st['Ffwd'], yb, x.h, x.w, pad8(x.c), ldx, op['cout'], ldy, op['ksize'], op['ksize'] ** 2 * op['cin'])
                     mean, var = (st['mean'], st['var']) if self.training else (mmean, mvar)
                     fin = False
+                    st['reorg_folded'] = False
                     if lp.stats:
                         part, rows = self._conv_stats(*conv, shift)
                         fin = self.opts.fold_finalize and ops.bn_fin_supported(rows, op['cout'], self.dtype)
@@ -564,6 +581,12 @@
                             ops.bn_leaky_pool_fin(yb, self.parts.bufs[part], rows, shift, mean, var, mmean, mvar, BN_DECAY, gamma, beta, pb, st.get('pool_idx'),
                                                   B, out.h, out.w, op['cout'], ldp, BN_EPS, LEAKY_ALPHA, zbuf, zn, ymax=st.get('pool_ymax'))
                             st['ymax_valid'] = 'pool_ymax' in st
+                        elif lp.reorg is not None:
+                            pb, ldp = self.act[lp.fwd_pool['out']]
+                            rb, ldr = self.act[lp.reorg['out']]
+                            ops.bn_leaky_pool_fin_reorg(yb, self.parts.bufs[part], rows, shift, mean, var, mmean, mvar, BN_DECAY, gamma, beta, pb, st['pool_idx'],
+                                                        rb, ldr, B, out.h, out.w, op['cout'], ldp, BN_EPS, LEAKY_ALPHA, zbuf, zn)
+                            pooled.add(lp.fwd_pool['name'])
                         elif lp.fwd_pool is not None:
                             pb, ldp = self.act[lp.fwd_pool['out']]
                             ops.bn_leaky_pool_fin(yb, self.parts.bufs[part], rows, shift, mean, var, mmean, mvar, BN_DECAY, gamma, beta, pb, None,
@@ -573,6 +596,7 @@
                             ob, ldo = self.act[out]
                             ops.bn_leaky_fin(yb, self.parts.bufs[part], rows, shift, mean, var, mmean, mvar, BN_DECAY, gamma, beta, ob, M, op['cout'], ldo,
                                              BN_EPS, LEAKY_ALPHA, zbuf, zn)
+                        st['reorg_folded'] = lp.reorg is not None
                         self.parts.consumed(part)
                     elif pool is not None:
                         pb, ldp = self.act[pool['out']]
@@ -604,6 +628,8 @@
                 ops.maxpool_fwd(self.act[x][0], self.act[out][0], B, x.h, x.w, x.c, op['stride'])
             elif kind == 'reorg':
                 x, out = op['x'], op['out']
+                if self._reorg_folded(x):
+                    continue
                 assert self.act[x][1] == x.c
                 ops.reorg(self.act[x][0], self.act[out][0], B, x.h, x.w, x.c, self.act[out][1])
             elif kind == 'concat':
@@ -665,6 +691,7 @@
                     gamma, beta = self.var[op['gamma'].name], self.var[op['beta'].name]
                     dgam, dbet = self.gvar[op['gamma'].name], self.gvar[op['beta'].name]
                     pool, limit, first = lp.pool, lp.fin_limit, lp.path == 'first'
+                    folded = lp.reorg if st.get('reorg_folded') else None
                     pfin = None
                     if first:
                         dpb, lddp = self.gact[pool['out']]
@@ -673,6 +700,12 @@
                                                         B, x.h, x.w, BN_EPS, LEAKY_ALPHA)
                         ops.bn_part_to_grads(self.parts.bufs[part], 32, dgam, dbet)
                         self.parts.consumed(part, cleared=True)
+                    elif folded is not None:
+                        dpb, lddp = self.gact[lp.fwd_pool['out']]
+                        drb, ldr = self.gact[folded['out']]
+                        rows = ops.bn_leaky_pool_bwd_reduce_part_reorg(dpb, lddp, st['pool_idx'], yb, drb, ldr, st['mean'], st['var'], gamma, beta, self.ws, limit,
+                                                                       B, out.h, out.w, cout, BN_EPS, LEAKY_ALPHA)
+                        pfin = _Sums(self.ws, rows, rows * cout, -1)
                     elif pool is not None:
                         dpb, lddp = self.gact[pool['out']]
                         if limit >= 64 and st.get('ymax_valid'):
@@ -704,6 +737,9 @@
                             ops.first_layer_wgrad_bn(xb, yb, dpb, lddp, st['pool_idx'], st['mean'], st['var'], gamma, beta, pfin.buf, pfin.rows, pfin.stride,
                                                      dgam, dbet, self.gvar[op['weights'].name], B, x.h, x.w, op['cin'], BN_EPS, LEAKY_ALPHA, zbuf, zn)
                             self._l2(op)
+                        elif folded is not None:
+                            ops.bn_leaky_pool_bwd_apply_fin_reorg(dpb, lddp, st['pool_idx'], yb, drb, ldr, st['mean'], st['var'], gamma, beta, pfin.buf, pfin.rows,
+                                                                  pfin.stride, dgam, dbet, dy, B, out.h, out.w, cout, BN_EPS, LEAKY_ALPHA, zbuf, zn)
                         elif pool is not None:
                             ops.bn_leaky_pool_bwd_apply_fin(dpb, lddp, st['pool_idx'], yb, st['mean'], st['var'], gamma, beta, pfin.buf, pfin.rows, pfin.stride,
                                                             dgam, dbet, dy, B, out.h, out.w, cout, BN_EPS, LEAKY_ALPHA, zbuf, zn)
@@ -764,7 +800,7 @@
                     on_layer_done(op, done)
             elif kind == 'pool':
                 x, out = op['x'], op['out']
-                if x in self.fused_pool:
+                if x in self.fused_pool or self._reorg_folded(x):
                     continue
                 if x in written and op['stride'] == 2 and self.gact[x][1] == x.c:
                     ops.maxpool_bwd_acc(self.act[x][0], self.gact[out][0], self.gact[x][0], B, x.h, x.w, x.c)
@@ -776,6 +812,8 @@
                     fin()
             elif kind == 'reorg':
                 x, out = op['x'], op['out']
+                if self._reorg_folded(x):
+                    continue
                 dst, ldd, fin = self._grad_sink(x, written)
                 assert ldd == x.c
                 ops.reorg_bwd(self.gact[out][0], self.gact[out][1], dst, B, x.h, x.w, x.c)
diff --git a/yolo_tf_amd/ops.py b/yolo_tf_amd/ops.py
--- a/yolo_tf_amd/ops.py
+++ b/yolo_tf_amd/ops.py
@@ -219,6 +219,27 @@
     call('yolo2_bn_leaky_pool_bwd_reduce_part', ptr(dP), lddp, ptr(idx), ptr(Y), ptr(mean), ptr(var), ptr(gamma), ptr(beta), ptr(ws), ctypes.byref(rows),
          rows_limit, B, H, W, C, eps, alpha, dtype_code(Y.dtype), _stream())
     return rows.value
+
+
+def bn_leaky_pool_fin_reorg(Y, bn_part, rows, shift, mean, var, mm, mv, decay, gamma, beta, P, idx, R, ldr, B, H, W, C, ldp, eps, alpha,
+                            zero=None, zero_floats=0, ymax=None):
+    z, zn = _zero_args(zero, zero_floats)
+    call('yolo2_bn_leaky_pool_fin_reorg', ptr(Y), ptr(bn_part), rows, ptr(shift), ptr(mean), ptr(var), ptr(mm), ptr(mv), decay, ptr(gamma), ptr(beta),
+         ptr(P), ptr(idx), ptr(ymax), ptr(R), ldr, 2, B, H, W, C, ldp, eps, alpha, z, zn, dtype_code(Y.dtype), _stream())
+
+
+def bn_leaky_pool_bwd_reduce_part_reorg(dP, lddp, idx, Y, dR, ldr, mean, var, gamma, beta, ws, rows_limit, B, H, W, C, eps, alpha):
+    rows = ctypes.c_int(0)
+    call('yolo2_bn_leaky_pool_bwd_reduce_part_reorg', ptr(dP), lddp, ptr(idx), ptr(Y), ptr(dR), ldr, 2, ptr(mean), ptr(var), ptr(gamma), ptr(beta), ptr(ws),
+         ctypes.byref(rows), rows_limit, B, H, W, C, eps, alpha, dtype_code(Y.dtype), _stream())
+    return rows.value
+
+
+def bn_leaky_pool_bwd_apply_fin_reorg(dP, lddp, idx, Y, dR, ldr, mean, var, gamma, beta, part, rows, plane_stride, dgamma, dbeta, dY, B, H, W, C, eps, alpha,
+                                      zero=None, zero_floats=0):
+    z, zn = _zero_args(zero, zero_floats)
+    call('yolo2_bn_leaky_pool_bwd_apply_fin_reorg', ptr(dP), lddp, ptr(idx), ptr(Y), ptr(dR), ldr, 2, ptr(mean), ptr(var), ptr(gamma), ptr(beta), ptr(part), rows,
+         plane_stride, ptr(dgamma), ptr(dbeta), ptr(dY), B, H, W, C, eps, alpha, z, zn, dtype_code(Y.dtype), _stream())
 
 
 def bn_leaky_pool(Y, mean, var, gamma, beta, P, idx, B, H, W, C, ldp, eps, alpha):
```

Result: no change. 4742 img/s (-0.7%).
